# Ishikawa-lab/Area_average_interpolation

Measured on NVIDIA B200. Metric: output Mpixels/s (device-timed), higher is better.
Workload: dtype f32

## Files before the change

area_average_interpolation_b200/__init__.py:

```python
from __future__ import annotations

import ctypes as C
import os
from dataclasses import dataclass
from typing import Optional, Sequence, Tuple

import numpy as np

_HERE = os.path.dirname(os.path.abspath(__file__))
LIB_PATH = os.path.join(_HERE, "libaai_b200.so")

AAI_OK = 0
ERR_RESOLUTION_XY, ERR_RESOLUTION_NONPOS, ERR_NO_ROWS, ERR_NO_COLUMNS = 1, 2, 3, 4
ERR_ANGLE, ERR_ARGUMENT, ERR_CUDA, ERR_NO_DEVICE = 5, 6, 7, 8
F64, F32, U8, U16 = 0, 1, 2, 3
MODE_AREA_AVERAGE, MODE_FAST, MODE_AREA_AVERAGE_EXACT = 1, 2, 3
ARITH_F64, ARITH_F32, ARITH_F32_STAGED, ARITH_F32_BINNED, ARITH_F32_RING = 0, 1, 2, 3, 4

_NP_TO_AAI = {np.dtype(np.float64): F64, np.dtype(np.float32): F32, np.dtype(np.uint8): U8, np.dtype(np.uint16): U16}
_AAI_TO_NP = {v: k for k, v in _NP_TO_AAI.items()}


class AaiError(RuntimeError):
    def __init__(self, status: int, message: str):
        super().__init__(f"aai status {status}: {message}")
        self.status = status
        self.message = message


class Plan(C.Structure):
    _fields_ = [
        ("status", C.c_int32), ("scale", C.c_uint32), ("quadrant", C.c_int32), ("axis_aligned", C.c_int32),
        ("src_w", C.c_int64), ("src_h", C.c_int64), ("mod_w", C.c_int64), ("mod_h", C.c_int64),
        ("dst_w", C.c_int64), ("dst_h", C.c_int64),
        ("theta_deg", C.c_double), ("sin_t", C.c_double), ("cos_t", C.c_double),
        ("iso_x", C.c_double), ("iso_y", C.c_double), ("ratio", C.c_double), ("side", C.c_double),
        ("dst_iso_x", C.c_double), ("dst_iso_y", C.c_double), ("off_ix", C.c_double), ("off_iy", C.c_double),
        ("off_x", C.c_double), ("off_y", C.c_double), ("reach", C.c_double),
    ]

    @property
    def message(self) -> str:
        return status_string(self.status)

    @property
    def dst_isocenter(self) -> Tuple[float, float]:
        return (self.dst_iso_x, self.dst_iso_y)


class Image(C.Structure):
    _fields_ = [
        ("data", C.c_void_p), ("pitch_bytes", C.c_int64), ("width", C.c_int64), ("height", C.c_int64),
        ("y0", C.c_int64), ("rows", C.c_int64), ("dtype", C.c_int32), ("channels", C.c_int32),
    ]


_lib_handle = None


def lib() -> C.CDLL:
    global _lib_handle
    if _lib_handle is None:
        if not os.path.exists(LIB_PATH):
            raise ImportError(
                f"{LIB_PATH} is missing: run `python -c 'import __graft_entry__ as g; g.build()'` "
                "(nvcc, sm_100a).  There is no CPU fallback.")
        L = C.CDLL(LIB_PATH)
        L.aai_plan_create.restype = C.c_int
        L.aai_plan_create.argtypes = [C.c_int64, C.c_int64] + [C.c_double] * 7 + [C.POINTER(Plan)]
        L.aai_status_string.restype = C.c_char_p
        L.aai_status_string.argtypes = [C.c_int]
        L.aai_last_error.restype = C.c_char_p
        L.aai_partition_rows.restype = C.c_int
        L.aai_partition_rows.argtypes = [C.POINTER(Plan), C.c_int, C.POINTER(C.c_int64)]
        L.aai_partition_rows_weighted.restype = C.c_int
        L.aai_partition_rows_weighted.argtypes = [C.POINTER(Plan), C.c_int, C.c_double, C.POINTER(C.c_int64)]
        L.aai_band_empty_weight.restype = C.c_double
        L.aai_band_empty_weight.argtypes = [C.POINTER(Plan), C.c_int, C.c_int]
        L.aai_band_source_window.restype = C.c_int
        L.aai_band_source_window.argtypes = [C.POINTER(Plan), C.c_int64, C.c_int64] + [C.POINTER(C.c_int64)] * 4
        L.aai_covered_pixels.restype = C.c_int64
        L.aai_covered_pixels.argtypes = [C.POINTER(Plan), C.c_int64, C.c_int64]
        L.aai_device_count.restype = C.c_int
        L.aai_image_alloc.restype = C.c_int
        L.aai_image_alloc.argtypes = [C.POINTER(Image), C.c_int] + [C.c_int64] * 4 + [C.c_int32, C.c_int32]
        L.aai_image_free.restype = C.c_int
        L.aai_image_free.argtypes = [C.POINTER(Image), C.c_int]
        L.aai_image_upload.restype = C.c_int
        L.aai_image_upload.argtypes = [C.POINTER(Image), C.POINTER(Image), C.c_int, C.c_void_p]
        L.aai_image_download.restype = C.c_int
        L.aai_image_download.argtypes = [C.POINTER(Image), C.POINTER(Image), C.c_int, C.c_void_p]
        L.aai_image_copy_rows.restype = C.c_int
        L.aai_image_copy_rows.argtypes = [C.POINTER(Image), C.POINTER(Image), C.c_int64, C.c_int64, C.c_int, C.c_void_p]
        L.aai_ipc_export.restype = C.c_int
        L.aai_ipc_export.argtypes = [C.c_void_p, C.c_char_p]
        L.aai_ipc_open.restype = C.c_int
        L.aai_ipc_open.argtypes = [C.c_char_p, C.c_int, C.POINTER(C.c_void_p)]
        L.aai_ipc_close.restype = C.c_int
        L.aai_ipc_close.argtypes = [C.c_void_p, C.c_int]
        L.aai_measure_fp32_tflops.restype = C.c_int
        L.aai_measure_fp32_tflops.argtypes = [C.c_int, C.POINTER(C.c_double)]
        L.aai_expand_device.restype = C.c_int
        L.aai_expand_device.argtypes = [C.POINTER(Plan), C.POINTER(Image), C.POINTER(Image), C.c_int, C.c_void_p]
        L.aai_run_device.restype = C.c_int
        L.aai_run_device.argtypes = [C.POINTER(Plan), C.c_int, C.c_int, C.POINTER(Image), C.POINTER(Image),
                                     C.c_int64, C.c_int64, C.c_int, C.c_void_p]
        L.aai_run_device_batch.restype = C.c_int
        L.aai_run_device_batch.argtypes = [C.POINTER(Plan), C.c_int, C.c_int, C.POINTER(Image), C.POINTER(Image),
                                           C.c_int, C.c_int, C.c_void_p]
        L.aai_run_device_adjoint.restype = C.c_int
        L.aai_run_device_adjoint.argtypes = [C.POINTER(Plan), C.c_int, C.POINTER(Image), C.POINTER(Image), C.c_int,
                                             C.c_int, C.c_void_p]
        L.aai_run_host.restype = C.c_int
        L.aai_run_host.argtypes = [C.POINTER(Plan), C.c_int, C.c_int, C.POINTER(Image), C.POINTER(Image),
                                   C.POINTER(C.c_int), C.c_int]
        L.aai_run_host_band.restype = C.c_int
        L.aai_run_host_band.argtypes = [C.POINTER(Plan), C.c_int, C.c_int, C.POINTER(Image), C.POINTER(Image),
                                        C.c_int64, C.c_int64, C.c_int, C.c_void_p, C.c_int]
        L.aai_run_host_batch.restype = C.c_int
        L.aai_run_host_batch.argtypes = [C.POINTER(Plan), C.c_int, C.c_int, C.POINTER(Image), C.POINTER(Image),
                                         C.c_int, C.c_int, C.c_void_p, C.c_int]
        L.aai_peer_create.restype = C.c_int
        L.aai_peer_create.argtypes = [C.POINTER(Plan), C.c_int32, C.c_int32, C.c_int, C.c_int, C.c_int,
                                      C.POINTER(C.c_void_p)]
        L.aai_peer_export.restype = C.c_int
        L.aai_peer_export.argtypes = [C.c_void_p, C.c_char_p]
        L.aai_peer_connect.restype = C.c_int
        L.aai_peer_connect.argtypes = [C.c_void_p, C.c_char_p]
        L.aai_peer_owned_rows.restype = C.c_int
        L.aai_peer_owned_rows.argtypes = [C.c_void_p, C.POINTER(C.c_int64), C.POINTER(C.c_int64)]
        L.aai_peer_band.restype = C.c_int
        L.aai_peer_band.argtypes = [C.c_void_p, C.POINTER(C.c_int64), C.POINTER(C.c_int64)]
        L.aai_peer_run.restype = C.c_int
        L.aai_peer_run.argtypes = [C.c_void_p, C.c_int, C.c_int, C.POINTER(Image), C.POINTER(Image), C.c_void_p, C.c_int]
        L.aai_peer_device_source.restype = C.c_int
        L.aai_peer_device_source.argtypes = [C.c_void_p, C.POINTER(Image)]
        L.aai_peer_upload_chunks.restype = C.c_int
        L.aai_peer_upload_chunks.argtypes = [C.c_int]
        L.aai_peer_last_timing.restype = C.c_int
        L.aai_peer_last_timing.argtypes = [C.c_void_p, C.POINTER(C.c_float)]
        L.aai_peer_destroy.restype = C.c_int
        L.aai_peer_destroy.argtypes = [C.c_void_p]
        L.aai_launch_count.restype = C.c_int64
        L.aai_last_host_timing.restype = C.c_int
        L.aai_last_host_timing.argtypes = [C.POINTER(C.c_float)] * 3
        _lib_handle = L
    return _lib_handle


def status_string(status: int) -> str:
    return lib().aai_status_string(int(status)).decode()


def last_error() -> str:
    return lib().aai_last_error().decode()


def _check(status: int) -> None:
    if status != AAI_OK:
        msg = status_string(status)
        if status >= ERR_ARGUMENT:
            detail = last_error()
            if detail:
                msg = f"{msg} {detail}"
        raise AaiError(status, msg)


def _pair(v) -> Tuple[float, float]:
    if np.isscalar(v):
        return float(v), float(v)
    return float(v[0]), float(v[1])


def make_plan(src_w: int, src_h: int, src_resolution, dst_resolution, src_isocenter, rotation_angle: float) -> Plan:
    rx, ry = _pair(src_resolution)
    dx, dy = _pair(dst_resolution)
    ix, iy = _pair(src_isocenter)
    p = Plan()
    lib().aai_plan_create(int(src_w), int(src_h), rx, ry, dx, dy, ix, iy, float(rotation_angle), C.byref(p))
    return p


def band_empty_weight(plan: Plan, mode: int = MODE_AREA_AVERAGE, arith: int = ARITH_F32) -> float:
    return float(lib().aai_band_empty_weight(C.byref(plan), int(mode), int(arith)))


def partition_rows(plan: Plan, n_parts: int, empty_weight: Optional[float] = None) -> list:
    b = (C.c_int64 * (n_parts + 1))()
    if empty_weight is None:
        _check(lib().aai_partition_rows(C.byref(plan), int(n_parts), b))
    else:
        _check(lib().aai_partition_rows_weighted(C.byref(plan), int(n_parts), float(empty_weight), b))
    return list(b)


def band_source_window(plan: Plan, row0: int, row1: int) -> Tuple[int, int, int, int]:
    v = [C.c_int64() for _ in range(4)]
    _check(lib().aai_band_source_window(C.byref(plan), int(row0), int(row1), *[C.byref(a) for a in v]))
    return tuple(a.value for a in v)


def covered_pixels(plan: Plan, row0: int = 0, row1: Optional[int] = None) -> int:
    return int(lib().aai_covered_pixels(C.byref(plan), int(row0), int(plan.dst_h if row1 is None else row1)))


def device_count() -> int:
    return int(lib().aai_device_count())


def launch_count() -> int:
    return int(lib().aai_launch_count())


def last_host_timing() -> dict:
    a, b, c = C.c_float(), C.c_float(), C.c_float()
    _check(lib().aai_last_host_timing(C.byref(a), C.byref(b), C.byref(c)))
    return {"h2d_ms": a.value, "kernel_ms": b.value, "d2h_ms": c.value}


def _host_image(arr: np.ndarray) -> Image:
    if arr.dtype not in _NP_TO_AAI:
        raise TypeError(f"unsupported dtype {arr.dtype}; use float64, float32, uint8 or uint16")
    if arr.ndim == 2:
        h, w = arr.shape
        ch = 1
    elif arr.ndim == 3:
        h, w, ch = arr.shape
    else:
        raise ValueError("image must be [h, w] or [h, w, channels]")
    if arr.strides[-1] != arr.itemsize or (arr.ndim == 3 and arr.strides[1] != ch * arr.itemsize):
        raise ValueError("image rows must be dense (only the row pitch may be padded)")
    return Image(arr.ctypes.data, arr.strides[0], w, h, 0, h, _NP_TO_AAI[arr.dtype], ch)


def tensor_image(t, y0: int = 0, height: Optional[int] = None) -> Image:
    import torch

    dt = {torch.float64: F64, torch.float32: F32, torch.uint8: U8, torch.uint16: U16}[t.dtype]
    if t.dim() == 2:
        rows, w = t.shape
        ch = 1
    else:
        rows, w, ch = t.shape
    if t.stride(-1) != 1 or (t.dim() == 3 and t.stride(1) != ch):
        raise ValueError("tensor rows must be dense")
    return Image(t.data_ptr(), t.stride(0) * t.element_size(), w, int(height if height is not None else rows),
                 int(y0), rows, dt, ch)


def image_alloc(device: int, width: int, height: int, dtype: int, channels: int = 1, y0: int = 0,
                rows: Optional[int] = None) -> Image:
    img = Image()
    _check(lib().aai_image_alloc(C.byref(img), int(device), int(width), int(height), int(y0),
                                 int(height if rows is None else rows), int(dtype), int(channels)))
    return img


def image_free(img: Image, device: int) -> None:
    _check(lib().aai_image_free(C.byref(img), int(device)))


def image_upload(device_img: Image, host_img: Image, device: int = 0, stream: int = 0) -> None:
    _check(lib().aai_image_upload(C.byref(device_img), C.byref(host_img), int(device), C.c_void_p(stream)))


def image_download(host_img: Image, device_img: Image, device: int = 0, stream: int = 0) -> None:
    _check(lib().aai_image_download(C.byref(host_img), C.byref(device_img), int(device), C.c_void_p(stream)))


def image_copy_rows(dst_img: Image, src_img: Image, y0: int, y1: int, device: int = 0, stream: int = 0) -> None:
    _check(lib().aai_image_copy_rows(C.byref(dst_img), C.byref(src_img), int(y0), int(y1), int(device),
                                     C.c_void_p(stream)))


def ipc_export(device_ptr: int) -> bytes:
    buf = C.create_string_buffer(64)
    _check(lib().aai_ipc_export(C.c_void_p(device_ptr), buf))
    return buf.raw


def ipc_open(handle: bytes, device: int) -> int:
    p = C.c_void_p()
    _check(lib().aai_ipc_open(handle, int(device), C.byref(p)))
    return p.value


def ipc_close(device_ptr: int, device: int) -> None:
    _check(lib().aai_ipc_close(C.c_void_p(device_ptr), int(device)))


def measure_fp32_tflops(device: int = 0) -> float:
    v = C.c_double(0.0)
    _check(lib().aai_measure_fp32_tflops(int(device), C.byref(v)))
    return v.value


def expand_device(plan: Plan, src_img: Image, dst_mod_img: Image, device: int = 0, stream: int = 0) -> None:
    _check(lib().aai_expand_device(C.byref(plan), C.byref(src_img), C.byref(dst_mod_img), int(device), C.c_void_p(stream)))


def run_device(plan: Plan, src_img: Image, dst_img: Image, row0: int = 0, row1: Optional[int] = None,
               mode: int = MODE_AREA_AVERAGE, arith: int = ARITH_F64, device: int = 0, stream: int = 0) -> None:
    _check(lib().aai_run_device(C.byref(plan), int(mode), int(arith), C.byref(src_img), C.byref(dst_img),
                                int(row0), int(plan.dst_h if row1 is None else row1), int(device),
                                C.c_void_p(stream)))


def run_device_batch(plan: Plan, src_imgs: Sequence[Image], dst_imgs: Sequence[Image], mode: int = MODE_AREA_AVERAGE,
                     arith: int = ARITH_F64, device: int = 0, stream: int = 0) -> None:
    n = len(src_imgs)
    sa, da = (Image * n)(*src_imgs), (Image * n)(*dst_imgs)
    _check(lib().aai_run_device_batch(C.byref(plan), int(mode), int(arith), sa, da, n, int(device), C.c_void_p(stream)))


def run_device_adjoint(plan: Plan, canvas_imgs: Sequence[Image], src_imgs: Sequence[Image],
                       mode: int = MODE_AREA_AVERAGE, device: int = 0, stream: int = 0) -> None:
    n = len(canvas_imgs)
    if len(src_imgs) != n:
        raise ValueError("run_device_adjoint: as many source images as canvas images")
    ca, sa = (Image * max(n, 1))(*canvas_imgs), (Image * max(n, 1))(*src_imgs)
    _check(lib().aai_run_device_adjoint(C.byref(plan), int(mode), ca, sa, n, int(device), C.c_void_p(stream)))


def run_host(plan: Plan, src: np.ndarray, dst: np.ndarray, mode: int = MODE_AREA_AVERAGE, arith: int = ARITH_F64,
             devices: Optional[Sequence[int]] = None) -> None:
    si, di = _host_image(src), _host_image(dst)
    if devices:
        arr = (C.c_int * len(devices))(*devices)
        n = len(devices)
    else:
        arr, n = None, 0
    _check(lib().aai_run_host(C.byref(plan), int(mode), int(arith), C.byref(si), C.byref(di), arr, n))


def run_host_band(plan: Plan, src_img: Image, dst_img: Image, row0: int, row1: int, mode: int = MODE_AREA_AVERAGE,
                  arith: int = ARITH_F64, device: int = 0, stream: int = 0, synchronize: bool = True) -> None:
    _check(lib().aai_run_host_band(C.byref(plan), int(mode), int(arith), C.byref(src_img), C.byref(dst_img),
                                   int(row0), int(row1), int(device), C.c_void_p(stream), int(bool(synchronize))))


def run_host_batch(plan: Plan, src_imgs: Sequence[Image], dst_imgs: Sequence[Image], mode: int = MODE_AREA_AVERAGE,
                   arith: int = ARITH_F64, device: int = 0, stream: int = 0, synchronize: bool = True) -> None:
    n = len(src_imgs)
    sa, da = (Image * n)(*src_imgs), (Image * n)(*dst_imgs)
    _check(lib().aai_run_host_batch(C.byref(plan), int(mode), int(arith), sa, da, n, int(device), C.c_void_p(stream),
                                    int(bool(synchronize))))


PEER_BLOB_BYTES = 2048


def peer_upload_chunks(n: int = 0) -> int:
    return int(lib().aai_peer_upload_chunks(int(n)))


class PeerGroup:

    def __init__(self, plan: Plan, dtype: int, channels: int, rank: int, world: int, device: int, all_gather):
        self.plan, self.rank, self.world, self.device = plan, rank, world, device
        self._h = C.c_void_p()
        _check(lib().aai_peer_create(C.byref(plan), int(dtype), int(channels), int(rank), int(world), int(device),
                                     C.byref(self._h)))
        try:
            buf = C.create_string_buffer(PEER_BLOB_BYTES)
            _check(lib().aai_peer_export(self._h, buf))
            blobs = all_gather(buf.raw)
            if len(blobs) != world or any(len(b) != PEER_BLOB_BYTES for b in blobs):
                raise AaiError(ERR_ARGUMENT, "peer group: the gather must return one blob per rank, in rank order")
            _check(lib().aai_peer_connect(self._h, b"".join(blobs)))
        except Exception:
            self.close()
            raise

    def owned_rows(self) -> Tuple[int, int]:
        a, b = C.c_int64(), C.c_int64()
        _check(lib().aai_peer_owned_rows(self._h, C.byref(a), C.byref(b)))
        return a.value, b.value

    def band(self) -> Tuple[int, int]:
        a, b = C.c_int64(), C.c_int64()
        _check(lib().aai_peer_band(self._h, C.byref(a), C.byref(b)))
        return a.value, b.value

    def device_source(self) -> Image:
        img = Image()
        _check(lib().aai_peer_device_source(self._h, C.byref(img)))
        return img

    def run(self, host_src: Image, host_dst: Image, mode: int = MODE_AREA_AVERAGE, arith: int = ARITH_F64,
            stream: int = 0, synchronize: bool = True) -> None:
        _check(lib().aai_peer_run(self._h, int(mode), int(arith), C.byref(host_src), C.byref(host_dst),
                                  C.c_void_p(stream), int(bool(synchronize))))

    def last_timing(self) -> dict:
        ms = (C.c_float * 4)()
        _check(lib().aai_peer_last_timing(self._h, ms))
        return {"upload_ms": ms[0], "pull_ms": ms[1], "kernel_ms": ms[2], "download_ms": ms[3]}

    def close(self) -> None:
        if self._h:
            lib().aai_peer_destroy(self._h)
            self._h = C.c_void_p()


@dataclass
class Result:
    ok: bool
    message: str
    dst: np.ndarray
    dst_isocenter: Tuple[float, float]
    plan: Plan


class AreaAverageInterpolation:

    def __init__(self, arith: int = ARITH_F64, devices: Optional[Sequence[int]] = None, out_dtype=None):
        self.arith = arith
        self.devices = list(devices) if devices else None
        self.out_dtype = out_dtype

    def _run(self, mode, src, srcResolution, dstResolution, srcIsocenter, rotationAngle, dstIsocenter):
        src = np.asarray(src)
        if src.ndim == 1 and src.size == 0:
            src = src.reshape(0, 0)
        if src.ndim not in (2, 3):
            raise ValueError("src must be [h, w] or [h, w, c]")
        h, w = src.shape[0], src.shape[1]
        plan = make_plan(w, h, srcResolution, dstResolution, srcIsocenter, rotationAngle)
        if plan.status != AAI_OK:
            if plan.status > ERR_NO_COLUMNS:
                raise AaiError(plan.status, plan.message)
            return Result(False, plan.message, np.empty((0, 0)), tuple(dstIsocenter), plan)
        if src.dtype not in _NP_TO_AAI:
            src = src.astype(np.float64)
        src = np.ascontiguousarray(src)
        out_dtype = np.dtype(self.out_dtype) if self.out_dtype is not None else (
            np.dtype(np.float64) if src.dtype in (np.float64, np.uint16) or self.arith == ARITH_F64
            else np.dtype(np.float32))
        shape = (plan.dst_h, plan.dst_w) + ((src.shape[2],) if src.ndim == 3 else ())
        dst = np.empty(shape, dtype=out_dtype)
        if dst.size:
            run_host(plan, src, dst, mode, self.arith, self.devices)
        return Result(True, "", dst, plan.dst_isocenter, plan)

    def areaAverageInterpolation(self, src, srcResolution, dstResolution, srcIsocenter, rotationAngle,
                                 dstIsocenter=(0.0, 0.0)) -> Result:
        return self._run(MODE_AREA_AVERAGE, src, srcResolution, dstResolution, srcIsocenter, rotationAngle,
                         dstIsocenter)

    def fastAreaAverageInterpolation(self, src, srcResolution, dstResolution, srcIsocenter, rotationAngle,
                                     dstIsocenter=(0.0, 0.0)) -> Result:
        return self._run(MODE_FAST, src, srcResolution, dstResolution, srcIsocenter, rotationAngle, dstIsocenter)

    def exactAreaAverageInterpolation(self, src, srcResolution, dstResolution, srcIsocenter, rotationAngle,
                                      dstIsocenter=(0.0, 0.0)) -> Result:
        return self._run(MODE_AREA_AVERAGE_EXACT, src, srcResolution, dstResolution, srcIsocenter, rotationAngle,
                         dstIsocenter)


def __getattr__(name):
    if name in ("resample", "resample_adjoint"):
        from . import torch_ops

        return getattr(torch_ops, name)
    raise AttributeError(f"module {__name__!r} has no attribute {name!r}")


__all__ = [
    "AreaAverageInterpolation", "Result", "Plan", "Image", "AaiError", "make_plan", "partition_rows",
    "band_source_window", "covered_pixels", "device_count", "launch_count", "last_host_timing", "run_device", "run_device_batch", "run_device_adjoint",
    "expand_device", "measure_fp32_tflops", "image_alloc", "image_free", "image_upload", "image_download", "image_copy_rows",
    "ipc_export", "ipc_open", "ipc_close",
    "run_host", "run_host_band", "run_host_batch", "PeerGroup", "tensor_image", "status_string", "last_error", "lib", "LIB_PATH",
]
```

area_average_interpolation_b200/csrc/aai_capi.cu:

```cuda
#include <cuda_runtime.h>

#include <atomic>
#include <cmath>
#include <cstdarg>
#include <cstdio>
#include <cstdlib>
#include <cstring>
#include <mutex>
#include <string>
#include <thread>
#include <vector>

#include "aai_internal.h"

namespace {

thread_local char g_error[512] = "";
std::atomic<int64_t> g_launches{0};
thread_local float g_h2d_ms = -1.f, g_kernel_ms = -1.f, g_d2h_ms = -1.f;

int cuda_fail(cudaError_t e, const char *what) {
    aai_set_error("%s: %s (%s)", what, cudaGetErrorString(e), cudaGetErrorName(e));
    return (e == cudaErrorNoDevice || e == cudaErrorInsufficientDriver) ? AAI_ERR_NO_DEVICE : AAI_ERR_CUDA;
}
#define AAI_CUDA(call)                                   \
    do {                                                 \
        cudaError_t e_ = (call);                         \
        if (e_ != cudaSuccess) return cuda_fail(e_, #call); \
    } while (0)

bool image_ok(const aai_image *im) {
    return im && im->data && aai_elem_size(im->dtype) && im->channels >= 1 && im->channels <= 4 && im->width > 0 &&
           im->height > 0 && im->rows >= 0 && im->y0 >= 0 && im->y0 + im->rows <= im->height &&
           im->pitch_bytes >= (int64_t)(im->width * im->channels * (int64_t)aai_elem_size(im->dtype));
}

struct Workspace {
    void *ptr[2] = {nullptr, nullptr};
    size_t cap[2] = {0, 0};
    cudaStream_t stream = nullptr;
    cudaStream_t up = nullptr, dn = nullptr;
    cudaEvent_t ev[4] = {nullptr, nullptr, nullptr, nullptr};
    std::vector<cudaEvent_t> chunk_ev;
    cudaEvent_t fork = nullptr, join_up = nullptr, join_dn = nullptr;
    cudaEvent_t done = nullptr;
    bool done_valid = false;
    std::mutex busy;
};
constexpr int kMaxDevices = 64;
std::mutex g_ws_mutex;
Workspace g_ws[kMaxDevices];

int workspace_get(int device, size_t bytes0, size_t bytes1, Workspace **out) {
    if (device < 0 || device >= kMaxDevices) {
        aai_set_error("device index %d out of range", device);
        return AAI_ERR_ARGUMENT;
    }
    std::lock_guard<std::mutex> lock(g_ws_mutex);
    Workspace &w = g_ws[device];
    AAI_CUDA(cudaSetDevice(device));
    if (!w.stream) {
        AAI_CUDA(cudaStreamCreateWithFlags(&w.stream, cudaStreamNonBlocking));
        AAI_CUDA(cudaStreamCreateWithFlags(&w.up, cudaStreamNonBlocking));
        AAI_CUDA(cudaStreamCreateWithFlags(&w.dn, cudaStreamNonBlocking));
        for (auto &e : w.ev) AAI_CUDA(cudaEventCreate(&e));
        AAI_CUDA(cudaEventCreateWithFlags(&w.fork, cudaEventDisableTiming));
        AAI_CUDA(cudaEventCreateWithFlags(&w.join_up, cudaEventDisableTiming));
        AAI_CUDA(cudaEventCreateWithFlags(&w.join_dn, cudaEventDisableTiming));
        AAI_CUDA(cudaEventCreateWithFlags(&w.done, cudaEventDisableTiming));
    }
    const size_t need[2] = {bytes0, bytes1};
    for (int k = 0; k < 2; ++k) {
        if (w.cap[k] < need[k]) {
            if (w.ptr[k]) AAI_CUDA(cudaFree(w.ptr[k]));
            w.ptr[k] = nullptr;
            w.cap[k] = 0;
            AAI_CUDA(cudaMalloc(&w.ptr[k], need[k]));
            w.cap[k] = need[k];
        }
    }
    *out = &w;
    return AAI_OK;
}

int64_t round_up(int64_t v, int64_t a) { return (v + a - 1) / a * a; }

}

void aai_count_extra_launches(int n) { g_launches.fetch_add(n); }

int aai_check_dtype_pair(const char *who, int src_dtype, int dst_dtype) {
    if (aai_dtype_pair_ok(src_dtype, dst_dtype)) return AAI_OK;
    aai_set_error("%s: a %s source cannot write a %s canvas (a uint16 canvas takes a uint16 source; a uint16 source "
                  "writes float64, float32 or uint16 canvases)",
                  who, aai_dtype_name(src_dtype), aai_dtype_name(dst_dtype));
    return AAI_ERR_ARGUMENT;
}

void aai_set_error(const char *fmt, ...) {
    va_list ap;
    va_start(ap, fmt);
    vsnprintf(g_error, sizeof g_error, fmt, ap);
    va_end(ap);
}

AaiKernelParams aai_make_kernel_params(const aai_plan &p, const aai_image &src, const aai_image &dst, int64_t row0,
                                       int64_t row1) {
    AaiKernelParams k;
    std::memset(&k, 0, sizeof k);
    k.side = p.side;
    k.off_ix = p.off_ix;
    k.off_iy = p.off_iy;
    k.iso_x = p.iso_x;
    k.iso_y = p.iso_y;
    k.off_x = p.off_x;
    k.off_y = p.off_y;
    const double c = p.cos_t, s = p.sin_t, h = p.side / 2;
    {
        const double u0 = (p.off_ix * p.side - p.iso_x) + p.off_x, v0 = (p.off_iy * p.side - p.iso_y) + p.off_y;
        k.aff_x0 = (u0 * c + v0 * s) + p.iso_x;
        k.aff_y0 = (-u0 * s + v0 * c) + p.iso_y;
        k.aff_xx = p.side * c;
        k.aff_xy = p.side * s;
        k.aff_yx = -p.side * s;
        k.aff_yy = p.side * c;
        k.ext32 = (float)(h * (c + s) + 0.5 + 2e-6);
    }
    k.shape = aai_make_shape(c, s, p.side);
    const AaiShape &g = k.shape;
    k.shapef = aai_make_shape_f(c, s, p.side);
    const double amp = std::fmax(1.0, std::fmax(g.inv_c, g.inv_s));
    const uint64_t max_e = (uint64_t)(p.mod_w > p.mod_h ? p.mod_w : p.mod_h);
    k.f32_ok = (s > 0.0 && c > 0.0 && amp <= 20.0 && max_e * p.scale < 0x100000000ULL) ? 1 : 0;
    k.quirk = 1;
    k.reach = p.reach;
    k.hb = h * (c + s);
    k.mod_w = (int32_t)p.mod_w;
    k.mod_h = (int32_t)p.mod_h;
    k.dst_w = (int32_t)p.dst_w;
    k.dst_h = (int32_t)p.dst_h;
    k.scale = (int32_t)p.scale;
    k.quadrant = p.quadrant;
    const int32_t mw1 = (int32_t)p.mod_w - 1, mh1 = (int32_t)p.mod_h - 1;
    switch (p.quadrant) {
        case 0: k.e_axi = 1; k.e_axj = 0; k.e_ax0 = 0; k.e_ayi = 0; k.e_ayj = 1; k.e_ay0 = 0; break;
        case 1: k.e_axi = 0; k.e_axj = 1; k.e_ax0 = 0; k.e_ayi = -1; k.e_ayj = 0; k.e_ay0 = mw1; break;
        case 2: k.e_axi = -1; k.e_axj = 0; k.e_ax0 = mw1; k.e_ayi = 0; k.e_ayj = -1; k.e_ay0 = mh1; break;
        default: k.e_axi = 0; k.e_axj = -1; k.e_ax0 = mh1; k.e_ayi = 1; k.e_ayj = 0; k.e_ay0 = 0; break;
    }
    k.div_magic = p.scale > 1 ? (uint32_t)(0x100000000ULL / p.scale) + 1u : 0u;
    k.src = src.data;
    k.src_pitch = src.pitch_bytes;
    k.src_w = (int32_t)src.width;
    k.src_h = (int32_t)src.height;
    k.src_y0 = (int32_t)src.y0;
    k.src_rows = (int32_t)src.rows;
    k.channels = src.channels;
    k.dst = dst.data;
    k.dst_pitch = dst.pitch_bytes;
    k.dst_y0 = (int32_t)dst.y0;
    k.row0 = (int32_t)row0;
    k.row1 = (int32_t)row1;
    return k;
}

static int launch_rows(const aai_plan &plan, int mode, int arith, AaiKernelParams kp, int src_dtype, int dst_dtype,
                       void *stream) {
    const int32_t row0 = kp.row0, row1 = kp.row1;
    kp.staged = arith == AAI_ARITH_F32_STAGED ? 1 : arith == AAI_ARITH_F32_BINNED ? 2 : arith == AAI_ARITH_F32_RING ? 3 : 0;
    if (kp.staged) arith = AAI_ARITH_F32;
    for (int64_t a = row0; a < row1; a += AAI_MAX_ROWS_PER_LAUNCH) {
        kp.row0 = (int32_t)a;
        kp.row1 = (int32_t)(a + AAI_MAX_ROWS_PER_LAUNCH < row1 ? a + AAI_MAX_ROWS_PER_LAUNCH : row1);
        {
            const int64_t n = kp.row1 - kp.row0, e = n / 8 > 64 ? 64 : (n / 8 > 0 ? n / 8 : 1);
            kp.reverse_rows = aai_covered_pixels(&plan, kp.row0, kp.row0 + e) > aai_covered_pixels(&plan, kp.row1 - e, kp.row1) ? 1 : 0;
        }
        int e;
        if (mode == AAI_MODE_FAST)
            e = aai_launch_fast(kp, arith, src_dtype, dst_dtype, stream);
        else if (plan.axis_aligned)
            e = aai_launch_separable(kp, arith, src_dtype, dst_dtype, stream);
        else
            e = aai_launch_overlap(kp, arith, src_dtype, dst_dtype, stream);
        if (e != (int)cudaSuccess) return e;
        g_launches.fetch_add(1);
    }
    return (int)cudaSuccess;
}

extern "C" {

const char *aai_last_error(void) { return g_error; }

int64_t aai_launch_count(void) { return g_launches.load(); }

int aai_device_count(void) {
    int n = 0;
    if (cudaGetDeviceCount(&n) != cudaSuccess) {
        cudaGetLastError();
        return 0;
    }
    return n;
}

int aai_image_alloc(aai_image *img, int device, int64_t width, int64_t height, int64_t y0, int64_t rows,
                    int32_t dtype, int32_t channels) {
    if (!img || !aai_elem_size(dtype) || channels < 1 || channels > 4 || width <= 0 || height <= 0 || rows < 0 ||
        y0 < 0 || y0 + rows > height) {
        aai_set_error("aai_image_alloc: bad argument");
        return AAI_ERR_ARGUMENT;
    }
    AAI_CUDA(cudaSetDevice(device));
    std::memset(img, 0, sizeof *img);
    img->width = width;
    img->height = height;
    img->y0 = y0;
    img->rows = rows;
    img->dtype = dtype;
    img->channels = channels;
    img->pitch_bytes = round_up(width * channels * (int64_t)aai_elem_size(dtype), 512);
    const size_t bytes = (size_t)img->pitch_bytes * (size_t)(rows > 0 ? rows : 1);
    AAI_CUDA(cudaMalloc(&img->data, bytes));
    return AAI_OK;
}

int aai_image_free(aai_image *img, int device) {
    if (!img) return AAI_ERR_ARGUMENT;
    if (img->data) {
        AAI_CUDA(cudaSetDevice(device));
        AAI_CUDA(cudaFree(img->data));
    }
    img->data = nullptr;
    return AAI_OK;
}

static int copy_rows(const aai_image *dst, const aai_image *src, cudaMemcpyKind kind, int device, void *stream) {
    if (!image_ok(dst) || !image_ok(src) || dst->width != src->width || dst->height != src->height ||
        dst->dtype != src->dtype || dst->channels != src->channels) {
        aai_set_error("aai_image copy: incompatible images");
        return AAI_ERR_ARGUMENT;
    }
    const aai_image *band = (kind == cudaMemcpyHostToDevice) ? dst : src;
    const aai_image *full = (kind == cudaMemcpyHostToDevice) ? src : dst;
    if (band->y0 < full->y0 || band->y0 + band->rows > full->y0 + full->rows) {
        aai_set_error("aai_image copy: band rows [%lld,%lld) not inside [%lld,%lld)", (long long)band->y0,
                      (long long)(band->y0 + band->rows), (long long)full->y0, (long long)(full->y0 + full->rows));
        return AAI_ERR_ARGUMENT;
    }
    if (band->rows == 0) return AAI_OK;
    AAI_CUDA(cudaSetDevice(device));
    const size_t row_bytes = (size_t)(band->width * band->channels) * aai_elem_size(band->dtype);
    const char *s = (const char *)src->data + (kind == cudaMemcpyHostToDevice ? (band->y0 - src->y0) * src->pitch_bytes : 0);
    char *d = (char *)dst->data + (kind == cudaMemcpyDeviceToHost ? (band->y0 - dst->y0) * dst->pitch_bytes : 0);
    if ((size_t)dst->pitch_bytes == row_bytes && (size_t)src->pitch_bytes == row_bytes)
        AAI_CUDA(cudaMemcpyAsync(d, s, row_bytes * (size_t)band->rows, kind, (cudaStream_t)stream));
    else
        AAI_CUDA(cudaMemcpy2DAsync(d, (size_t)dst->pitch_bytes, s, (size_t)src->pitch_bytes, row_bytes,
                                   (size_t)band->rows, kind, (cudaStream_t)stream));
    return AAI_OK;
}

int aai_image_upload(const aai_image *device_img, const aai_image *host_img, int device, void *stream) {
    return copy_rows(device_img, host_img, cudaMemcpyHostToDevice, device, stream);
}
int aai_image_download(const aai_image *host_img, const aai_image *device_img, int device, void *stream) {
    return copy_rows(host_img, device_img, cudaMemcpyDeviceToHost, device, stream);
}

int aai_image_copy_rows(const aai_image *dst, const aai_image *src, int64_t y0, int64_t y1, int device, void *stream) {
    if (!image_ok(dst) || !image_ok(src) || dst->width != src->width || dst->height != src->height ||
        dst->dtype != src->dtype || dst->channels != src->channels || y0 < 0 || y1 < y0 || y0 < dst->y0 ||
        y1 > dst->y0 + dst->rows || y0 < src->y0 || y1 > src->y0 + src->rows) {
        aai_set_error("aai_image_copy_rows: incompatible images or rows [%lld,%lld) not present", (long long)y0,
                      (long long)y1);
        return AAI_ERR_ARGUMENT;
    }
    if (y1 == y0) return AAI_OK;
    AAI_CUDA(cudaSetDevice(device));
    const size_t row_bytes = (size_t)(src->width * src->channels) * aai_elem_size(src->dtype);
    char *d = (char *)dst->data + (y0 - dst->y0) * dst->pitch_bytes;
    const char *s = (const char *)src->data + (y0 - src->y0) * src->pitch_bytes;
    if ((size_t)dst->pitch_bytes == row_bytes && (size_t)src->pitch_bytes == row_bytes)
        AAI_CUDA(cudaMemcpyAsync(d, s, row_bytes * (size_t)(y1 - y0), cudaMemcpyDefault, (cudaStream_t)stream));
    else
        AAI_CUDA(cudaMemcpy2DAsync(d, (size_t)dst->pitch_bytes, s, (size_t)src->pitch_bytes, row_bytes,
                                   (size_t)(y1 - y0), cudaMemcpyDefault, (cudaStream_t)stream));
    return AAI_OK;
}

int aai_ipc_export(const void *device_ptr, unsigned char handle[AAI_IPC_HANDLE_BYTES]) {
    static_assert(sizeof(cudaIpcMemHandle_t) == AAI_IPC_HANDLE_BYTES, "IPC handle size");
    if (!device_ptr || !handle) return AAI_ERR_ARGUMENT;
    cudaIpcMemHandle_t h;
    AAI_CUDA(cudaIpcGetMemHandle(&h, const_cast<void *>(device_ptr)));
    std::memcpy(handle, &h, sizeof h);
    return AAI_OK;
}

int aai_ipc_open(const unsigned char handle[AAI_IPC_HANDLE_BYTES], int device, void **device_ptr) {
    if (!handle || !device_ptr) return AAI_ERR_ARGUMENT;
    AAI_CUDA(cudaSetDevice(device));
    cudaIpcMemHandle_t h;
    std::memcpy(&h, handle, sizeof h);
    AAI_CUDA(cudaIpcOpenMemHandle(device_ptr, h, cudaIpcMemLazyEnablePeerAccess));
    return AAI_OK;
}

int aai_ipc_close(void *device_ptr, int device) {
    if (!device_ptr) return AAI_OK;
    AAI_CUDA(cudaSetDevice(device));
    AAI_CUDA(cudaIpcCloseMemHandle(device_ptr));
    return AAI_OK;
}

int aai_run_device(const aai_plan *plan, int mode, int arith, const aai_image *src, const aai_image *dst,
                   int64_t row0, int64_t row1, int device, void *stream) {
    if (!plan) {
        aai_set_error("aai_run_device: null plan");
        return AAI_ERR_ARGUMENT;
    }
    if (plan->status != AAI_OK) return plan->status;
    if (!image_ok(src) || !image_ok(dst) || src->width != plan->src_w || src->height != plan->src_h ||
        dst->width != plan->dst_w || dst->height != plan->dst_h || src->channels != dst->channels) {
        aai_set_error("aai_run_device: images do not match the plan (src %lldx%lld, canvas %lldx%lld)",
                      (long long)plan->src_w, (long long)plan->src_h, (long long)plan->dst_w, (long long)plan->dst_h);
        return AAI_ERR_ARGUMENT;
    }
    if (const int r = aai_check_dtype_pair("aai_run_device", src->dtype, dst->dtype)) return r;
    if (mode != AAI_MODE_AREA_AVERAGE && mode != AAI_MODE_FAST && mode != AAI_MODE_AREA_AVERAGE_EXACT) {
        aai_set_error("aai_run_device: interpolation mode must be 1, 2 or 3");
        return AAI_ERR_ARGUMENT;
    }
    if (arith != AAI_ARITH_F64 && arith != AAI_ARITH_F32 && arith != AAI_ARITH_F32_STAGED && arith != AAI_ARITH_F32_BINNED &&
        arith != AAI_ARITH_F32_RING) {
        aai_set_error("aai_run_device: unknown arithmetic %d", arith);
        return AAI_ERR_ARGUMENT;
    }
    if (row0 < 0 || row1 > plan->dst_h || row0 > row1 || row0 < dst->y0 || row1 > dst->y0 + dst->rows) {
        aai_set_error("aai_run_device: rows [%lld,%lld) outside the destination band", (long long)row0, (long long)row1);
        return AAI_ERR_ARGUMENT;
    }
    if (row0 == row1) return AAI_OK;
    int64_t sx0, sx1, sy0, sy1;
    aai_band_source_window(plan, row0, row1, &sx0, &sx1, &sy0, &sy1);
    if (sy1 > sy0 && (sy0 < src->y0 || sy1 > src->y0 + src->rows)) {
        aai_set_error("aai_run_device: source rows [%lld,%lld) needed, [%lld,%lld) present", (long long)sy0,
                      (long long)sy1, (long long)src->y0, (long long)(src->y0 + src->rows));
        return AAI_ERR_ARGUMENT;
    }
    AAI_CUDA(cudaSetDevice(device));
    AaiKernelParams kp = aai_make_kernel_params(*plan, *src, *dst, row0, row1);
    kp.quirk = mode == AAI_MODE_AREA_AVERAGE_EXACT ? 0 : 1;
    const int e = launch_rows(*plan, mode, arith, kp, src->dtype, dst->dtype, stream);
    if (e != (int)cudaSuccess) return cuda_fail((cudaError_t)e, "kernel launch");
    return AAI_OK;
}

static int check_host_images(const char *who, const aai_plan *plan, const aai_image *src, const aai_image *dst,
                             bool whole) {
    if (!plan) {
        aai_set_error("%s: null plan", who);
        return AAI_ERR_ARGUMENT;
    }
    if (plan->status != AAI_OK) return plan->status;
    if (!image_ok(src) || !image_ok(dst) || src->width != plan->src_w || src->height != plan->src_h ||
        dst->width != plan->dst_w || dst->height != plan->dst_h || src->channels != dst->channels) {
        aai_set_error("%s: host images do not match the plan", who);
        return AAI_ERR_ARGUMENT;
    }
    if (const int r = aai_check_dtype_pair(who, src->dtype, dst->dtype)) return r;
    if (whole && (src->y0 != 0 || src->rows != src->height || dst->y0 != 0 || dst->rows != dst->height)) {
        aai_set_error("%s: whole host images expected", who);
        return AAI_ERR_ARGUMENT;
    }
    return AAI_OK;
}

int aai_expand_device(const aai_plan *plan, const aai_image *src, const aai_image *dst_mod, int device, void *stream) {
    if (!plan) {
        aai_set_error("aai_expand_device: null plan");
        return AAI_ERR_ARGUMENT;
    }
    if (plan->status != AAI_OK) return plan->status;
    if (!image_ok(src) || !image_ok(dst_mod) || src->width != plan->src_w || src->height != plan->src_h ||
        src->y0 != 0 || src->rows != src->height || dst_mod->width != plan->mod_w || dst_mod->height != plan->mod_h ||
        dst_mod->y0 != 0 || dst_mod->rows != dst_mod->height || src->dtype != dst_mod->dtype ||
        src->channels != dst_mod->channels) {
        aai_set_error("aai_expand_device: need a whole source image and a whole %lld x %lld image of the same type",
                      (long long)plan->mod_w, (long long)plan->mod_h);
        return AAI_ERR_ARGUMENT;
    }
    AAI_CUDA(cudaSetDevice(device));
    aai_image canvas = *dst_mod;
    canvas.width = plan->dst_w;
    canvas.height = plan->dst_h;
    AaiKernelParams kp = aai_make_kernel_params(*plan, *src, canvas, 0, 0);
    kp.dst = dst_mod->data;
    kp.dst_pitch = dst_mod->pitch_bytes;
    const int e = aai_launch_expand(kp, (int)aai_elem_size(src->dtype), stream);
    if (e != (int)cudaSuccess) return cuda_fail((cudaError_t)e, "expand kernel launch");
    g_launches.fetch_add(1);
    return AAI_OK;
}

int aai_measure_fp32_tflops(int device, double *tflops) {
    if (!tflops) {
        aai_set_error("aai_measure_fp32_tflops: null result");
        return AAI_ERR_ARGUMENT;
    }
    AAI_CUDA(cudaSetDevice(device));
    int sms = 0;
    AAI_CUDA(cudaDeviceGetAttribute(&sms, cudaDevAttrMultiProcessorCount, device));
    float *scratch = nullptr;
    cudaEvent_t e0 = nullptr, e1 = nullptr;
    double flop = 0.0, best = 0.0;
    int rc = AAI_OK;
    cudaError_t ce = cudaMalloc(&scratch, 256);
    if (ce == cudaSuccess) ce = cudaEventCreate(&e0);
    if (ce == cudaSuccess) ce = cudaEventCreate(&e1);
    if (ce != cudaSuccess) rc = cuda_fail(ce, "FP32 probe set-up");
    for (int rep = 0; rep < 4 && rc == AAI_OK; ++rep) {
        cudaEventRecord(e0, 0);
        const int e = aai_probe_fp32(sms * 8, 1 << 16, scratch, &flop, nullptr);
        cudaEventRecord(e1, 0);
        if (e != (int)cudaSuccess || cudaEventSynchronize(e1) != cudaSuccess) {
            rc = cuda_fail((cudaError_t)(e != (int)cudaSuccess ? e : (int)cudaGetLastError()), "FP32 probe");
            break;
        }
        float ms = 0.f;
        cudaEventElapsedTime(&ms, e0, e1);
        if (rep > 0 && ms > 0.f && flop / (ms * 1e-3) / 1e12 > best) best = flop / (ms * 1e-3) / 1e12;
    }
    if (e0) cudaEventDestroy(e0);
    if (e1) cudaEventDestroy(e1);
    if (scratch) cudaFree(scratch);
    *tflops = best;
    return rc;
}

static bool whole_image_stack(const aai_plan *plan, const aai_image *srcs, const aai_image *dsts, int n_images,
                              int64_t *sstride_out, int64_t *dstride_out) {
    const aai_image &s0 = srcs[0], &d0 = dsts[0];
    bool stack = n_images > 1 && image_ok(&s0) && image_ok(&d0) && s0.y0 == 0 && s0.rows == s0.height && d0.y0 == 0 &&
                 d0.rows == d0.height && s0.width == plan->src_w && s0.height == plan->src_h &&
                 d0.width == plan->dst_w && d0.height == plan->dst_h && s0.channels == d0.channels;
    const int64_t sstride = stack ? (const char *)srcs[1].data - (const char *)s0.data : 0;
    const int64_t dstride = stack ? (const char *)dsts[1].data - (const char *)d0.data : 0;
    for (int k = 1; stack && k < n_images; ++k) {
        const aai_image &a = srcs[k], &b = dsts[k];
        stack = a.data == (const char *)s0.data + k * sstride && b.data == (char *)d0.data + k * dstride &&
                a.pitch_bytes == s0.pitch_bytes && b.pitch_bytes == d0.pitch_bytes && a.dtype == s0.dtype &&
                b.dtype == d0.dtype && a.width == s0.width && a.height == s0.height && a.y0 == 0 &&
                a.rows == a.height && b.width == d0.width && b.height == d0.height && b.y0 == 0 &&
                b.rows == b.height && a.channels == s0.channels && b.channels == d0.channels;
    }
    *sstride_out = sstride;
    *dstride_out = dstride;
    return stack && sstride > 0 && dstride > 0 && sstride % s0.pitch_bytes == 0 && dstride % d0.pitch_bytes == 0 &&
           sstride / s0.pitch_bytes < (1 << 30) && dstride / d0.pitch_bytes < (1 << 30);
}

int aai_run_device_batch(const aai_plan *plan, int mode, int arith, const aai_image *srcs, const aai_image *dsts,
                         int n_images, int device, void *stream) {
    if (!plan || !srcs || !dsts || n_images <= 0) {
        aai_set_error("aai_run_device_batch: bad argument");
        return AAI_ERR_ARGUMENT;
    }
    if (plan->status != AAI_OK) return plan->status;
    for (int k = 0; k < n_images; ++k)
        if (const int r = aai_check_dtype_pair("aai_run_device_batch", srcs[k].dtype, dsts[k].dtype)) return r;
    const aai_image &s0 = srcs[0], &d0 = dsts[0];
    const bool known = (mode == AAI_MODE_AREA_AVERAGE || mode == AAI_MODE_FAST || mode == AAI_MODE_AREA_AVERAGE_EXACT) &&
                       (arith == AAI_ARITH_F64 || arith == AAI_ARITH_F32 || arith == AAI_ARITH_F32_STAGED ||
                        arith == AAI_ARITH_F32_BINNED || arith == AAI_ARITH_F32_RING);
    int64_t sstride = 0, dstride = 0;
    if (known && whole_image_stack(plan, srcs, dsts, n_images, &sstride, &dstride)) {
        AAI_CUDA(cudaSetDevice(device));
        const int64_t srows = sstride / s0.pitch_bytes, drows = dstride / d0.pitch_bytes;
        int64_t per_launch = 65535;
        const int64_t most_rows = srows > drows ? srows : drows;
        if (per_launch * most_rows > 0x7fffffffLL) per_launch = 0x7fffffffLL / most_rows;
        if (per_launch < 1) per_launch = 1;
        for (int first = 0; first < n_images; first += (int)per_launch) {
            const int n = n_images - first < per_launch ? n_images - first : (int)per_launch;
            AaiKernelParams kp = aai_make_kernel_params(*plan, srcs[first], dsts[first], 0, plan->dst_h);
            kp.quirk = mode == AAI_MODE_AREA_AVERAGE_EXACT ? 0 : 1;
            kp.batch = n;
            kp.src_batch_stride = sstride;
            kp.dst_batch_stride = dstride;
            kp.src_batch_rows = (int32_t)srows;
            kp.dst_batch_rows = (int32_t)drows;
            const int e = launch_rows(*plan, mode, arith, kp, s0.dtype, d0.dtype, stream);
            if (e != (int)cudaSuccess) return cuda_fail((cudaError_t)e, "batched kernel launch");
        }
        return AAI_OK;
    }
    for (int k = 0; k < n_images; ++k) {
        const int r = aai_run_device(plan, mode, arith, &srcs[k], &dsts[k], 0, plan->dst_h, device, stream);
        if (r != AAI_OK) return r;
    }
    return AAI_OK;
}

static int check_adjoint_args(const aai_plan *plan, int mode, const aai_image *canvas_grads, const aai_image *src_grads,
                              int n_images) {
    const char *who = "aai_run_device_adjoint";
    if (!plan || !canvas_grads || !src_grads || n_images <= 0) {
        aai_set_error("%s: null pointer or no images", who);
        return AAI_ERR_ARGUMENT;
    }
    if (plan->status != AAI_OK) return plan->status;
    if (mode != AAI_MODE_AREA_AVERAGE && mode != AAI_MODE_FAST && mode != AAI_MODE_AREA_AVERAGE_EXACT) {
        aai_set_error("%s: interpolation mode must be 1, 2 or 3", who);
        return AAI_ERR_ARGUMENT;
    }
    for (int k = 0; k < n_images; ++k) {
        const aai_image &g = canvas_grads[k], &s = src_grads[k];
        if (!g.data || !s.data) {
            aai_set_error("%s: image %d has no data", who, k);
            return AAI_ERR_ARGUMENT;
        }
        if ((g.dtype != AAI_F32 && g.dtype != AAI_F64) || (s.dtype != AAI_F32 && s.dtype != AAI_F64) ||
            g.dtype != s.dtype) {
            aai_set_error("%s: gradients are float32 or float64, the same on both sides (image %d: canvas %s, source %s)",
                          who, k, aai_dtype_name(g.dtype), aai_dtype_name(s.dtype));
            return AAI_ERR_ARGUMENT;
        }
        if (g.channels != s.channels) {
            aai_set_error("%s: image %d: the canvas has %d channels, the source %d", who, k, (int)g.channels,
                          (int)s.channels);
            return AAI_ERR_ARGUMENT;
        }
        if (g.y0 != 0 || g.rows != g.height || s.y0 != 0 || s.rows != s.height) {
            aai_set_error("%s: image %d: whole images expected (y0 = 0, rows = height)", who, k);
            return AAI_ERR_ARGUMENT;
        }
        if (g.width != plan->dst_w || g.height != plan->dst_h || s.width != plan->src_w || s.height != plan->src_h ||
            !image_ok(&g) || !image_ok(&s)) {
            aai_set_error("%s: image %d does not match the plan (source %lldx%lld, canvas %lldx%lld, 1-4 channels, "
                          "pitch >= row bytes)",
                          who, k, (long long)plan->src_w, (long long)plan->src_h, (long long)plan->dst_w,
                          (long long)plan->dst_h);
            return AAI_ERR_ARGUMENT;
        }
    }
    return AAI_OK;
}

int aai_run_device_adjoint(const aai_plan *plan, int mode, const aai_image *canvas_grads, const aai_image *src_grads,
                           int n_images, int device, void *stream) {
    if (const int r = check_adjoint_args(plan, mode, canvas_grads, src_grads, n_images)) return r;
    AAI_CUDA(cudaSetDevice(device));
    cudaStream_t st = (cudaStream_t)stream;
    const aai_image &s0 = src_grads[0], &g0 = canvas_grads[0];
    AaiAdjointParams ap;
    std::memset(&ap, 0, sizeof ap);
    ap.kp = aai_make_kernel_params(*plan, s0, g0, 0, plan->dst_h);
    ap.kp.quirk = mode == AAI_MODE_AREA_AVERAGE_EXACT ? 0 : 1;
    const size_t rcp_bytes = (size_t)plan->dst_w * (size_t)plan->dst_h * sizeof(double);
    AAI_CUDA(cudaMallocAsync((void **)&ap.rcp, rcp_bytes, st));
    int e = (int)cudaSuccess;
    const char *what = "adjoint normaliser launch";
    for (int64_t a = 0; a < plan->dst_h && e == (int)cudaSuccess; a += AAI_MAX_ROWS_PER_LAUNCH) {
        ap.row0 = (int32_t)a;
        ap.row1 = (int32_t)(a + AAI_MAX_ROWS_PER_LAUNCH < plan->dst_h ? a + AAI_MAX_ROWS_PER_LAUNCH : plan->dst_h);
        e = aai_launch_adjoint_norm(ap, mode, plan->axis_aligned, st);
        if (e == (int)cudaSuccess) g_launches.fetch_add(1);
    }
    ap.inv_side = 1.0 / plan->side;
    auto gather = [&](int first, int n, int64_t canvas_stride, int64_t out_stride) {
        ap.kp.channels = src_grads[first].channels;
        ap.canvas = canvas_grads[first].data;
        ap.canvas_pitch = canvas_grads[first].pitch_bytes;
        ap.canvas_stride = canvas_stride;
        ap.out = src_grads[first].data;
        ap.out_pitch = src_grads[first].pitch_bytes;
        ap.out_stride = out_stride;
        for (int64_t a = 0; a < plan->src_h; a += AAI_MAX_ROWS_PER_LAUNCH) {
            ap.row0 = (int32_t)a;
            ap.row1 = (int32_t)(a + AAI_MAX_ROWS_PER_LAUNCH < plan->src_h ? a + AAI_MAX_ROWS_PER_LAUNCH : plan->src_h);
            const int r = aai_launch_adjoint_gather(ap, mode, plan->axis_aligned, src_grads[first].dtype, n, st);
            if (r != (int)cudaSuccess) return r;
            g_launches.fetch_add(1);
        }
        return (int)cudaSuccess;
    };
    if (e == (int)cudaSuccess) {
        what = "adjoint gather launch";
        int64_t sstride = 0, cstride = 0;
        if (whole_image_stack(plan, src_grads, canvas_grads, n_images, &sstride, &cstride)) {
            for (int first = 0; first < n_images && e == (int)cudaSuccess; first += 65535)
                e = gather(first, n_images - first < 65535 ? n_images - first : 65535, cstride, sstride);
        } else {
            for (int k = 0; k < n_images && e == (int)cudaSuccess; ++k) e = gather(k, 1, 0, 0);
        }
    }
    const cudaError_t ef = cudaFreeAsync(ap.rcp, st);
    if (e != (int)cudaSuccess) return cuda_fail((cudaError_t)e, what);
    AAI_CUDA(ef);
    return AAI_OK;
}

int aai_run_host_band(const aai_plan *plan, int mode, int arith, const aai_image *src, const aai_image *dst,
                      int64_t row0, int64_t row1, int device, void *stream, int synchronize) {
    int r = check_host_images("aai_run_host_band", plan, src, dst, false);
    if (r != AAI_OK) return r;
    if (row0 < 0 || row1 > plan->dst_h || row0 > row1) {
        aai_set_error("aai_run_host_band: bad rows [%lld,%lld)", (long long)row0, (long long)row1);
        return AAI_ERR_ARGUMENT;
    }
    if (row1 == row0) return AAI_OK;
    if (aai_device_count() <= device || device < 0) {
        aai_set_error("aai_run_host_band: device %d not present; this library has no CPU fallback", device);
        return aai_device_count() <= 0 ? AAI_ERR_NO_DEVICE : AAI_ERR_ARGUMENT;
    }
    int64_t sx0, sx1, sy0, sy1;
    aai_band_source_window(plan, row0, row1, &sx0, &sx1, &sy0, &sy1);
    aai_image dsrc = *src, ddst = *dst;
    dsrc.y0 = sy0;
    dsrc.rows = sy1 - sy0;
    dsrc.pitch_bytes = round_up(src->width * src->channels * (int64_t)aai_elem_size(src->dtype), 512);
    ddst.y0 = row0;
    ddst.rows = row1 - row0;
    ddst.pitch_bytes = round_up(dst->width * dst->channels * (int64_t)aai_elem_size(dst->dtype), 512);
    std::lock_guard<std::mutex> busy(g_ws[device < kMaxDevices ? device : 0].busy);
    Workspace *w = nullptr;
    r = workspace_get(device, (size_t)dsrc.pitch_bytes * (size_t)(dsrc.rows > 0 ? dsrc.rows : 1),
                      (size_t)ddst.pitch_bytes * (size_t)ddst.rows, &w);
    if (r != AAI_OK) return r;
    dsrc.data = w->ptr[0];
    ddst.data = w->ptr[1];
    cudaStream_t st = stream ? (cudaStream_t)stream : w->stream;
    if (w->done_valid) AAI_CUDA(cudaStreamWaitEvent(st, w->done, 0));
    const size_t total_bytes = (size_t)dsrc.pitch_bytes * (size_t)dsrc.rows + (size_t)ddst.pitch_bytes * (size_t)ddst.rows;
    const int64_t band_rows = row1 - row0;
    int chunks = 1;
    if (total_bytes >= ((size_t)48 << 20) && band_rows >= 64) chunks = (int)(band_rows < 32 * 16 ? band_rows / 16 : 32);
#ifdef AAI_DEV_KNOBS
    if (const char *e = getenv("AAI_HOST_CHUNKS")) chunks = atoi(e) > 0 ? atoi(e) : chunks;
#endif
    if (chunks > band_rows) chunks = (int)band_rows;
    if (chunks <= 1) {
        AAI_CUDA(cudaEventRecord(w->ev[0], st));
        if (dsrc.rows > 0) {
            r = aai_image_upload(&dsrc, src, device, st);
            if (r != AAI_OK) return r;
        }
        AAI_CUDA(cudaEventRecord(w->ev[1], st));
        r = aai_run_device(plan, mode, arith, &dsrc, &ddst, row0, row1, device, st);
        if (r != AAI_OK) return r;
        AAI_CUDA(cudaEventRecord(w->ev[2], st));
        r = aai_image_download(dst, &ddst, device, st);
        if (r != AAI_OK) return r;
        AAI_CUDA(cudaEventRecord(w->ev[3], st));
        AAI_CUDA(cudaEventRecord(w->done, st));
        w->done_valid = true;
        if (synchronize || !stream) {
            AAI_CUDA(cudaStreamSynchronize(st));
            AAI_CUDA(cudaEventElapsedTime(&g_h2d_ms, w->ev[0], w->ev[1]));
            AAI_CUDA(cudaEventElapsedTime(&g_kernel_ms, w->ev[1], w->ev[2]));
            AAI_CUDA(cudaEventElapsedTime(&g_d2h_ms, w->ev[2], w->ev[3]));
        }
        return AAI_OK;
    }
    while ((int)w->chunk_ev.size() < 2 * chunks) {
        cudaEvent_t e;
        AAI_CUDA(cudaEventCreateWithFlags(&e, cudaEventDisableTiming));
        w->chunk_ev.push_back(e);
    }
    AAI_CUDA(cudaEventRecord(w->ev[0], st));
    cudaStream_t s_k = st;
    AAI_CUDA(cudaStreamWaitEvent(w->up, w->ev[0], 0));
    AAI_CUDA(cudaStreamWaitEvent(w->dn, w->ev[0], 0));
    int64_t have_lo = 0, have_hi = 0;
    bool have_any = false;
    auto upload_rows = [&](int64_t a, int64_t b) -> int {
        if (b <= a) return AAI_OK;
        aai_image part = dsrc;
        part.data = (char *)dsrc.data + (a - dsrc.y0) * dsrc.pitch_bytes;
        part.y0 = a;
        part.rows = b - a;
        return aai_image_upload(&part, src, device, w->up);
    };
    for (int c = 0; c < chunks; ++c) {
        const int64_t r0 = row0 + band_rows * c / chunks, r1 = row0 + band_rows * (c + 1) / chunks;
        int64_t cx0, cx1, a, b;
        aai_band_source_window(plan, r0, r1, &cx0, &cx1, &a, &b);
        if (b > a) {
            if (!have_any) {
                r = upload_rows(a, b);
                have_lo = a;
                have_hi = b;
                have_any = true;
            } else {
                r = AAI_OK;
                if (a < have_lo) {
                    r = upload_rows(a, have_lo);
                    have_lo = a;
                }
                if (r == AAI_OK && b > have_hi) {
                    r = upload_rows(have_hi, b);
                    have_hi = b;
                }
            }
            if (r != AAI_OK) return r;
        }
        AAI_CUDA(cudaEventRecord(w->chunk_ev[2 * c], w->up));
        AAI_CUDA(cudaStreamWaitEvent(s_k, w->chunk_ev[2 * c], 0));
        r = aai_run_device(plan, mode, arith, &dsrc, &ddst, r0, r1, device, s_k);
        if (r != AAI_OK) return r;
        AAI_CUDA(cudaEventRecord(w->chunk_ev[2 * c + 1], s_k));
        AAI_CUDA(cudaStreamWaitEvent(w->dn, w->chunk_ev[2 * c + 1], 0));
        aai_image part = ddst;
        part.data = (char *)ddst.data + (r0 - ddst.y0) * ddst.pitch_bytes;
        part.y0 = r0;
        part.rows = r1 - r0;
        r = aai_image_download(dst, &part, device, w->dn);
        if (r != AAI_OK) return r;
    }
    AAI_CUDA(cudaEventRecord(w->join_up, w->up));
    AAI_CUDA(cudaEventRecord(w->join_dn, w->dn));
    AAI_CUDA(cudaStreamWaitEvent(st, w->join_up, 0));
    AAI_CUDA(cudaStreamWaitEvent(st, w->join_dn, 0));
    AAI_CUDA(cudaEventRecord(w->ev[3], st));
    AAI_CUDA(cudaEventRecord(w->done, st));
    w->done_valid = true;
    if (synchronize || !stream) {
        AAI_CUDA(cudaStreamSynchronize(st));
        float total = 0.f;
        AAI_CUDA(cudaEventElapsedTime(&total, w->ev[0], w->ev[3]));
        g_h2d_ms = total;
        g_kernel_ms = 0.f;
        g_d2h_ms = 0.f;
    }
    return AAI_OK;
}

int aai_run_host_batch(const aai_plan *plan, int mode, int arith, const aai_image *srcs, const aai_image *dsts,
                       int n_images, int device, void *stream, int synchronize) {
    if (!plan || !srcs || !dsts || n_images <= 0) {
        aai_set_error("aai_run_host_batch: bad argument");
        return AAI_ERR_ARGUMENT;
    }
    for (int k = 0; k < n_images; ++k) {
        const int r = check_host_images("aai_run_host_batch", plan, &srcs[k], &dsts[k], true);
        if (r != AAI_OK) return r;
        if (srcs[k].dtype != srcs[0].dtype || dsts[k].dtype != dsts[0].dtype || srcs[k].channels != srcs[0].channels) {
            aai_set_error("aai_run_host_batch: the images of a batch must share element types and channel count");
            return AAI_ERR_ARGUMENT;
        }
    }
    if (aai_device_count() <= device || device < 0) {
        aai_set_error("aai_run_host_batch: device %d not present; this library has no CPU fallback", device);
        return aai_device_count() <= 0 ? AAI_ERR_NO_DEVICE : AAI_ERR_ARGUMENT;
    }
    constexpr int kRing = 3;
    aai_image ds = srcs[0], dd = dsts[0];
    ds.pitch_bytes = round_up(ds.width * ds.channels * (int64_t)aai_elem_size(ds.dtype), 512);
    dd.pitch_bytes = round_up(dd.width * dd.channels * (int64_t)aai_elem_size(dd.dtype), 512);
    const size_t s_bytes = (size_t)ds.pitch_bytes * (size_t)ds.height, d_bytes = (size_t)dd.pitch_bytes * (size_t)dd.height;
    int per = (int)(((size_t)192 << 20) / (s_bytes + d_bytes));
    per = per < 1 ? 1 : (per > 16 ? 16 : per);
    if (per > n_images) per = n_images;
    const int groups = (n_images + per - 1) / per;
    std::lock_guard<std::mutex> busy(g_ws[device < kMaxDevices ? device : 0].busy);
    Workspace *w = nullptr;
    int r = workspace_get(device, s_bytes * (size_t)per * kRing, d_bytes * (size_t)per * kRing, &w);
    if (r != AAI_OK) return r;
    cudaStream_t st = stream ? (cudaStream_t)stream : w->stream;
    if (w->done_valid) AAI_CUDA(cudaStreamWaitEvent(st, w->done, 0));
    while ((int)w->chunk_ev.size() < 3 * kRing) {
        cudaEvent_t e;
        AAI_CUDA(cudaEventCreateWithFlags(&e, cudaEventDisableTiming));
        w->chunk_ev.push_back(e);
    }
    AAI_CUDA(cudaEventRecord(w->ev[0], st));
    AAI_CUDA(cudaStreamWaitEvent(w->up, w->ev[0], 0));
    AAI_CUDA(cudaStreamWaitEvent(w->dn, w->ev[0], 0));
    std::vector<aai_image> gs((size_t)per), gd((size_t)per);
    for (int g = 0; g < groups; ++g) {
        const int slot = g % kRing, first = g * per, n = n_images - first < per ? n_images - first : per;
        cudaEvent_t up_done = w->chunk_ev[3 * slot], k_done = w->chunk_ev[3 * slot + 1], dn_done = w->chunk_ev[3 * slot + 2];
        if (g >= kRing) {
            AAI_CUDA(cudaStreamWaitEvent(w->up, k_done, 0));
            AAI_CUDA(cudaStreamWaitEvent(st, dn_done, 0));
        }
        for (int k = 0; k < n; ++k) {
            gs[(size_t)k] = ds;
            gs[(size_t)k].data = (char *)w->ptr[0] + ((size_t)slot * per + k) * s_bytes;
            gd[(size_t)k] = dd;
            gd[(size_t)k].data = (char *)w->ptr[1] + ((size_t)slot * per + k) * d_bytes;
            r = aai_image_upload(&gs[(size_t)k], &srcs[first + k], device, w->up);
            if (r != AAI_OK) return r;
        }
        AAI_CUDA(cudaEventRecord(up_done, w->up));
        AAI_CUDA(cudaStreamWaitEvent(st, up_done, 0));
        r = aai_run_device_batch(plan, mode, arith, gs.data(), gd.data(), n, device, st);
        if (r != AAI_OK) return r;
        AAI_CUDA(cudaEventRecord(k_done, st));
        AAI_CUDA(cudaStreamWaitEvent(w->dn, k_done, 0));
        for (int k = 0; k < n; ++k) {
            r = aai_image_download(&dsts[first + k], &gd[(size_t)k], device, w->dn);
            if (r != AAI_OK) return r;
        }
        AAI_CUDA(cudaEventRecord(dn_done, w->dn));
    }
    AAI_CUDA(cudaEventRecord(w->join_up, w->up));
    AAI_CUDA(cudaEventRecord(w->join_dn, w->dn));
    AAI_CUDA(cudaStreamWaitEvent(st, w->join_up, 0));
    AAI_CUDA(cudaStreamWaitEvent(st, w->join_dn, 0));
    AAI_CUDA(cudaEventRecord(w->ev[3], st));
    AAI_CUDA(cudaEventRecord(w->done, st));
    w->done_valid = true;
    if (synchronize || !stream) {
        AAI_CUDA(cudaStreamSynchronize(st));
        float total = 0.f;
        AAI_CUDA(cudaEventElapsedTime(&total, w->ev[0], w->ev[3]));
        g_h2d_ms = total;
        g_kernel_ms = 0.f;
        g_d2h_ms = 0.f;
    }
    return AAI_OK;
}

int aai_run_host(const aai_plan *plan, int mode, int arith, const aai_image *src, const aai_image *dst,
                 const int *devices, int n_devices) {
    int rc = check_host_images("aai_run_host", plan, src, dst, true);
    if (rc != AAI_OK) return rc;
    const int dev0 = 0;
    if (!devices || n_devices <= 0) {
        devices = &dev0;
        n_devices = 1;
    }
    const int have = aai_device_count();
    if (have <= 0) {
        aai_set_error("aai_run_host: no CUDA device; this library has no CPU fallback");
        return AAI_ERR_NO_DEVICE;
    }
    for (int k = 0; k < n_devices; ++k)
        if (devices[k] < 0 || devices[k] >= have) {
            aai_set_error("aai_run_host: device %d not present (%d devices)", devices[k], have);
            return AAI_ERR_ARGUMENT;
        }
    std::vector<int64_t> bounds((size_t)n_devices + 1);
    rc = aai_partition_rows_weighted(plan, n_devices, aai_band_empty_weight(plan, mode, arith), bounds.data());
    if (rc != AAI_OK) return rc;
    if (n_devices == 1) return aai_run_host_band(plan, mode, arith, src, dst, 0, plan->dst_h, devices[0], nullptr, 1);

    std::vector<int> status((size_t)n_devices, AAI_OK);
    std::vector<std::string> messages((size_t)n_devices);
    std::vector<float> t_h2d((size_t)n_devices, 0.f), t_k((size_t)n_devices, 0.f), t_d2h((size_t)n_devices, 0.f);
    std::vector<std::thread> pool;
    for (int k = 0; k < n_devices; ++k)
        pool.emplace_back([&, k]() {
            status[(size_t)k] = aai_run_host_band(plan, mode, arith, src, dst, bounds[(size_t)k],
                                                  bounds[(size_t)k + 1], devices[k], nullptr, 1);
            if (status[(size_t)k] != AAI_OK) messages[(size_t)k] = g_error;
            t_h2d[(size_t)k] = g_h2d_ms;
            t_k[(size_t)k] = g_kernel_ms;
            t_d2h[(size_t)k] = g_d2h_ms;
        });
    for (auto &t : pool) t.join();
    for (int k = 0; k < n_devices; ++k)
        if (status[(size_t)k] != AAI_OK) {
            aai_set_error("device %d: %s", devices[k], messages[(size_t)k].c_str());
            return status[(size_t)k];
        }
    g_h2d_ms = g_kernel_ms = g_d2h_ms = 0.f;
    for (int k = 0; k < n_devices; ++k) {
        g_h2d_ms = std::fmax(g_h2d_ms, t_h2d[(size_t)k]);
        g_kernel_ms = std::fmax(g_kernel_ms, t_k[(size_t)k]);
        g_d2h_ms = std::fmax(g_d2h_ms, t_d2h[(size_t)k]);
    }
    return AAI_OK;
}

int aai_last_host_timing(float *h2d_ms, float *kernel_ms, float *d2h_ms) {
    if (g_kernel_ms < 0.f) return AAI_ERR_ARGUMENT;
    if (h2d_ms) *h2d_ms = g_h2d_ms;
    if (kernel_ms) *kernel_ms = g_kernel_ms;
    if (d2h_ms) *d2h_ms = g_d2h_ms;
    return AAI_OK;
}

}
```

area_average_interpolation_b200/csrc/aai_device.cuh:

```cuda
#ifndef AAI_DEVICE_CUH_
#define AAI_DEVICE_CUH_

#include <cuda.h>
#include <cuda_runtime.h>

#include <cfloat>
#include <cstdint>

#include "aai_cell.cuh"
#include "aai_internal.h"

namespace aai_dev {

constexpr int TILE_W = AAI_TILE_W;
constexpr int TILE_H = AAI_TILE_H;

template <typename T>
struct Elem;
template <>
struct Elem<double> {
    static constexpr int dtype = AAI_F64;
    static constexpr CUtensorMapDataType tmap = CU_TENSOR_MAP_DATA_TYPE_FLOAT64;
};
template <>
struct Elem<float> {
    static constexpr int dtype = AAI_F32;
    static constexpr CUtensorMapDataType tmap = CU_TENSOR_MAP_DATA_TYPE_FLOAT32;
};
template <>
struct Elem<uint16_t> {
    static constexpr int dtype = AAI_U16;
    static constexpr CUtensorMapDataType tmap = CU_TENSOR_MAP_DATA_TYPE_UINT16;
};
template <>
struct Elem<uint8_t> {
    static constexpr int dtype = AAI_U8;
    static constexpr CUtensorMapDataType tmap = CU_TENSOR_MAP_DATA_TYPE_UINT8;
};
template <typename TI, typename TO>
constexpr bool pair_ok() {
    return aai_dtype_pair_ok(Elem<TI>::dtype, Elem<TO>::dtype);
}

template <typename T>
struct SrcLoad;
template <>
struct SrcLoad<double> {
    static __device__ __forceinline__ double get(const void *row, int idx) { return __ldg((const double *)row + idx); }
};
template <>
struct SrcLoad<float> {
    static __device__ __forceinline__ double get(const void *row, int idx) {
        return (double)__ldg((const float *)row + idx);
    }
};
template <>
struct SrcLoad<uint8_t> {
    static __device__ __forceinline__ double get(const void *row, int idx) {
        return (double)__ldg((const uint8_t *)row + idx);
    }
};
template <>
struct SrcLoad<uint16_t> {
    static __device__ __forceinline__ double get(const void *row, int idx) {
        return (double)__ldg((const uint16_t *)row + idx);
    }
};

#ifndef AAI_U16_CVT_MAGIC
#define AAI_U16_CVT_MAGIC 1
#endif
__device__ __forceinline__ float u16_to_float(uint32_t v) {
#if AAI_U16_CVT_MAGIC
    return __int_as_float(0x4B000000u | v) - 8388608.0f;
#else
    return (float)v;
#endif
}
template <typename TA, typename T>
__device__ __forceinline__ TA to_arith(T v) {
    return (TA)v;
}
template <>
__device__ __forceinline__ float to_arith<float, uint16_t>(uint16_t v) {
    return u16_to_float(v);
}

template <typename T>
struct LoadF;
template <>
struct LoadF<double> {
    static __device__ __forceinline__ float get(const char *p) { return (float)__ldg((const double *)p); }
};
template <>
struct LoadF<float> {
    static __device__ __forceinline__ float get(const char *p) { return __ldg((const float *)p); }
};
template <>
struct LoadF<uint8_t> {
    static __device__ __forceinline__ float get(const char *p) { return (float)__ldg((const uint8_t *)p); }
};
template <>
struct LoadF<uint16_t> {
    static __device__ __forceinline__ float get(const char *p) { return u16_to_float(__ldg((const uint16_t *)p)); }
};

template <typename T>
__device__ __forceinline__ void store_dst(void *row, int idx, double v);
template <>
__device__ __forceinline__ void store_dst<double>(void *row, int idx, double v) {
    ((double *)row)[idx] = v;
}
template <>
__device__ __forceinline__ void store_dst<float>(void *row, int idx, double v) {
    ((float *)row)[idx] = (float)v;
}
template <>
__device__ __forceinline__ void store_dst<uint8_t>(void *row, int idx, double v) {
    double r = floor(v + 0.5);
    r = fmin(fmax(r, 0.0), 255.0);
    ((uint8_t *)row)[idx] = (uint8_t)(int)r;
}
template <>
__device__ __forceinline__ void store_dst<uint16_t>(void *row, int idx, double v) {
    double r = floor(v + 0.5);
    r = fmin(fmax(r, 0.0), 65535.0);
    ((uint16_t *)row)[idx] = (uint16_t)(int)r;
}

template <typename T>
__device__ __forceinline__ void store_f(void *row, int idx, float v);
template <>
__device__ __forceinline__ void store_f<double>(void *row, int idx, float v) {
    ((double *)row)[idx] = (double)v;
}
template <>
__device__ __forceinline__ void store_f<float>(void *row, int idx, float v) {
    ((float *)row)[idx] = v;
}
template <>
__device__ __forceinline__ void store_f<uint8_t>(void *row, int idx, float v) {
    ((uint8_t *)row)[idx] = (uint8_t)__float2int_rd(fminf(fmaxf(v + 0.5f, 0.0f), 255.0f));
}
template <>
__device__ __forceinline__ void store_f<uint16_t>(void *row, int idx, float v) {
    ((uint16_t *)row)[idx] = (uint16_t)__float2int_rd(fminf(fmaxf(v + 0.5f, 0.0f), 65535.0f));
}

__device__ __forceinline__ int src_row0(const AaiKernelParams &kp) {
    return kp.src_y0 - (int)blockIdx.z * kp.src_batch_rows;
}
__device__ __forceinline__ int dst_row0(const AaiKernelParams &kp) {
    return kp.dst_y0 - (int)blockIdx.z * kp.dst_batch_rows;
}

__device__ __forceinline__ void mod_to_src(const AaiKernelParams &kp, int mx, int my, int &sx, int &sy) {
    int ex, ey;
    switch (kp.quadrant) {
        case 0: ex = mx; ey = my; break;
        case 1: ex = my; ey = kp.mod_w - 1 - mx; break;
        case 2: ex = kp.mod_w - 1 - mx; ey = kp.mod_h - 1 - my; break;
        default: ex = kp.mod_h - 1 - my; ey = mx; break;
    }
    if (kp.scale == 1) {
        sx = ex;
        sy = ey;
    } else {
        sx = ex / kp.scale;
        sy = ey / kp.scale;
    }
}

__device__ __forceinline__ void pixel_centre(const AaiKernelParams &kp, int x, int y, double &cx, double &cy) {
    const double u = __dadd_rn(__dsub_rn(__dmul_rn(__dadd_rn((double)x, kp.off_ix), kp.side), kp.iso_x), kp.off_x);
    const double v = __dadd_rn(__dsub_rn(__dmul_rn(__dadd_rn((double)y, kp.off_iy), kp.side), kp.iso_y), kp.off_y);
    cx = __dadd_rn(__dadd_rn(__dmul_rn(u, kp.shape.cs), __dmul_rn(v, kp.shape.sn)), kp.iso_x);
    cy = __dadd_rn(__dadd_rn(__dmul_rn(-u, kp.shape.sn), __dmul_rn(v, kp.shape.cs)), kp.iso_y);
}

__device__ __forceinline__ void search_window(const AaiKernelParams &kp, double cx, double cy, int &x0, int &x1,
                                              int &y0, int &y1) {
    x0 = max(0, __double2int_rd(__dsub_rn(__dsub_rn(cx, kp.reach), 1.0)));
    x1 = min(__double2int_ru(__dadd_rn(__dadd_rn(cx, kp.reach), 1.0)), kp.mod_w - 1);
    y0 = max(0, __double2int_rd(__dsub_rn(__dsub_rn(cy, kp.reach), 1.0)));
    y1 = min(__double2int_ru(__dadd_rn(__dadd_rn(cy, kp.reach), 1.0)), kp.mod_h - 1);
}

template <typename TI, int NC>
__device__ __forceinline__ void pixel_f64(const AaiKernelParams &kp, double cx, double cy, int ix0, int ix1, int jy0,
                                          int jy1, double &sumA, double (&acc)[NC]) {
    sumA = 0.0;
#pragma unroll
    for (int ch = 0; ch < NC; ++ch) acc[ch] = 0.0;
    if (ix0 > ix1 || jy0 > jy1) return;
    const AaiShape &g = kp.shape;
    double xlT, xrT;
    aai_chord_h(g, ((double)jy0 - 0.5) - cy, xlT, xrT);
    for (int j = jy0; j <= jy1; ++j) {
        const double ry = (double)j - cy;
        double xlB, xrB;
        aai_chord_h(g, ry + 0.5, xlB, xrB);
        double yt, yb;
        aai_chord_v(g, ((double)ix0 - 0.5) - cx, yt, yb);
        double lenL = aai_overlap1(yt, yb, ry);
        for (int i = ix0; i <= ix1; ++i) {
            const double rx = (double)i - cx;
            aai_chord_v(g, rx + 0.5, yt, yb);
            const double lenR = aai_overlap1(yt, yb, ry);
            const double lenT = aai_overlap1(xlT, xrT, rx);
            const double lenB = aai_overlap1(xlB, xrB, rx);
            const double area = aai_cell_area(g, rx, ry, lenT, lenB, lenL, lenR, kp.quirk != 0);
            lenL = lenR;
            if (area != 0.0) {
                int sx, sy;
                mod_to_src(kp, i, j, sx, sy);
                const char *row = (const char *)kp.src + (int64_t)(sy - src_row0(kp)) * kp.src_pitch;
                sumA += area;
#pragma unroll
                for (int ch = 0; ch < NC; ++ch) acc[ch] += SrcLoad<TI>::get(row, sx * NC + ch) * area;
            }
        }
        xlT = xlB;
        xrT = xrB;
    }
}

template <typename TI, int NC>
__device__ __forceinline__ void pixel_fast_f64(const AaiKernelParams &kp, int x, int y, int &count, double (&acc)[NC]) {
    double cx, cy;
    pixel_centre(kp, x, y, cx, cy);
    int wx0, wx1, wy0, wy1;
    search_window(kp, cx, cy, wx0, wx1, wy0, wy1);
    const double ext = kp.hb + 1e-6;
    const int ix0 = max(wx0, __double2int_ru(cx - ext)), ix1 = min(wx1, __double2int_rd(cx + ext));
    const int jy0 = max(wy0, __double2int_ru(cy - ext)), jy1 = min(wy1, __double2int_rd(cy + ext));
    count = 0;
#pragma unroll
    for (int ch = 0; ch < NC; ++ch) acc[ch] = 0.0;
    for (int j = jy0; j <= jy1; ++j) {
        const double ry = (double)j - cy;
        for (int i = ix0; i <= ix1; ++i) {
            const double rx = (double)i - cx;
            const double u0 = rx * kp.shape.cs - ry * kp.shape.sn;
            const double v0 = rx * kp.shape.sn + ry * kp.shape.cs;
            if (fabs(u0) <= kp.shape.half && fabs(v0) <= kp.shape.half) {
                int sx, sy;
                mod_to_src(kp, i, j, sx, sy);
                const char *row = (const char *)kp.src + (int64_t)(sy - src_row0(kp)) * kp.src_pitch;
                count += 1;
#pragma unroll
                for (int ch = 0; ch < NC; ++ch) acc[ch] += SrcLoad<TI>::get(row, sx * NC + ch);
            }
        }
    }
}

__device__ __forceinline__ bool cell_range(const AaiKernelParams &kp, double cx, double cy, int &ix0, int &ix1,
                                           int &jy0, int &jy1) {
    const double ext = kp.hb + 0.5 + 1e-9;
    const int bx0 = __double2int_ru(cx - ext), bx1 = __double2int_rd(cx + ext);
    const int by0 = __double2int_ru(cy - ext), by1 = __double2int_rd(cy + ext);
    ix0 = max(0, bx0);
    ix1 = min(kp.mod_w - 1, bx1);
    jy0 = max(0, by0);
    jy1 = min(kp.mod_h - 1, by1);
    return bx0 < 0 || by0 < 0 || bx1 > kp.mod_w - 1 || by1 > kp.mod_h - 1;
}


template <typename TI, int NC>
__device__ __forceinline__ void warp_pixels_f64(const AaiKernelParams &kp, bool need, int x, int y, double &sumA,
                                                double (&acc)[NC]) {
    constexpr unsigned FULL = 0xffffffffu;
    const int lane = (threadIdx.y * TILE_W + threadIdx.x) & 31;
    unsigned todo = __ballot_sync(FULL, need);
    while (todo) {
        const int src_lane = __ffs(todo) - 1;
        todo &= todo - 1;
        const int px = __shfl_sync(FULL, x, src_lane), py = __shfl_sync(FULL, y, src_lane);
        double cx, cy;
        pixel_centre(kp, px, py, cx, cy);
        int i0, i1, j0, j1;
        cell_range(kp, cx, cy, i0, i1, j0, j1);
        const int nc = i1 - i0 + 1, ncell = nc > 0 && j1 >= j0 ? nc * (j1 - j0 + 1) : 0;
        double s = 0.0, a[NC];
#pragma unroll
        for (int ch = 0; ch < NC; ++ch) a[ch] = 0.0;
        for (int c = lane; c < ncell; c += 32) {
            const int j = j0 + c / nc, i = i0 + c % nc;
            const double area = aai_pair_area(kp.shape, cx, cy, i, j, kp.quirk != 0);
            if (area != 0.0) {
                int sx, sy;
                mod_to_src(kp, i, j, sx, sy);
                const char *row = (const char *)kp.src + (int64_t)(sy - src_row0(kp)) * kp.src_pitch;
                s += area;
#pragma unroll
                for (int ch = 0; ch < NC; ++ch) a[ch] += SrcLoad<TI>::get(row, sx * NC + ch) * area;
            }
        }
#pragma unroll
        for (int off = 16; off > 0; off >>= 1) {
            s += __shfl_xor_sync(FULL, s, off);
#pragma unroll
            for (int ch = 0; ch < NC; ++ch) a[ch] += __shfl_xor_sync(FULL, a[ch], off);
        }
        if (lane == src_lane) {
            sumA = s;
#pragma unroll
            for (int ch = 0; ch < NC; ++ch) acc[ch] = a[ch];
        }
    }
}

}

#endif
```

area_average_interpolation_b200/csrc/aai_internal.h:

```cpp
#ifndef AAI_INTERNAL_H_
#define AAI_INTERNAL_H_

#include <cstdint>
#include <vector>

#include "../../include/aai.h"
#include "aai_cell.cuh"

#ifndef AAI_TILE_W
#define AAI_TILE_W 16
#endif
#ifndef AAI_TILE_H
#define AAI_TILE_H 8
#endif
#define AAI_MAX_ROWS_PER_LAUNCH (65535LL * AAI_TILE_H)

struct AaiKernelParams {
    double side, off_ix, off_iy, iso_x, iso_y, off_x, off_y;
    double aff_x0, aff_xx, aff_xy, aff_y0, aff_yx, aff_yy;
    float ext32;
    AaiShape shape;
    AaiShapeF shapef;
    int32_t f32_ok;
    int32_t quirk;
    int32_t staged;
    int32_t reverse_rows;
    double reach;
    double hb;
    int32_t mod_w, mod_h, dst_w, dst_h;
    int32_t scale, quadrant;
    int32_t e_axi, e_axj, e_ax0, e_ayi, e_ayj, e_ay0;
    uint32_t div_magic;
    const void *src;
    int64_t src_pitch;
    int32_t src_w, src_h, src_y0, src_rows;
    int32_t channels;
    void *dst;
    int64_t dst_pitch;
    int32_t dst_y0, row0, row1;
    int32_t batch;
    int64_t src_batch_stride, dst_batch_stride;
    int32_t src_batch_rows, dst_batch_rows;
};

inline size_t aai_elem_size(int dtype) {
    switch (dtype) {
        case AAI_F64: return 8;
        case AAI_F32: return 4;
        case AAI_U16: return 2;
        case AAI_U8: return 1;
        default: return 0;
    }
}
inline const char *aai_dtype_name(int dtype) {
    switch (dtype) {
        case AAI_F64: return "float64";
        case AAI_F32: return "float32";
        case AAI_U16: return "uint16";
        case AAI_U8: return "uint8";
        default: return "unknown";
    }
}
inline constexpr bool aai_dtype_pair_ok(int src_dtype, int dst_dtype) {
    if (dst_dtype == AAI_U16) return src_dtype == AAI_U16;
    if (src_dtype == AAI_U16) return dst_dtype != AAI_U8;
    return true;
}
int aai_check_dtype_pair(const char *who, int src_dtype, int dst_dtype);

AaiKernelParams aai_make_kernel_params(const aai_plan &plan, const aai_image &src, const aai_image &dst,
                                       int64_t row0, int64_t row1);

int aai_launch_overlap(const AaiKernelParams &kp, int arith, int src_dtype, int dst_dtype, void *stream);
int aai_launch_separable(const AaiKernelParams &kp, int arith, int src_dtype, int dst_dtype, void *stream);
int aai_launch_fast(const AaiKernelParams &kp, int arith, int src_dtype, int dst_dtype, void *stream);
int aai_launch_expand(const AaiKernelParams &kp, int elem_bytes, void *stream);
int aai_probe_fp32(int blocks, int iters, float *scratch, double *flop, void *stream);
int aai_launch_separable_tma(const AaiKernelParams &kp, int arith, int src_dtype, int dst_dtype, void *stream);
int aai_launch_separable_direct_f32(const AaiKernelParams &kp, int src_dtype, int dst_dtype, void *stream);
int aai_launch_overlap_f32_n4(const AaiKernelParams &kp, int src_dtype, int dst_dtype, void *stream);
int aai_launch_overlap_f32_n5(const AaiKernelParams &kp, int src_dtype, int dst_dtype, void *stream);
int aai_launch_overlap_f32_n6(const AaiKernelParams &kp, int src_dtype, int dst_dtype, void *stream);
int aai_launch_overlap_f32_n8(const AaiKernelParams &kp, int src_dtype, int dst_dtype, void *stream);
int aai_launch_fast_f32_n4(const AaiKernelParams &kp, int src_dtype, int dst_dtype, void *stream);
int aai_launch_fast_f32_n5(const AaiKernelParams &kp, int src_dtype, int dst_dtype, void *stream);
int aai_launch_fast_f32_n6(const AaiKernelParams &kp, int src_dtype, int dst_dtype, void *stream);
int aai_launch_fast_f32_n8(const AaiKernelParams &kp, int src_dtype, int dst_dtype, void *stream);
int aai_launch_fast_bin(const AaiKernelParams &kp, int src_dtype, int dst_dtype, void *stream);
int aai_launch_overlap_f64_n4(const AaiKernelParams &kp, int src_dtype, int dst_dtype, void *stream);
int aai_launch_overlap_f64_n5(const AaiKernelParams &kp, int src_dtype, int dst_dtype, void *stream);
int aai_launch_overlap_f64_n6(const AaiKernelParams &kp, int src_dtype, int dst_dtype, void *stream);
int aai_launch_overlap_f64_n8(const AaiKernelParams &kp, int src_dtype, int dst_dtype, void *stream);

struct AaiAdjointParams {
    AaiKernelParams kp;
    double *rcp;
    double inv_side;
    const void *canvas;
    int64_t canvas_pitch, canvas_stride;
    void *out;
    int64_t out_pitch, out_stride;
    int32_t row0, row1;
};
int aai_launch_adjoint_norm(const AaiAdjointParams &ap, int mode, int axis_aligned, void *stream);
int aai_launch_adjoint_gather(const AaiAdjointParams &ap, int mode, int axis_aligned, int dtype, int n_images,
                              void *stream);

void aai_set_error(const char *fmt, ...);
void aai_count_extra_launches(int n);

#endif
```

area_average_interpolation_b200/csrc/aai_kernels.cu:

```cuda
#include <cuda_runtime.h>

#include <cfloat>
#include <cstdint>
#include <cstdlib>

#include "aai_device.cuh"

using namespace aai_dev;

namespace {

template <typename TI, typename TO, int NC>
__global__ void __launch_bounds__(TILE_W *TILE_H)
    overlap_kernel_f64(const __grid_constant__ AaiKernelParams kp) {
    const int x = blockIdx.x * TILE_W + threadIdx.x;
    const int y = kp.row0 + blockIdx.y * TILE_H + threadIdx.y;
    if (x >= kp.dst_w || y >= kp.row1) return;
    double cx, cy;
    pixel_centre(kp, x, y, cx, cy);
    int ix0, ix1, jy0, jy1;
    cell_range(kp, cx, cy, ix0, ix1, jy0, jy1);
    double sumA, acc[NC];
    pixel_f64<TI, NC>(kp, cx, cy, ix0, ix1, jy0, jy1, sumA, acc);
    char *drow = (char *)kp.dst + (int64_t)(y - dst_row0(kp)) * kp.dst_pitch;
    const bool ok = DBL_EPSILON < fabs(sumA);
#pragma unroll
    for (int ch = 0; ch < NC; ++ch) store_dst<TO>(drow, x * NC + ch, ok ? acc[ch] / sumA : 0.0);
}

template <typename TI, typename TO, int NC>
__global__ void __launch_bounds__(TILE_W *TILE_H)
    separable_kernel_f64(const __grid_constant__ AaiKernelParams kp) {
    const int x = blockIdx.x * TILE_W + threadIdx.x;
    const int y = kp.row0 + blockIdx.y * TILE_H + threadIdx.y;
    if (x >= kp.dst_w || y >= kp.row1) return;
    double cx, cy;
    pixel_centre(kp, x, y, cx, cy);
    int wx0, wx1, wy0, wy1;
    search_window(kp, cx, cy, wx0, wx1, wy0, wy1);
    const double ext = kp.shape.half + 0.5 + 1e-9;
    const int ix0 = max(wx0, __double2int_ru(cx - ext)), ix1 = min(wx1, __double2int_rd(cx + ext));
    const int jy0 = max(wy0, __double2int_ru(cy - ext)), jy1 = min(wy1, __double2int_rd(cy + ext));
    const double xl = cx - kp.shape.half, xr = cx + kp.shape.half, yt = cy - kp.shape.half, yb = cy + kp.shape.half;
    double sumA = 0.0;
    double acc[NC];
#pragma unroll
    for (int ch = 0; ch < NC; ++ch) acc[ch] = 0.0;
    for (int j = jy0; j <= jy1; ++j) {
        const double wy = fmax(fmin(yb, (double)j + 0.5) - fmax(yt, (double)j - 0.5), 0.0);
        for (int i = ix0; i <= ix1; ++i) {
            const double wx = fmax(fmin(xr, (double)i + 0.5) - fmax(xl, (double)i - 0.5), 0.0);
            const double area = wx * wy;
            if (area != 0.0) {
                int sx, sy;
                mod_to_src(kp, i, j, sx, sy);
                const char *row = (const char *)kp.src + (int64_t)(sy - src_row0(kp)) * kp.src_pitch;
                sumA += area;
#pragma unroll
                for (int ch = 0; ch < NC; ++ch) acc[ch] += SrcLoad<TI>::get(row, sx * NC + ch) * area;
            }
        }
    }
    char *drow = (char *)kp.dst + (int64_t)(y - dst_row0(kp)) * kp.dst_pitch;
    const bool ok = DBL_EPSILON < fabs(sumA);
#pragma unroll
    for (int ch = 0; ch < NC; ++ch) store_dst<TO>(drow, x * NC + ch, ok ? acc[ch] / sumA : 0.0);
}

template <typename TI, typename TO, int NC>
__global__ void __launch_bounds__(TILE_W *TILE_H) fast_kernel(const __grid_constant__ AaiKernelParams kp) {
    const int x = blockIdx.x * TILE_W + threadIdx.x;
    const int y = kp.row0 + blockIdx.y * TILE_H + threadIdx.y;
    if (x >= kp.dst_w || y >= kp.row1) return;
    int count;
    double acc[NC];
    pixel_fast_f64<TI, NC>(kp, x, y, count, acc);
    char *drow = (char *)kp.dst + (int64_t)(y - dst_row0(kp)) * kp.dst_pitch;
#pragma unroll
    for (int ch = 0; ch < NC; ++ch) store_dst<TO>(drow, x * NC + ch, count > 0 ? acc[ch] / (double)count : 0.0);
}

template <typename TI, typename TO, int NC>
__global__ void __launch_bounds__(TILE_W *TILE_H) fast_kernel_f32(const __grid_constant__ AaiKernelParams kp) {
    const int x = blockIdx.x * TILE_W + threadIdx.x;
    const int y = kp.row0 + blockIdx.y * TILE_H + threadIdx.y;
    if (x >= kp.dst_w || y >= kp.row1) return;
    const double cx = fma((double)x, kp.aff_xx, fma((double)y, kp.aff_xy, kp.aff_x0));
    const double cy = fma((double)x, kp.aff_yx, fma((double)y, kp.aff_yy, kp.aff_y0));
    const int irx = __double2int_rn(cx), iry = __double2int_rn(cy);
    const float fx = (float)(cx - (double)irx), fy = (float)(cy - (double)iry);
    const float ext = kp.shapef.hb + 4e-6f;
    const int ix0 = max(0, irx + __float2int_ru(fx - ext)), ix1 = min(kp.mod_w - 1, irx + __float2int_rd(fx + ext));
    const int jy0 = max(0, iry + __float2int_ru(fy - ext)), jy1 = min(kp.mod_h - 1, iry + __float2int_rd(fy + ext));
    const AaiShapeF &g = kp.shapef;
    const float tau = 4e-6f;
    float count = 0.0f, acc[NC], worst = 1.0f;
#pragma unroll
    for (int ch = 0; ch < NC; ++ch) acc[ch] = 0.0f;
    const bool ident = kp.scale == 1 && kp.quadrant == 0;
    constexpr int ESZ = (int)sizeof(TI) * NC;
    const float rx0 = (float)(ix0 - irx) - fx;
    for (int j = jy0; j <= jy1; ++j) {
        const float ry = (float)(j - iry) - fy;
        const float ur = -ry * g.sn, vr = ry * g.cs;
        const char *rowp = (const char *)kp.src + (int64_t)(j - src_row0(kp)) * kp.src_pitch + (int64_t)ix0 * ESZ;
        float rx = rx0;
        for (int i = ix0; i <= ix1; ++i, rx += 1.0f, rowp += ESZ) {
            const float mu = g.half - fabsf(fmaf(rx, g.cs, ur));
            const float mv = g.half - fabsf(fmaf(rx, g.sn, vr));
            if (mv > -tau) worst = fminf(worst, fabsf(mu));
            if (mu > -tau) worst = fminf(worst, fabsf(mv));
            if (mu >= 0.0f && mv >= 0.0f) {
                const char *p = rowp;
                if (!ident) {
                    int sx, sy;
                    mod_to_src(kp, i, j, sx, sy);
                    p = (const char *)kp.src + (int64_t)(sy - src_row0(kp)) * kp.src_pitch + (int64_t)sx * ESZ;
                }
                count += 1.0f;
#pragma unroll
                for (int ch = 0; ch < NC; ++ch) acc[ch] += LoadF<TI>::get(p + ch * (int)sizeof(TI));
            }
        }
    }
    char *drow = (char *)kp.dst + (int64_t)(y - dst_row0(kp)) * kp.dst_pitch;
    if (worst < tau) {
        int c64;
        double a64[NC];
        pixel_fast_f64<TI, NC>(kp, x, y, c64, a64);
#pragma unroll
        for (int ch = 0; ch < NC; ++ch) store_dst<TO>(drow, x * NC + ch, c64 > 0 ? a64[ch] / (double)c64 : 0.0);
    } else {
        const float inv = count > 0.0f ? 1.0f / count : 0.0f;
#pragma unroll
        for (int ch = 0; ch < NC; ++ch) store_dst<TO>(drow, x * NC + ch, (double)(acc[ch] * inv));
    }
}

template <typename T>
__global__ void __launch_bounds__(256) expand_kernel(const __grid_constant__ AaiKernelParams kp) {
    const int mx = blockIdx.x * 64 + (threadIdx.x & 63);
    const int my = kp.row0 + blockIdx.y * 4 + (threadIdx.x >> 6);
    if (mx >= kp.mod_w || my >= kp.mod_h) return;
    int sx, sy;
    mod_to_src(kp, mx, my, sx, sy);
    const T *srow = (const T *)((const char *)kp.src + (int64_t)(sy - kp.src_y0) * kp.src_pitch);
    T *drow = (T *)((char *)kp.dst + (int64_t)my * kp.dst_pitch);
    for (int ch = 0; ch < kp.channels; ++ch) drow[mx * kp.channels + ch] = srow[sx * kp.channels + ch];
}

__global__ void __launch_bounds__(256) fp32_peak_kernel(float *out, int iters, float a, float b) {
    float v[16];
#pragma unroll
    for (int k = 0; k < 16; ++k) v[k] = (float)(threadIdx.x + k);
    for (int it = 0; it < iters; ++it) {
#pragma unroll
        for (int k = 0; k < 16; ++k) v[k] = fmaf(v[k], a, b);
    }
    float sum = 0.0f;
#pragma unroll
    for (int k = 0; k < 16; ++k) sum += v[k];
    if (sum == 123.456f) out[0] = sum;
}

enum KernelKind { K_OVERLAP, K_SEPARABLE, K_FAST, K_FAST_F32 };

template <typename TI, typename TO, int NC>
cudaError_t launch_typed(KernelKind kind, const AaiKernelParams &kp, cudaStream_t stream) {
    const int rows = kp.row1 - kp.row0;
    if (rows <= 0 || kp.dst_w <= 0) return cudaSuccess;
    dim3 block(TILE_W, TILE_H);
    dim3 grid((kp.dst_w + TILE_W - 1) / TILE_W, (rows + TILE_H - 1) / TILE_H, kp.batch > 1 ? kp.batch : 1);
    switch (kind) {
        case K_OVERLAP: overlap_kernel_f64<TI, TO, NC><<<grid, block, 0, stream>>>(kp); break;
        case K_SEPARABLE: separable_kernel_f64<TI, TO, NC><<<grid, block, 0, stream>>>(kp); break;
        case K_FAST: fast_kernel<TI, TO, NC><<<grid, block, 0, stream>>>(kp); break;
        case K_FAST_F32: fast_kernel_f32<TI, TO, NC><<<grid, block, 0, stream>>>(kp); break;
    }
    return cudaGetLastError();
}

template <typename TI, typename TO>
cudaError_t launch_channels(KernelKind kind, const AaiKernelParams &kp, cudaStream_t stream) {
    switch (kp.channels) {
        case 1: return launch_typed<TI, TO, 1>(kind, kp, stream);
        case 2: return launch_typed<TI, TO, 2>(kind, kp, stream);
        case 3: return launch_typed<TI, TO, 3>(kind, kp, stream);
        case 4: return launch_typed<TI, TO, 4>(kind, kp, stream);
        default: return cudaErrorInvalidValue;
    }
}

template <typename TI>
cudaError_t launch_dst(KernelKind kind, const AaiKernelParams &kp, int dst_dtype, cudaStream_t stream) {
    switch (dst_dtype) {
        case AAI_F64: return launch_channels<TI, double>(kind, kp, stream);
        case AAI_F32: return launch_channels<TI, float>(kind, kp, stream);
        case AAI_U8: if constexpr (pair_ok<TI, uint8_t>()) return launch_channels<TI, uint8_t>(kind, kp, stream); break;
        case AAI_U16: if constexpr (pair_ok<TI, uint16_t>()) return launch_channels<TI, uint16_t>(kind, kp, stream); break;
    }
    return cudaErrorInvalidValue;
}

cudaError_t launch_any(KernelKind kind, const AaiKernelParams &kp, int src_dtype, int dst_dtype, cudaStream_t stream) {
    switch (src_dtype) {
        case AAI_F64: return launch_dst<double>(kind, kp, dst_dtype, stream);
        case AAI_F32: return launch_dst<float>(kind, kp, dst_dtype, stream);
        case AAI_U8: return launch_dst<uint8_t>(kind, kp, dst_dtype, stream);
        case AAI_U16: return launch_dst<uint16_t>(kind, kp, dst_dtype, stream);
        default: return cudaErrorInvalidValue;
    }
}

}

int aai_launch_overlap(const AaiKernelParams &kp, int arith, int src_dtype, int dst_dtype, void *stream) {
    if (arith == AAI_ARITH_F32 && kp.f32_ok && (kp.channels == 1 || kp.channels == 3)) {
        const int n = (int)floor(2.0 * (double)kp.ext32 + 1e-6) + 1;
        if (n <= 4) return aai_launch_overlap_f32_n4(kp, src_dtype, dst_dtype, stream);
        if (n <= 5) return aai_launch_overlap_f32_n5(kp, src_dtype, dst_dtype, stream);
        if (n <= 6) return aai_launch_overlap_f32_n6(kp, src_dtype, dst_dtype, stream);
        if (n <= 8) return aai_launch_overlap_f32_n8(kp, src_dtype, dst_dtype, stream);
    }
    const uint64_t max_e = (uint64_t)(kp.mod_w > kp.mod_h ? kp.mod_w : kp.mod_h);
    bool unrolled = kp.shape.sn > 0.0 && kp.shape.cs > 0.0 && max_e * (uint64_t)kp.scale < 0x100000000ULL;
#ifdef AAI_DEV_KNOBS
    if (getenv("AAI_F64_ROLLED")) unrolled = false;
#endif
    if (unrolled) {
        const int n = (int)floor(2.0 * kp.hb + 1.0 + 2e-9) + 1;
        int e = (int)cudaErrorNotSupported;
        if (n <= 4) e = aai_launch_overlap_f64_n4(kp, src_dtype, dst_dtype, stream);
        else if (n <= 5) e = aai_launch_overlap_f64_n5(kp, src_dtype, dst_dtype, stream);
        else if (n <= 6) e = aai_launch_overlap_f64_n6(kp, src_dtype, dst_dtype, stream);
        else if (n <= 8) e = aai_launch_overlap_f64_n8(kp, src_dtype, dst_dtype, stream);
        if (e != (int)cudaErrorNotSupported) return e;
    }
    return (int)launch_any(K_OVERLAP, kp, src_dtype, dst_dtype, (cudaStream_t)stream);
}
int aai_probe_fp32(int blocks, int iters, float *scratch, double *flop, void *stream) {
    fp32_peak_kernel<<<blocks, 256, 0, (cudaStream_t)stream>>>(scratch, iters, 0.999f, 0.001f);
    *flop = (double)blocks * 256.0 * 16.0 * 2.0 * (double)iters;
    return (int)cudaGetLastError();
}
int aai_launch_separable(const AaiKernelParams &kp, int arith, int src_dtype, int dst_dtype, void *stream) {
    int e = aai_launch_separable_tma(kp, arith, src_dtype, dst_dtype, stream);
    if (e != (int)cudaErrorNotSupported) return e;
    if (arith == AAI_ARITH_F32) {
        e = aai_launch_separable_direct_f32(kp, src_dtype, dst_dtype, stream);
        if (e != (int)cudaErrorNotSupported) return e;
    }
    return (int)launch_any(K_SEPARABLE, kp, src_dtype, dst_dtype, (cudaStream_t)stream);
}
int aai_launch_expand(const AaiKernelParams &kp, int elem_bytes, void *stream) {
    if (kp.mod_w <= 0 || kp.mod_h <= 0) return (int)cudaSuccess;
    cudaStream_t st = (cudaStream_t)stream;
    AaiKernelParams k = kp;
    constexpr int kSlab = 65535 * 4;
    for (int r0 = 0; r0 < kp.mod_h; r0 += kSlab) {
        const int rows = kp.mod_h - r0 < kSlab ? kp.mod_h - r0 : kSlab;
        const dim3 grid((kp.mod_w + 63) / 64, (rows + 3) / 4);
        k.row0 = r0;
        switch (elem_bytes) {
            case 1: expand_kernel<uint8_t><<<grid, 256, 0, st>>>(k); break;
            case 2: expand_kernel<uint16_t><<<grid, 256, 0, st>>>(k); break;
            case 4: expand_kernel<float><<<grid, 256, 0, st>>>(k); break;
            case 8: expand_kernel<double><<<grid, 256, 0, st>>>(k); break;
            default: return (int)cudaErrorInvalidValue;
        }
        const cudaError_t e = cudaGetLastError();
        if (e != cudaSuccess) return (int)e;
    }
    return (int)cudaSuccess;
}

int aai_launch_fast(const AaiKernelParams &kp, int arith, int src_dtype, int dst_dtype, void *stream) {
    const uint64_t max_e = (uint64_t)(kp.mod_w > kp.mod_h ? kp.mod_w : kp.mod_h);
    const bool f32 = arith == AAI_ARITH_F32 && src_dtype != AAI_F64 && dst_dtype != AAI_F64 && max_e < (1u << 30);
    if (f32 && kp.staged == 2) {
        const int e = aai_launch_fast_bin(kp, src_dtype, dst_dtype, stream);
        if (e != (int)cudaErrorNotSupported) return e;
    }
    if (f32 && (kp.channels == 1 || kp.channels == 3) && max_e * (uint64_t)kp.scale < 0x100000000ULL) {
        const int nf = (int)floor(2.0 * ((double)kp.shapef.hb + 4e-6) + 1e-6) + 1;
        if (nf <= 3) return aai_launch_fast_f32_n4(kp, src_dtype, dst_dtype, stream);
        if (nf <= 4) return aai_launch_fast_f32_n5(kp, src_dtype, dst_dtype, stream);
        if (nf <= 5) return aai_launch_fast_f32_n6(kp, src_dtype, dst_dtype, stream);
        if (nf <= 7) return aai_launch_fast_f32_n8(kp, src_dtype, dst_dtype, stream);
    }
    return (int)launch_any(f32 ? K_FAST_F32 : K_FAST, kp, src_dtype, dst_dtype, (cudaStream_t)stream);
}
```

area_average_interpolation_b200/csrc/aai_kernels_f32.cu:

```cuda
#include <cuda.h>

#include <algorithm>
#include <cmath>

#include "aai_device.cuh"

#ifndef AAI_MAXN
#error "compile with -DAAI_MAXN=4|5|6|8"
#endif

using namespace aai_dev;

namespace {

constexpr int MAXN = AAI_MAXN;
#ifndef AAI_ROW_UNROLL
#define AAI_ROW_UNROLL 1
#endif
constexpr int kRowUnroll = AAI_ROW_UNROLL;
#ifndef AAI_MINC
#define AAI_MINC (AAI_MAXN == 8 ? 6 : AAI_MAXN == 4 ? 2 : AAI_MAXN - 1)
#endif
constexpr int MINC = AAI_MINC;


struct StageParams {
    int bw, bh;
};

__device__ __forceinline__ uint32_t st_smem_u32(const void *p) { return (uint32_t)__cvta_generic_to_shared(p); }

template <int EB, int NC>
__device__ __forceinline__ void stage_window(const CUtensorMap *tmap, const AaiKernelParams &kp, const StageParams &sp,
                                             unsigned char *smem, uint64_t *bar, int *origin, float ext, int &sox,
                                             int &soy) {
    const int tid = threadIdx.y * TILE_W + threadIdx.x;
    if (tid == 0) {
        const int x0 = blockIdx.x * TILE_W, y0 = kp.row0 + blockIdx.y * TILE_H;
        double lox = 1e300, loy = 1e300;
#pragma unroll
        for (int c = 0; c < 4; ++c) {
            const double xx = (double)(x0 + (c & 1) * (TILE_W - 1)), yy = (double)(y0 + (c >> 1) * (TILE_H - 1));
            lox = fmin(lox, fma(xx, kp.aff_xx, fma(yy, kp.aff_xy, kp.aff_x0)));
            loy = fmin(loy, fma(xx, kp.aff_yx, fma(yy, kp.aff_yy, kp.aff_y0)));
        }
        constexpr int EAL = 16 / EB;
        int ex = (__double2int_rd(lox - (double)ext) - 1) * NC;
        ex = (ex >= 0 ? ex / EAL : -((-ex + EAL - 1) / EAL)) * EAL;
        const int ey = __double2int_rd(loy - (double)ext) - 1;
        origin[0] = ex;
        origin[1] = ey;
        asm volatile("mbarrier.init.shared::cta.b64 [%0], %1;" ::"r"(st_smem_u32(bar)), "r"(1));
        asm volatile("fence.mbarrier_init.release.cluster;" ::: "memory");
        const uint32_t bytes = (uint32_t)(sp.bw * sp.bh * EB);
        asm volatile("mbarrier.arrive.expect_tx.shared::cta.b64 _, [%0], %1;" ::"r"(st_smem_u32(bar)), "r"(bytes) : "memory");
        asm volatile(
            "cp.async.bulk.tensor.2d.shared::cluster.global.mbarrier::complete_tx::bytes [%0], [%1, {%3, %4}], [%2];" ::
                "r"(st_smem_u32(smem)),
            "l"(tmap), "r"(st_smem_u32(bar)), "r"(ex), "r"(ey - src_row0(kp))
            : "memory");
    }
    __syncthreads();
    sox = origin[0];
    soy = origin[1];
    asm volatile(
        "{\n"
        ".reg .pred p;\n"
        "ST_WAIT:\n"
        "mbarrier.try_wait.parity.shared::cta.b64 p, [%0], %1;\n"
        "@p bra.uni ST_DONE;\n"
        "bra.uni ST_WAIT;\n"
        "ST_DONE:\n"
        "}\n" ::"r"(st_smem_u32(bar)),
        "r"(0)
        : "memory");
}

template <typename TI, bool STAGED>
struct LoadS {
    static __device__ __forceinline__ float get(const char *p) {
        if constexpr (STAGED)
            return to_arith<float>(*reinterpret_cast<const TI *>(p));
        else
            return LoadF<TI>::get(p);
    }
};

typedef CUresult (*StEncodeTiledFn)(CUtensorMap *, CUtensorMapDataType, cuuint32_t, void *, const cuuint64_t *,
                                    const cuuint64_t *, const cuuint32_t *, const cuuint32_t *, CUtensorMapInterleave,
                                    CUtensorMapSwizzle, CUtensorMapL2promotion, CUtensorMapFloatOOBfill);
StEncodeTiledFn st_encode_fn() {
    static const StEncodeTiledFn fn = [] {
        void *p = nullptr;
        cudaDriverEntryPointQueryResult q;
        if (cudaGetDriverEntryPoint("cuTensorMapEncodeTiled", &p, cudaEnableDefault, &q) == cudaSuccess &&
            q == cudaDriverEntryPointSuccess)
            return (StEncodeTiledFn)p;
        cudaGetLastError();
        return (StEncodeTiledFn) nullptr;
    }();
    return fn;
}

struct StageHost {
    CUtensorMap map;
    StageParams sp;
    size_t smem;
};
template <typename TI, int NC>
bool stage_prepare(const AaiKernelParams &kp, double ext, StageHost &h) {
    StEncodeTiledFn enc = st_encode_fn();
    if (!enc || kp.scale != 1 || kp.quadrant != 0 || sizeof(TI) == 8) return false;
    if ((kp.src_pitch % 16) != 0 || (reinterpret_cast<uintptr_t>(kp.src) % 16) != 0) return false;
    constexpr int EB = (int)sizeof(TI), EAL = 16 / EB;
    const double sx = (TILE_W - 1) * std::fabs(kp.aff_xx) + (TILE_H - 1) * std::fabs(kp.aff_xy);
    const double sy = (TILE_W - 1) * std::fabs(kp.aff_yx) + (TILE_H - 1) * std::fabs(kp.aff_yy);
    const int wpx = (int)std::ceil(sx + 2.0 * ext) + 4;
    h.sp.bw = (wpx * NC + (EAL - 1) + EAL - 1) / EAL * EAL;
    h.sp.bh = (int)std::ceil(sy + 2.0 * ext) + 4;
    h.smem = (size_t)h.sp.bw * h.sp.bh * EB;
    if (h.sp.bw > 256 || h.sp.bh > 256 || h.smem > 30 * 1024) return false;
    const int64_t rows = kp.batch > 1 ? (int64_t)kp.src_batch_rows * kp.batch : (int64_t)kp.src_rows;
    const cuuint64_t gdim[2] = {(cuuint64_t)kp.src_w * NC, (cuuint64_t)rows};
    const cuuint64_t gstride[1] = {(cuuint64_t)kp.src_pitch};
    const cuuint32_t box[2] = {(cuuint32_t)h.sp.bw, (cuuint32_t)h.sp.bh};
    const cuuint32_t estr[2] = {1, 1};
    return enc(&h.map, Elem<TI>::tmap, 2, const_cast<void *>(kp.src), gdim, gstride, box, estr, CU_TENSOR_MAP_INTERLEAVE_NONE,
               CU_TENSOR_MAP_SWIZZLE_NONE, CU_TENSOR_MAP_L2_PROMOTION_L2_128B,
               CU_TENSOR_MAP_FLOAT_OOB_FILL_NONE) == CUDA_SUCCESS;
}


#ifndef AAI_F32_MIN_BLOCKS
#define AAI_F32_MIN_BLOCKS ((AAI_MAXN <= 4 ? 896 : AAI_MAXN == 5 ? 768 : 512) / (AAI_TILE_W * AAI_TILE_H))
#endif
enum { ADDR_GENERAL = 0, ADDR_IDENT = 1, ADDR_GROUPED = 2 };
template <typename TI, typename TO, int NC, int ADDR, bool STAGED, bool PDL = false, bool REV = false>
__device__ __forceinline__ void overlap_body(const AaiKernelParams &kp, const char *stage, int spitch, int sox, int soy) {
    constexpr bool IDENT = ADDR == ADDR_IDENT, GROUPED = ADDR == ADDR_GROUPED;
    static_assert(!STAGED || IDENT, "staging is implemented for identity addressing");
    if constexpr (PDL) asm volatile("griddepcontrol.launch_dependents;");
    const int x = blockIdx.x * TILE_W + threadIdx.x;
    const int by = REV ? (int)gridDim.y - 1 - (int)blockIdx.y : (int)blockIdx.y;
    const int y = kp.row0 + by * TILE_H + threadIdx.y;
    const bool valid = x < kp.dst_w && y < kp.row1;
    const double cx = fma((double)x, kp.aff_xx, fma((double)y, kp.aff_xy, kp.aff_x0));
    const double cy = fma((double)x, kp.aff_yx, fma((double)y, kp.aff_yy, kp.aff_y0));
    const int irx = __double2int_rn(cx), iry = __double2int_rn(cy);
    const float fx = (float)(cx - (double)irx), fy = (float)(cy - (double)iry);
    const int bx0 = irx + __float2int_ru(fx - kp.ext32), bx1 = irx + __float2int_rd(fx + kp.ext32);
    const int by0 = iry + __float2int_ru(fy - kp.ext32), by1 = iry + __float2int_rd(fy + kp.ext32);
    const int ix0 = max(0, bx0), ix1 = min(kp.mod_w - 1, bx1), jy0 = max(0, by0), jy1 = min(kp.mod_h - 1, by1);
    const bool border = bx0 < 0 || by0 < 0 || bx1 > kp.mod_w - 1 || by1 > kp.mod_h - 1;
    const int ncols = ix1 - ix0 + 1, nrows = jy1 - jy0 + 1;
    char *drow = (char *)kp.dst + (int64_t)(y - dst_row0(kp)) * kp.dst_pitch;
    const bool work = valid && ncols > 0 && nrows > 0;
    if constexpr (PDL) asm volatile("griddepcontrol.wait;" ::: "memory");
    if (valid && !work) {
#pragma unroll
        for (int ch = 0; ch < NC; ++ch) store_f<TO>(drow, x * NC + ch, 0.0f);
    }
    float sumA = 0.0f, acc[NC];
#pragma unroll
    for (int ch = 0; ch < NC; ++ch) acc[ch] = 0.0f;
    float worst = 1.0f;
    bool redo = work && (border || ncols > MAXN || nrows > MAXN || ncols < MINC);
    if (work && !redo) {
        const AaiShapeF &g = kp.shapef;
        const int dj0 = jy0 - iry;
        const float rx0 = (float)(ix0 - irx) - fx;
        float yt[MAXN + 1], yb[MAXN + 1];
        if (!GROUPED) {
#pragma unroll
            for (int k = 0; k + 1 <= MAXN; k += 2) {
                AaiF2 t2, b2;
                aai_chord_v_f32x2(g, aai_f2(rx0 + ((float)k - 0.5f), rx0 + ((float)k + 0.5f)), t2, b2);
                yt[k] = t2.x;
                yt[k + 1] = t2.y;
                yb[k] = b2.x;
                yb[k + 1] = b2.y;
            }
            if ((MAXN + 1) & 1) aai_chord_v_f32(g, rx0 + ((float)MAXN - 0.5f), yt[MAXN], yb[MAXN]);
        }
        float xlT = 0.0f, xrT = 0.0f;
        const float t0 = ((float)dj0 - fy) - 0.5f;
        if (!GROUPED) aai_chord_h_f32(g, t0, xlT, xrT);
        const float e0 = rx0 - 0.5f;
        constexpr int ESZ = (int)sizeof(TI) * NC;
        const int64_t pitch = STAGED ? (int64_t)spitch : kp.src_pitch;
        const char *rowp0 = STAGED ? stage + (jy0 - soy) * spitch + (ix0 * NC - sox) * (int)sizeof(TI)
                                   : (const char *)kp.src + (int64_t)(jy0 - src_row0(kp)) * kp.src_pitch + (int64_t)ix0 * ESZ;
        const char *rowp = rowp0;
        const bool swapped = kp.e_axi == 0;
        auto div_s = [&](int e) -> int64_t {
            return (int64_t)(kp.scale != 1 ? __umulhi((unsigned)e, kp.div_magic) : (unsigned)e);
        };
        auto col_off = [&](int i) -> int64_t {
            return swapped ? (div_s(kp.e_ayi * i + kp.e_ay0) - src_row0(kp)) * kp.src_pitch
                           : div_s(kp.e_axi * i + kp.e_ax0) * ESZ;
        };
        auto row_off = [&](int j) -> int64_t {
            return swapped ? div_s(kp.e_axj * j + kp.e_ax0) * ESZ
                           : (div_s(kp.e_ayj * j + kp.e_ay0) - src_row0(kp)) * kp.src_pitch;
        };
        int64_t coff[MAXN];
        if (!IDENT && !GROUPED) {
#pragma unroll
            for (int k = 0; k < MAXN; ++k) coff[k] = col_off(ix0 + min(k, ncols - 1));
        }
        int nA = MAXN, nT = MAXN;
        float W00 = 0.0f, W01 = 0.0f, W10 = 0.0f, W11 = 0.0f;
        if (GROUPED) {
            auto first_group = [&](int e, int step) -> int {
                const int rem = e - (int)div_s(e) * kp.scale;
                return step > 0 ? kp.scale - rem : rem + 1;
            };
            const int ac = swapped ? kp.e_ayi : kp.e_axi, ec0 = swapped ? kp.e_ay0 : kp.e_ax0;
            const int ar = swapped ? kp.e_axj : kp.e_ayj, er0 = swapped ? kp.e_ax0 : kp.e_ay0;
            nA = first_group(ac * ix0 + ec0, ac);
            nT = first_group(ar * jy0 + er0, ar);
            aai_quadrant_areas_f32(g, e0 + (float)nA, t0 + (float)nT, nA < ncols, nT < nrows, W00, W01, W10, W11);
        }
        float lenTop[MAXN];
        if (!GROUPED) {
#pragma unroll
            for (int k = 0; k < MAXN; ++k) lenTop[k] = aai_overlap1_f32(xlT, xrT, e0 + (float)k);
        }
        constexpr bool PREFETCH = NC == 1 && !GROUPED;
        float buf[MAXN][NC];
        auto fetch = [&](int r, float (&v)[MAXN][NC]) {
            if (IDENT)
                rowp = rowp0 + (int64_t)r * pitch;
            else
                rowp = (const char *)kp.src + row_off(jy0 + r);
#pragma unroll
            for (int k = 0; k < MAXN; ++k) {
#pragma unroll
                for (int ch = 0; ch < NC; ++ch) v[k][ch] = 0.0f;
                if (k < MINC || k < ncols) {
                    const char *p = IDENT ? rowp + k * ESZ : rowp + coff[k];
#pragma unroll
                    for (int ch = 0; ch < NC; ++ch) v[k][ch] = LoadS<TI, STAGED>::get(p + ch * (int)sizeof(TI));
                }
            }
        };
        if (PREFETCH) fetch(0, buf);
        auto row = [&](int r, float (&cur)[MAXN][NC], float (&nxt)[MAXN][NC]) {
            if (PREFETCH) {
                if (r + 1 < nrows) fetch(r + 1, nxt);
            } else {
                rowp = IDENT ? rowp0 + (int64_t)r * pitch : (const char *)kp.src + row_off(jy0 + r);
            }
            const float ry = (float)(dj0 + r) - fy;
            float xlB, xrB;
            aai_chord_h_f32(g, ry + 0.5f, xlB, xrB);
            const float ey = ry - 0.5f;
            float lenL = aai_overlap1_f32(yt[0], yb[0], ey);
            const float ur = -ry * g.sn, vr = ry * g.cs;
            auto take = [&](int k, float area) {
                if (PREFETCH) {
#pragma unroll
                    for (int ch = 0; ch < NC; ++ch) acc[ch] = fmaf(cur[k][ch], area, acc[ch]);
                } else if (k < MINC || k < ncols) {
                    const char *p = IDENT ? rowp + k * ESZ : rowp + coff[k];
#pragma unroll
                    for (int ch = 0; ch < NC; ++ch)
                        acc[ch] = fmaf(LoadS<TI, STAGED>::get(p + ch * (int)sizeof(TI)), area, acc[ch]);
                }
            };
#pragma unroll
            for (int k = 0; k + 1 < MAXN; k += 2) {
                const float rxa = rx0 + (float)k, rxb = rx0 + (float)(k + 1);
                const float exa = rxa - 0.5f, exb = rxb - 0.5f;
                const AaiF2 lMR = aai_sub2(aai_f2(aai_sat(yb[k + 1] - ey), aai_sat(yb[k + 2] - ey)),
                                           aai_f2(aai_sat(yt[k + 1] - ey), aai_sat(yt[k + 2] - ey)));
                const float lenM = lMR.x, lenR = lMR.y;
                const AaiF2 lT = aai_f2(lenTop[k], lenTop[k + 1]);
                const AaiF2 lB = aai_sub2(aai_f2(aai_sat(xrB - exa), aai_sat(xrB - exb)),
                                          aai_f2(aai_sat(xlB - exa), aai_sat(xlB - exb)));
                lenTop[k] = lB.x;
                lenTop[k + 1] = lB.y;
                const AaiF2 rx2 = aai_f2(rxa, rxb);
                const AaiF2 u0 = aai_fma2(rx2, aai_f2(g.cs), aai_f2(ur)), v0 = aai_fma2(rx2, aai_f2(g.sn), aai_f2(vr));
                const AaiF2 area = aai_cell_exact_f32x2(g, u0, v0, lT, lB, aai_f2(lenL, lenM), aai_f2(lenM, lenR));
                lenL = lenR;
                take(k, area.x);
                take(k + 1, area.y);
            }
            if (MAXN & 1) {
                constexpr int k = MAXN - 1;
                const float rx = rx0 + (float)k;
                const float ex = rx - 0.5f;
                const float lenR = aai_overlap1_f32(yt[k + 1], yb[k + 1], ey);
                const float lenT = lenTop[k];
                const float lenB = aai_overlap1_f32(xlB, xrB, ex);
                lenTop[k] = lenB;
                const float u0 = fmaf(rx, g.cs, ur), v0 = fmaf(rx, g.sn, vr);
                const float area = aai_cell_exact_f32(g, u0, v0, lenT, lenB, lenL, lenR);
                take(k, area);
            }
        };
        if (!GROUPED) {
#pragma unroll kRowUnroll
            for (int r = 0; r < nrows; ++r) {
                float nxt[MAXN][NC];
                row(r, buf, nxt);
                if (PREFETCH) {
#pragma unroll
                    for (int k = 0; k < MAXN; ++k)
#pragma unroll
                        for (int ch = 0; ch < NC; ++ch) buf[k][ch] = nxt[k][ch];
                }
            }
        }
        sumA = g.area_total;
        if (kp.quirk) {
            const float g0m = g.steep ? e0 : t0, g0M = g.steep ? t0 : e0;
            const int64_t minor_stride = IDENT ? (g.steep ? (int64_t)ESZ : pitch) : 0;
            auto fix2 = [&](int mi, int Mi, float d_before, float d_after) {
                const int mlim = (g.steep ? ncols : nrows) - 2, Mlim = (g.steep ? nrows : ncols) - 1;
                mi = max(0, min(mi, mlim));
                Mi = max(0, min(Mi, Mlim));
                const int k = g.steep ? mi : Mi, r = g.steep ? Mi : mi;
                if (GROUPED) {
                    const int k1 = k + (g.steep ? 1 : 0), r1 = r + (g.steep ? 0 : 1);
                    const float both = d_before + d_after;
                    if (g.steep) {
                        const float dA = (k < nA ? d_before : 0.0f) + (k1 < nA ? d_after : 0.0f), dB = both - dA;
                        const bool top = r < nT;
                        W00 += top ? dA : 0.0f;
                        W01 += top ? dB : 0.0f;
                        W10 += top ? 0.0f : dA;
                        W11 += top ? 0.0f : dB;
                    } else {
                        const float dT = (r < nT ? d_before : 0.0f) + (r1 < nT ? d_after : 0.0f), dBt = both - dT;
                        const bool left = k < nA;
                        W00 += left ? dT : 0.0f;
                        W10 += left ? dBt : 0.0f;
                        W01 += left ? 0.0f : dT;
                        W11 += left ? 0.0f : dBt;
                    }
                    sumA += both;
                    return;
                }
                const char *p0, *p1;
                if (IDENT) {
                    p0 = rowp0 + (int64_t)r * pitch + (int64_t)k * ESZ;
                    p1 = p0 + minor_stride;
                } else {
                    p0 = (const char *)kp.src + row_off(jy0 + r) + col_off(ix0 + k);
                    p1 = (const char *)kp.src + row_off(jy0 + r + (g.steep ? 0 : 1)) + col_off(ix0 + k + (g.steep ? 1 : 0));
                }
                sumA += d_before + d_after;
#pragma unroll
                for (int ch = 0; ch < NC; ++ch) {
                    acc[ch] = fmaf(LoadS<TI, STAGED>::get(p0 + ch * (int)sizeof(TI)), d_before, acc[ch]);
                    acc[ch] = fmaf(LoadS<TI, STAGED>::get(p1 + ch * (int)sizeof(TI)), d_after, acc[ch]);
                }
            };
            for (int q = 0; q < g.ncross; ++q) {
                int mi[2], Mi[2];
                float db[2], da[2];
                aai_edge_quirk_pair_f32(g, g0m, g0M, q, mi, Mi, db, da, worst);
                fix2(mi[0], Mi[0], db[0], da[0]);
                fix2(mi[1], Mi[1], db[1], da[1]);
            }

        }
        if (GROUPED) {
            const int64_t roff0 = row_off(jy0), roffL = row_off(jy1), coff0 = col_off(ix0), coffL = col_off(ix1);
            const char *base = (const char *)kp.src;
            const char *p00 = base + roff0 + coff0, *p01 = base + roff0 + coffL;
            const char *p10 = base + roffL + coff0, *p11 = base + roffL + coffL;
#pragma unroll
            for (int ch = 0; ch < NC; ++ch) {
                const int o = ch * (int)sizeof(TI);
                acc[ch] = fmaf(LoadS<TI, STAGED>::get(p00 + o), W00,
                               fmaf(LoadS<TI, STAGED>::get(p01 + o), W01,
                                    fmaf(LoadS<TI, STAGED>::get(p10 + o), W10, LoadS<TI, STAGED>::get(p11 + o) * W11)));
            }
        }
        redo = worst < g.tau || sumA < 0.25f;
    }
    double s64 = 0.0, a64[NC];
    if (__any_sync(0xffffffffu, redo)) warp_pixels_f64<TI, NC>(kp, redo, x, y, s64, a64);
    if (redo) {
        const bool ok = DBL_EPSILON < fabs(s64);
#pragma unroll
        for (int ch = 0; ch < NC; ++ch) store_dst<TO>(drow, x * NC + ch, ok ? a64[ch] / s64 : 0.0);
    } else if (work) {
        const float inv = 1.0f / sumA;
#pragma unroll
        for (int ch = 0; ch < NC; ++ch) store_f<TO>(drow, x * NC + ch, acc[ch] * inv);
    }
}

template <typename TI, typename TO, int NC, int ADDR, bool PDL = false, bool REV = false>
__global__ void __launch_bounds__(TILE_W *TILE_H, AAI_F32_MIN_BLOCKS)
    overlap_kernel_f32(const __grid_constant__ AaiKernelParams kp) {
    overlap_body<TI, TO, NC, ADDR, false, PDL, REV>(kp, nullptr, 0, 0, 0);
}
#ifndef AAI_PDL
#define AAI_PDL 1
#endif
constexpr long long kPdlMaxCtas = 150000;
template <typename TI, typename TO, int NC>
cudaError_t launch_short_pdl(const AaiKernelParams &kp, dim3 grid, dim3 block, cudaStream_t stream) {
    cudaLaunchConfig_t cfg = {};
    cfg.gridDim = grid;
    cfg.blockDim = block;
    cfg.dynamicSmemBytes = 0;
    cfg.stream = stream;
    cudaLaunchAttribute attr[1];
    attr[0].id = cudaLaunchAttributeProgrammaticStreamSerialization;
    attr[0].val.programmaticStreamSerializationAllowed = 1;
    cfg.attrs = attr;
    cfg.numAttrs = 1;
    if (kp.reverse_rows) return cudaLaunchKernelEx(&cfg, overlap_kernel_f32<TI, TO, NC, ADDR_IDENT, true, true>, kp);
    return cudaLaunchKernelEx(&cfg, overlap_kernel_f32<TI, TO, NC, ADDR_IDENT, true, false>, kp);
}

template <typename TI, typename TO, int NC>
__global__ void __launch_bounds__(TILE_W *TILE_H, AAI_F32_MIN_BLOCKS)
    overlap_kernel_f32_tma(const __grid_constant__ CUtensorMap tmap, const __grid_constant__ AaiKernelParams kp,
                           const StageParams sp) {
    extern __shared__ __align__(128) unsigned char stage_raw[];
    __shared__ uint64_t bar;
    __shared__ int origin[2];
    int sox, soy;
    stage_window<(int)sizeof(TI), NC>(&tmap, kp, sp, stage_raw, &bar, origin, kp.ext32, sox, soy);
    overlap_body<TI, TO, NC, ADDR_IDENT, true>(kp, (const char *)stage_raw, sp.bw * (int)sizeof(TI), sox, soy);
}

template <typename TI, typename TO, int NC>
cudaError_t launch3(const AaiKernelParams &kp, cudaStream_t stream) {
    const int rows = kp.row1 - kp.row0;
    if (rows <= 0 || kp.dst_w <= 0) return cudaSuccess;
    dim3 block(TILE_W, TILE_H);
    dim3 grid((kp.dst_w + TILE_W - 1) / TILE_W, (rows + TILE_H - 1) / TILE_H, kp.batch > 1 ? kp.batch : 1);
    if (kp.scale == 1 && kp.quadrant == 0) {
        StageHost h;
        if (kp.staged == 1 && stage_prepare<TI, NC>(kp, (double)kp.ext32, h)) {
            overlap_kernel_f32_tma<TI, TO, NC><<<grid, block, h.smem, stream>>>(h.map, kp, h.sp);
            return cudaGetLastError();
        }
        if (AAI_PDL && (long long)grid.x * grid.y * grid.z <= kPdlMaxCtas) return launch_short_pdl<TI, TO, NC>(kp, grid, block, stream);
        overlap_kernel_f32<TI, TO, NC, ADDR_IDENT><<<grid, block, 0, stream>>>(kp);
    } else if (MAXN == 4 && kp.scale >= MAXN - 1)
        overlap_kernel_f32<TI, TO, NC, (MAXN == 4 ? ADDR_GROUPED : ADDR_GENERAL)><<<grid, block, 0, stream>>>(kp);
    else
        overlap_kernel_f32<TI, TO, NC, ADDR_GENERAL><<<grid, block, 0, stream>>>(kp);
    return cudaGetLastError();
}
template <typename TI, typename TO>
cudaError_t launch2(const AaiKernelParams &kp, cudaStream_t stream) {
    return kp.channels == 1 ? launch3<TI, TO, 1>(kp, stream) : launch3<TI, TO, 3>(kp, stream);
}
template <typename TI>
cudaError_t launch1(const AaiKernelParams &kp, int dst_dtype, cudaStream_t stream) {
    switch (dst_dtype) {
        case AAI_F64: return launch2<TI, double>(kp, stream);
        case AAI_F32: return launch2<TI, float>(kp, stream);
        case AAI_U8: if constexpr (pair_ok<TI, uint8_t>()) return launch2<TI, uint8_t>(kp, stream); break;
        case AAI_U16: if constexpr (pair_ok<TI, uint16_t>()) return launch2<TI, uint16_t>(kp, stream); break;
    }
    return cudaErrorInvalidValue;
}


constexpr int NF = MAXN - 1;
#ifndef AAI_FAST_VEC_LOADS
#define AAI_FAST_VEC_LOADS 1
#endif
#ifndef AAI_FAST_PRED_LOADS
#define AAI_FAST_PRED_LOADS 1
#endif
#ifndef AAI_FAST_SKIP_LOADS
#define AAI_FAST_SKIP_LOADS 1
#endif
template <typename TI, typename TO, int NC, bool IDENT, bool STAGED, bool VEC = false>
__device__ __forceinline__ void fast_body(const AaiKernelParams &kp, const char *stage, int spitch, int sox, int soy,
                                          int tile_x, int tile_y) {
    static_assert(!STAGED || IDENT, "staging is implemented for identity addressing");
    static_assert(!VEC || (IDENT && !STAGED && NC == 1 && sizeof(TI) == 4), "vector loads: float, 1 channel, identity");
    constexpr int NV = (NF + 3 + 3) / 4;
    const int x = tile_x * TILE_W + threadIdx.x;
    const int y = kp.row0 + tile_y * TILE_H + threadIdx.y;
    if (x >= kp.dst_w || y >= kp.row1) return;
    const double cx = fma((double)x, kp.aff_xx, fma((double)y, kp.aff_xy, kp.aff_x0));
    const double cy = fma((double)x, kp.aff_yx, fma((double)y, kp.aff_yy, kp.aff_y0));
    const int irx = __double2int_rn(cx), iry = __double2int_rn(cy);
    const float fx = (float)(cx - (double)irx), fy = (float)(cy - (double)iry);
    const AaiShapeF &g = kp.shapef;
    constexpr float tau = 4e-6f;
    const float ext = g.hb + tau;
    const int bx0 = irx + __float2int_ru(fx - ext), bx1 = irx + __float2int_rd(fx + ext);
    const int by0 = iry + __float2int_ru(fy - ext), by1 = iry + __float2int_rd(fy + ext);
    char *drow = (char *)kp.dst + (int64_t)(y - dst_row0(kp)) * kp.dst_pitch;
    if (bx1 < 0 || by1 < 0 || bx0 > kp.mod_w - 1 || by0 > kp.mod_h - 1) {
#pragma unroll
        for (int ch = 0; ch < NC; ++ch) store_f<TO>(drow, x * NC + ch, 0.0f);
        return;
    }
    const bool inside_img = bx0 >= 0 && by0 >= 0 && bx0 + NF - 1 <= kp.mod_w - 1 && by0 + NF - 1 <= kp.mod_h - 1 &&
                            bx1 - bx0 < NF && by1 - by0 < NF && (!VEC || (bx0 & ~3) + 4 * NV <= kp.mod_w);
    float count = 0.0f, acc[NC], worst = 1.0f;
#pragma unroll
    for (int ch = 0; ch < NC; ++ch) acc[ch] = 0.0f;
    if (inside_img) {
        constexpr int ESZ = (int)sizeof(TI) * NC;
        const bool swapped = kp.e_axi == 0;
        auto div_s = [&](int e) -> int64_t {
            return (int64_t)(kp.scale != 1 ? __umulhi((unsigned)e, kp.div_magic) : (unsigned)e);
        };
        int64_t coff[NF], roff[NF];
        if (STAGED) {
#pragma unroll
            for (int k = 0; k < NF; ++k) {
                coff[k] = ((bx0 + k) * NC - sox) * (int)sizeof(TI);
                roff[k] = (by0 + k - soy) * spitch;
            }
        } else if (IDENT) {
#pragma unroll
            for (int k = 0; k < NF; ++k) {
                coff[k] = (int64_t)(bx0 + k) * ESZ;
                roff[k] = (int64_t)(by0 + k - src_row0(kp)) * kp.src_pitch;
            }
        } else {
#pragma unroll
            for (int k = 0; k < NF; ++k) {
                const int i = bx0 + k, j = by0 + k;
                coff[k] = swapped ? (div_s(kp.e_ayi * i + kp.e_ay0) - src_row0(kp)) * kp.src_pitch
                                  : div_s(kp.e_axi * i + kp.e_ax0) * ESZ;
                roff[k] = swapped ? div_s(kp.e_axj * j + kp.e_ax0) * ESZ
                                  : (div_s(kp.e_ayj * j + kp.e_ay0) - src_row0(kp)) * kp.src_pitch;
            }
        }
        const float rx0 = (float)(bx0 - irx) - fx, ry0 = (float)(by0 - iry) - fy;
        if constexpr (VEC) {
            const int o = bx0 & 3;
            const char *rowp = (const char *)kp.src + (int64_t)(by0 - src_row0(kp)) * kp.src_pitch + (int64_t)(bx0 - o) * 4;
            float v[NF][NF];
            const int last_col = o + (bx1 - bx0), last_row = by1 - by0;
#pragma unroll
            for (int r = 0; r < NF; ++r) {
                float w[4 * NV];
#pragma unroll
                for (int q = 0; q < NV; ++q) {
                    const bool need = AAI_FAST_SKIP_LOADS ? (r <= last_row && 4 * q <= last_col) : true;
                    const float4 t = need ? __ldg(reinterpret_cast<const float4 *>(rowp) + q) : make_float4(0.f, 0.f, 0.f, 0.f);
                    w[4 * q] = t.x;
                    w[4 * q + 1] = t.y;
                    w[4 * q + 2] = t.z;
                    w[4 * q + 3] = t.w;
                }
                rowp += kp.src_pitch;
                float t1[NF + 2];
#pragma unroll
                for (int i = 0; i < NF + 2; ++i) t1[i] = (o & 1) ? w[i + 1] : w[i];
#pragma unroll
                for (int k = 0; k < NF; ++k) v[r][k] = (o & 2) ? t1[k + 2] : t1[k];
            }
#pragma unroll
            for (int r = 0; r < NF; ++r) {
                const float ry = ry0 + (float)r;
                const float2 uvr = make_float2(-ry * g.sn, ry * g.cs), cssn = make_float2(g.cs, g.sn);
#pragma unroll
                for (int k = 0; k < NF; ++k) {
                    const float rx = rx0 + (float)k;
                    const float2 uv = __ffma2_rn(make_float2(rx, rx), cssn, uvr);
                    const float m = g.half - fmaxf(fabsf(uv.x), fabsf(uv.y));
                    worst = fminf(worst, fabsf(m));
                    if (m >= 0.0f) {
                        count += 1.0f;
                        acc[0] += v[r][k];
                    }
                }
            }
        } else
        if constexpr (AAI_FAST_PRED_LOADS && NC > 1) {
        float mm[NF][NF];
#pragma unroll
        for (int r = 0; r < NF; ++r) {
            const float ry = ry0 + (float)r;
            const float ur = -ry * g.sn, vr = ry * g.cs;
#pragma unroll
            for (int k = 0; k < NF; ++k) {
                const float rx = rx0 + (float)k;
                const float mu = g.half - fabsf(fmaf(rx, g.cs, ur));
                const float mv = g.half - fabsf(fmaf(rx, g.sn, vr));
                const float m = fminf(mu, mv);
                worst = fminf(worst, fabsf(m));
                mm[r][k] = m;
            }
        }
#pragma unroll
        for (int r = 0; r < NF; ++r) {
            const char *rowp = (STAGED ? stage : (const char *)kp.src) + roff[r];
#pragma unroll
            for (int k = 0; k < NF; ++k) {
                if (mm[r][k] >= 0.0f) {
                    count += 1.0f;
#pragma unroll
                    for (int ch = 0; ch < NC; ++ch)
                        acc[ch] += LoadS<TI, STAGED>::get(rowp + coff[k] + ch * (int)sizeof(TI));
                }
            }
        }
        } else {
#pragma unroll
        for (int r = 0; r < NF; ++r) {
            float v[NF][NC];
            const char *rowp = (STAGED ? stage : (const char *)kp.src) + roff[r];
#pragma unroll
            for (int k = 0; k < NF; ++k)
#pragma unroll
                for (int ch = 0; ch < NC; ++ch) v[k][ch] = LoadS<TI, STAGED>::get(rowp + coff[k] + ch * (int)sizeof(TI));
            const float ry = ry0 + (float)r;
            const float ur = -ry * g.sn, vr = ry * g.cs;
#pragma unroll
            for (int k = 0; k < NF; ++k) {
                const float rx = rx0 + (float)k;
                const float mu = g.half - fabsf(fmaf(rx, g.cs, ur));
                const float mv = g.half - fabsf(fmaf(rx, g.sn, vr));
                const float m = fminf(mu, mv);
                worst = fminf(worst, fabsf(m));
                if (m >= 0.0f) {
                    count += 1.0f;
#pragma unroll
                    for (int ch = 0; ch < NC; ++ch) acc[ch] += v[k][ch];
                }
            }
        }
        }
    }
    if (!inside_img || worst < tau) {
        int c64;
        double a64[NC];
        pixel_fast_f64<TI, NC>(kp, x, y, c64, a64);
#pragma unroll
        for (int ch = 0; ch < NC; ++ch) store_dst<TO>(drow, x * NC + ch, c64 > 0 ? a64[ch] / (double)c64 : 0.0);
    } else {
        const float inv = count > 0.0f ? 1.0f / count : 0.0f;
#pragma unroll
        for (int ch = 0; ch < NC; ++ch) store_f<TO>(drow, x * NC + ch, acc[ch] * inv);
    }
}

template <typename TI, typename TO, int NC, bool IDENT>
__global__ void __launch_bounds__(TILE_W *TILE_H, 1024 / (TILE_W * TILE_H))
    fast_kernel_f32u(const __grid_constant__ AaiKernelParams kp) {
    fast_body<TI, TO, NC, IDENT, false>(kp, nullptr, 0, 0, 0, blockIdx.x, blockIdx.y);
}
template <typename TO>
__global__ void __launch_bounds__(TILE_W *TILE_H, 1024 / (TILE_W * TILE_H))
    fast_kernel_f32u_vec(const __grid_constant__ AaiKernelParams kp) {
    fast_body<float, TO, 1, true, false, true>(kp, nullptr, 0, 0, 0, blockIdx.x, blockIdx.y);
}

template <typename TI, typename TO, int NC>
__global__ void __launch_bounds__(TILE_W *TILE_H, 1024 / (TILE_W * TILE_H))
    fast_kernel_f32u_tma(const __grid_constant__ CUtensorMap tmap, const __grid_constant__ AaiKernelParams kp,
                         const StageParams sp) {
    extern __shared__ __align__(128) unsigned char stage_raw[];
    __shared__ uint64_t bar;
    __shared__ int origin[2];
    int sox, soy;
    stage_window<(int)sizeof(TI), NC>(&tmap, kp, sp, stage_raw, &bar, origin, kp.shapef.hb + 4e-6f, sox, soy);
    fast_body<TI, TO, NC, true, true>(kp, (const char *)stage_raw, sp.bw * (int)sizeof(TI), sox, soy, blockIdx.x, blockIdx.y);
}

constexpr int RING_STAGES = 2;
template <typename TI, typename TO, int NC>
__global__ void __launch_bounds__(TILE_W *TILE_H, 1024 / (TILE_W * TILE_H))
    fast_kernel_f32u_ring(const __grid_constant__ CUtensorMap tmap, const __grid_constant__ AaiKernelParams kp,
                          const StageParams sp, const int tiles_x, const int ntiles) {
    extern __shared__ __align__(128) unsigned char stage_raw[];
    __shared__ uint64_t full[RING_STAGES];
    __shared__ int origin[RING_STAGES][2];
    constexpr int EB = (int)sizeof(TI), EAL = 16 / EB;
    const int tid = threadIdx.y * TILE_W + threadIdx.x;
    const uint32_t stage_bytes = (uint32_t)(sp.bw * sp.bh * EB);
    const uint32_t stage_stride = (stage_bytes + 127u) & ~127u;
    const float ext = kp.shapef.hb + 4e-6f;
    auto issue = [&](int t, int s) {
        const int ty = t / tiles_x, tx = t - ty * tiles_x;
        const int x0 = tx * TILE_W, y0 = kp.row0 + ty * TILE_H;
        double lox = 1e300, loy = 1e300;
#pragma unroll
        for (int c = 0; c < 4; ++c) {
            const double xx = (double)(x0 + (c & 1) * (TILE_W - 1)), yy = (double)(y0 + (c >> 1) * (TILE_H - 1));
            lox = fmin(lox, fma(xx, kp.aff_xx, fma(yy, kp.aff_xy, kp.aff_x0)));
            loy = fmin(loy, fma(xx, kp.aff_yx, fma(yy, kp.aff_yy, kp.aff_y0)));
        }
        int ex = (__double2int_rd(lox - (double)ext) - 1) * NC;
        ex = (ex >= 0 ? ex / EAL : -((-ex + EAL - 1) / EAL)) * EAL;
        const int ey = __double2int_rd(loy - (double)ext) - 1;
        origin[s][0] = ex;
        origin[s][1] = ey;
        asm volatile("mbarrier.arrive.expect_tx.shared::cta.b64 _, [%0], %1;" ::"r"(st_smem_u32(&full[s])), "r"(stage_bytes)
                     : "memory");
        asm volatile(
            "cp.async.bulk.tensor.2d.shared::cluster.global.mbarrier::complete_tx::bytes [%0], [%1, {%3, %4}], [%2];" ::
                "r"(st_smem_u32(stage_raw + (size_t)s * stage_stride)),
            "l"(&tmap), "r"(st_smem_u32(&full[s])), "r"(ex), "r"(ey - src_row0(kp))
            : "memory");
    };
    if (tid == 0) {
#pragma unroll
        for (int s = 0; s < RING_STAGES; ++s)
            asm volatile("mbarrier.init.shared::cta.b64 [%0], %1;" ::"r"(st_smem_u32(&full[s])), "r"(1));
        asm volatile("fence.mbarrier_init.release.cluster;" ::: "memory");
        if ((int)blockIdx.x < ntiles) issue((int)blockIdx.x, 0);
    }
    int k = 0;
    for (int t = (int)blockIdx.x; t < ntiles; t += (int)gridDim.x, ++k) {
        const int s = k & 1;
        __syncthreads();
        if (tid == 0 && t + (int)gridDim.x < ntiles) issue(t + (int)gridDim.x, s ^ 1);
        asm volatile(
            "{\n"
            ".reg .pred p;\n"
            "RG_WAIT:\n"
            "mbarrier.try_wait.parity.shared::cta.b64 p, [%0], %1;\n"
            "@p bra.uni RG_DONE;\n"
            "bra.uni RG_WAIT;\n"
            "RG_DONE:\n"
            "}\n" ::"r"(st_smem_u32(&full[s])),
            "r"((k >> 1) & 1)
            : "memory");
        const int ty = t / tiles_x, tx = t - ty * tiles_x;
        fast_body<TI, TO, NC, true, true>(kp, (const char *)stage_raw + (size_t)s * stage_stride, sp.bw * EB, origin[s][0],
                                          origin[s][1], tx, ty);
    }
}

template <typename TI, typename TO, int NC>
cudaError_t launch_fast3(const AaiKernelParams &kp, cudaStream_t stream) {
    const int rows = kp.row1 - kp.row0;
    if (rows <= 0 || kp.dst_w <= 0) return cudaSuccess;
    dim3 block(TILE_W, TILE_H);
    dim3 grid((kp.dst_w + TILE_W - 1) / TILE_W, (rows + TILE_H - 1) / TILE_H, kp.batch > 1 ? kp.batch : 1);
    if (kp.scale == 1 && kp.quadrant == 0) {
        StageHost h;
        if ((kp.staged == 1 || kp.staged == 3) && stage_prepare<TI, NC>(kp, (double)kp.shapef.hb + 1e-5, h)) {
            if (kp.staged == 3) {
                int dev = 0, sms = 0;
                cudaGetDevice(&dev);
                cudaDeviceGetAttribute(&sms, cudaDevAttrMultiProcessorCount, dev);
                const int tiles_x = (int)grid.x, ntiles = (int)(grid.x * grid.y);
                const size_t smem = RING_STAGES * ((h.smem + 127) & ~(size_t)127);
                const int per_sm = 1024 / (TILE_W * TILE_H);
                const dim3 pgrid((unsigned)std::min(ntiles, sms * per_sm), 1, grid.z);
                static thread_local int attr_dev = -1;
                if (attr_dev != dev) {
                    const cudaError_t e = cudaFuncSetAttribute(fast_kernel_f32u_ring<TI, TO, NC>,
                                                               cudaFuncAttributeMaxDynamicSharedMemorySize, 64 * 1024);
                    if (e != cudaSuccess) return e;
                    attr_dev = dev;
                }
                fast_kernel_f32u_ring<TI, TO, NC><<<pgrid, block, smem, stream>>>(h.map, kp, h.sp, tiles_x, ntiles);
                return cudaGetLastError();
            }
            fast_kernel_f32u_tma<TI, TO, NC><<<grid, block, h.smem, stream>>>(h.map, kp, h.sp);
            return cudaGetLastError();
        }
        if constexpr (sizeof(TI) == 4 && NC == 1) {
            if ((kp.src_pitch % 16) == 0 && (reinterpret_cast<uintptr_t>(kp.src) % 16) == 0 && AAI_FAST_VEC_LOADS) {
                fast_kernel_f32u_vec<TO><<<grid, block, 0, stream>>>(kp);
                return cudaGetLastError();
            }
        }
        fast_kernel_f32u<TI, TO, NC, true><<<grid, block, 0, stream>>>(kp);
    } else {
        fast_kernel_f32u<TI, TO, NC, false><<<grid, block, 0, stream>>>(kp);
    }
    return cudaGetLastError();
}
template <typename TI>
cudaError_t launch_fast1(const AaiKernelParams &kp, int dst_dtype, cudaStream_t stream) {
    const bool one = kp.channels == 1;
    switch (dst_dtype) {
        case AAI_F32: return one ? launch_fast3<TI, float, 1>(kp, stream) : launch_fast3<TI, float, 3>(kp, stream);
        case AAI_U8:
            if constexpr (pair_ok<TI, uint8_t>())
                return one ? launch_fast3<TI, uint8_t, 1>(kp, stream) : launch_fast3<TI, uint8_t, 3>(kp, stream);
            break;
        case AAI_U16:
            if constexpr (pair_ok<TI, uint16_t>())
                return one ? launch_fast3<TI, uint16_t, 1>(kp, stream) : launch_fast3<TI, uint16_t, 3>(kp, stream);
            break;
    }
    return cudaErrorInvalidValue;
}

}

#define AAI_CAT2(a, b) a##b
#define AAI_CAT(a, b) AAI_CAT2(a, b)

int AAI_CAT(aai_launch_overlap_f32_n, AAI_MAXN)(const AaiKernelParams &kp, int src_dtype, int dst_dtype, void *stream) {
    cudaStream_t st = (cudaStream_t)stream;
    switch (src_dtype) {
        case AAI_F64: return (int)launch1<double>(kp, dst_dtype, st);
        case AAI_F32: return (int)launch1<float>(kp, dst_dtype, st);
        case AAI_U8: return (int)launch1<uint8_t>(kp, dst_dtype, st);
        case AAI_U16: return (int)launch1<uint16_t>(kp, dst_dtype, st);
        default: return (int)cudaErrorInvalidValue;
    }
}

int AAI_CAT(aai_launch_fast_f32_n, AAI_MAXN)(const AaiKernelParams &kp, int src_dtype, int dst_dtype, void *stream) {
    cudaStream_t st = (cudaStream_t)stream;
    switch (src_dtype) {
        case AAI_F32: return (int)launch_fast1<float>(kp, dst_dtype, st);
        case AAI_U8: return (int)launch_fast1<uint8_t>(kp, dst_dtype, st);
        case AAI_U16: return (int)launch_fast1<uint16_t>(kp, dst_dtype, st);
        default: return (int)cudaErrorInvalidValue;
    }
}
```

area_average_interpolation_b200/csrc/aai_plan.cpp:

```cpp
#include <cfloat>
#include <cmath>
#include <cstring>

#include "aai_internal.h"

namespace {

inline void centre_of(const aai_plan &p, double x, double y, double &cx, double &cy) {
    const double u = (x + p.off_ix) * p.side - p.iso_x + p.off_x;
    const double v = (y + p.off_iy) * p.side - p.iso_y + p.off_y;
    cx = u * p.cos_t + v * p.sin_t + p.iso_x;
    cy = -u * p.sin_t + v * p.cos_t + p.iso_y;
}

inline void covered_span(const aai_plan &p, int64_t y, int64_t &xa, int64_t &xb) {
    const double m = p.reach + 2.0;
    double c0x, c0y;
    centre_of(p, 0.0, (double)y, c0x, c0y);
    const double dxx = p.side * p.cos_t, dxy = -p.side * p.sin_t;
    double lo = 0.0, hi = (double)p.dst_w;
    auto clip = [&](double c0, double d, double cmin, double cmax) {
        if (std::fabs(d) < 1e-300) {
            if (c0 < cmin || c0 > cmax) hi = lo;
            return;
        }
        double t0 = (cmin - c0) / d, t1 = (cmax - c0) / d;
        if (t0 > t1) {
            double t = t0;
            t0 = t1;
            t1 = t;
        }
        if (t0 > lo) lo = t0;
        if (t1 + 1.0 < hi) hi = t1 + 1.0;
    };
    clip(c0x, dxx, -m, (double)(p.mod_w - 1) + m);
    clip(c0y, dxy, -m, (double)(p.mod_h - 1) + m);
    if (!(hi > lo)) {
        xa = xb = 0;
        return;
    }
    xa = (int64_t)std::floor(lo);
    xb = (int64_t)std::ceil(hi);
    if (xa < 0) xa = 0;
    if (xb > p.dst_w) xb = p.dst_w;
    if (xb < xa) xb = xa;
}

}

extern "C" {

const char *aai_status_string(int status) {
    switch (status) {
        case AAI_OK: return "";
        case AAI_ERR_RESOLUTION_XY: return "Assumed X & Y resolution are same.";
        case AAI_ERR_RESOLUTION_NONPOS: return "0 or negative resolution is not acceptable.";
        case AAI_ERR_NO_ROWS: return "There is no data in src array.";
        case AAI_ERR_NO_COLUMNS: return "There is no data in the second dimension of src array.";
        case AAI_ERR_ANGLE: return "Rotation angle is not a finite number.";
        case AAI_ERR_ARGUMENT: return "Invalid argument.";
        case AAI_ERR_CUDA: return "CUDA failure.";
        case AAI_ERR_NO_DEVICE: return "No usable CUDA device (this library has no CPU fallback).";
        default: return "Unknown status.";
    }
}

int aai_plan_create(int64_t src_w, int64_t src_h, double src_res_x, double src_res_y, double dst_res_x,
                    double dst_res_y, double src_iso_x, double src_iso_y, double angle_deg, aai_plan *plan) {
    if (!plan) return AAI_ERR_ARGUMENT;
    std::memset(plan, 0, sizeof *plan);
    aai_plan &p = *plan;
    if (DBL_EPSILON < std::fabs(src_res_x - src_res_y) || DBL_EPSILON < std::fabs(dst_res_x - dst_res_y))
        return p.status = AAI_ERR_RESOLUTION_XY;
    if (src_res_x <= DBL_EPSILON || dst_res_x <= DBL_EPSILON) return p.status = AAI_ERR_RESOLUTION_NONPOS;
    if (src_h <= 0) return p.status = AAI_ERR_NO_ROWS;
    if (src_w <= 0) return p.status = AAI_ERR_NO_COLUMNS;
    if (!std::isfinite(angle_deg)) return p.status = AAI_ERR_ANGLE;
    if (!std::isfinite(src_res_x) || !std::isfinite(dst_res_x) || !std::isfinite(src_iso_x) ||
        !std::isfinite(src_iso_y))
        return p.status = AAI_ERR_ARGUMENT;

    const double scale_real = dst_res_x / src_res_x * std::sqrt(2) + 1 + DBL_EPSILON;
    if (!(scale_real < 65536.0)) return p.status = AAI_ERR_ARGUMENT;
    p.scale = static_cast<unsigned int>(scale_real);
    double angle = angle_deg;
    if (std::fabs(angle) > 1e9) angle = std::fmod(angle, 360.0);
    while (angle < 0) angle += 360;
    while (360 <= angle) angle -= 360;
    if (angle < 90) {
        p.quadrant = 0;
    } else if (angle < 180) {
        p.quadrant = 1;
        angle -= 90;
    } else if (angle < 270) {
        p.quadrant = 2;
        angle -= 180;
    } else {
        p.quadrant = 3;
        angle -= 270;
    }
    p.theta_deg = angle;
    p.sin_t = std::sin(angle / 180.0 * M_PI);
    p.cos_t = std::cos(angle / 180.0 * M_PI);

    p.src_w = src_w;
    p.src_h = src_h;
    const int64_t ew = src_w * (int64_t)p.scale, eh = src_h * (int64_t)p.scale;
    if (ew > 0x7fffffffLL || eh > 0x7fffffffLL) return p.status = AAI_ERR_ARGUMENT;
    const bool swapped = (p.quadrant == 1 || p.quadrant == 3);
    const unsigned mw = (unsigned)(swapped ? eh : ew), mh = (unsigned)(swapped ? ew : eh);
    p.mod_w = mw;
    p.mod_h = mh;

    p.iso_x = src_iso_x * p.scale + (p.scale - 1) / 2.0;
    p.iso_y = src_iso_y * p.scale + (p.scale - 1) / 2.0;
    const double src_res = src_res_x * p.scale;
    p.ratio = dst_res_x / src_res;
    p.side = src_res / dst_res_x;
    const double wreal = std::round((mw * std::fabs(p.cos_t) + mh * std::fabs(p.sin_t)) * p.ratio);
    const double hreal = std::round((mw * std::fabs(p.sin_t) + mh * std::fabs(p.cos_t)) * p.ratio);
    if (!(wreal < 2147483647.0) || !(hreal < 2147483647.0)) return p.status = AAI_ERR_ARGUMENT;
    p.dst_w = (unsigned int)wreal;
    p.dst_h = (unsigned int)hreal;
    const double dix = (p.iso_x * p.cos_t + (mh - p.iso_y) * p.sin_t) * p.ratio;
    const double diy = (p.iso_x * p.sin_t + p.iso_y * p.cos_t) * p.ratio;
    if (!(std::fabs(dix) < 2147483647.0) || !(std::fabs(diy) < 2147483647.0)) return p.status = AAI_ERR_ARGUMENT;
    p.off_ix = dix - int(dix);
    p.off_iy = diy - int(diy);
    p.dst_iso_x = (int)dix;
    p.dst_iso_y = (int)diy;
    const double sx = p.iso_x, sy = p.iso_y, c = p.cos_t, s = p.sin_t;
    double ox = 0, oy = 0;
    ox = std::fmin(ox, -sx * c + sy * s + sx);
    oy = std::fmin(oy, -sx * s - sy * c + sy);
    ox = std::fmin(ox, (mw - 1 - sx) * c + sy * s + sx);
    oy = std::fmin(oy, (mw - 1 - sx) * s - sy * c + sy);
    ox = std::fmin(ox, -sx * c - (mh - 1 - sy) * s + sx);
    oy = std::fmin(oy, -sx * s + (mh - 1 - sy) * c + sy);
    ox = std::fmin(ox, (mw - 1 - sx) * c - (mh - 1 - sy) * s + sx);
    oy = std::fmin(oy, (mw - 1 - sx) * s + (mh - 1 - sy) * c + sy);
    p.off_x = ox;
    p.off_y = oy;
    p.reach = p.side * std::sqrt(2) / 2;
    p.axis_aligned = (p.sin_t == 0.0 && p.cos_t == 1.0) ? 1 : 0;
    return p.status = AAI_OK;
}

int64_t aai_covered_pixels(const aai_plan *plan, int64_t row0, int64_t row1) {
    if (!plan || plan->status != AAI_OK) return 0;
    if (row0 < 0) row0 = 0;
    if (row1 > plan->dst_h) row1 = plan->dst_h;
    int64_t total = 0;
    for (int64_t y = row0; y < row1; ++y) {
        int64_t xa, xb;
        covered_span(*plan, y, xa, xb);
        total += xb - xa;
    }
    return total;
}

double aai_band_empty_weight(const aai_plan *plan, int mode, int arith) {
    if (mode == AAI_MODE_FAST) return 0.27;
    if (arith == AAI_ARITH_F64) return 0.06;
    return (plan && plan->scale >= 3) ? 0.20 : 0.17;
}

int aai_partition_rows(const aai_plan *plan, int n_parts, int64_t *bounds) {
    return aai_partition_rows_weighted(plan, n_parts, aai_band_empty_weight(plan, AAI_MODE_AREA_AVERAGE, AAI_ARITH_F32), bounds);
}

int aai_partition_rows_weighted(const aai_plan *plan, int n_parts, double empty_weight, int64_t *bounds) {
    if (!plan || plan->status != AAI_OK || n_parts <= 0 || !bounds || !(empty_weight >= 0.0) || !(empty_weight <= 1.0))
        return AAI_ERR_ARGUMENT;
    const int64_t h = plan->dst_h;
    std::vector<double> prefix((size_t)h + 1, 0.0);
    for (int64_t y = 0; y < h; ++y) {
        int64_t xa, xb;
        covered_span(*plan, y, xa, xb);
        prefix[(size_t)y + 1] = prefix[(size_t)y] + (double)(xb - xa) + empty_weight * (double)(plan->dst_w - (xb - xa)) + 1.0;
    }
    const double total = prefix[(size_t)h];
    bounds[0] = 0;
    int64_t y = 0;
    for (int k = 1; k < n_parts; ++k) {
        const double target = total * (double)k / (double)n_parts;
        while (y < h && prefix[(size_t)y + 1] <= target) ++y;
        int64_t cut = y;
        if (y < h && (target - prefix[(size_t)y]) > (prefix[(size_t)y + 1] - target)) cut = y + 1;
        if (cut < bounds[k - 1]) cut = bounds[k - 1];
        bounds[k] = cut;
    }
    bounds[n_parts] = h;
    return AAI_OK;
}

int aai_band_source_window(const aai_plan *plan, int64_t row0, int64_t row1, int64_t *src_x0, int64_t *src_x1,
                           int64_t *src_y0, int64_t *src_y1) {
    if (!plan || plan->status != AAI_OK) return AAI_ERR_ARGUMENT;
    const aai_plan &p = *plan;
    if (row0 < 0) row0 = 0;
    if (row1 > p.dst_h) row1 = p.dst_h;
    int64_t mx0 = 0, mx1 = 0, my0 = 0, my1 = 0;
    if (row1 > row0 && p.dst_w > 0) {
        double lox = 1e300, hix = -1e300, loy = 1e300, hiy = -1e300;
        const double xs[2] = {0.0, (double)(p.dst_w - 1)}, ys[2] = {(double)row0, (double)(row1 - 1)};
        for (double x : xs)
            for (double y : ys) {
                double cx, cy;
                centre_of(p, x, y, cx, cy);
                lox = std::fmin(lox, cx);
                hix = std::fmax(hix, cx);
                loy = std::fmin(loy, cy);
                hiy = std::fmax(hiy, cy);
            }
        const double m = p.reach + 2.0;
        mx0 = (int64_t)std::floor(std::fmax(lox - m, 0.0));
        my0 = (int64_t)std::floor(std::fmax(loy - m, 0.0));
        mx1 = (int64_t)std::fmin(std::ceil(hix + m) + 1.0, (double)p.mod_w);
        my1 = (int64_t)std::fmin(std::ceil(hiy + m) + 1.0, (double)p.mod_h);
        if (mx1 < mx0) mx1 = mx0;
        if (my1 < my0) my1 = my0;
    }
    int64_t ex0, ex1, ey0, ey1;
    switch (p.quadrant) {
        case 0: ex0 = mx0; ex1 = mx1; ey0 = my0; ey1 = my1; break;
        case 1: ex0 = my0; ex1 = my1; ey0 = p.mod_w - mx1; ey1 = p.mod_w - mx0; break;
        case 2: ex0 = p.mod_w - mx1; ex1 = p.mod_w - mx0; ey0 = p.mod_h - my1; ey1 = p.mod_h - my0; break;
        default: ex0 = p.mod_h - my1; ex1 = p.mod_h - my0; ey0 = mx0; ey1 = mx1; break;
    }
    const int64_t S = (int64_t)p.scale;
    auto lo = [&](int64_t e) { return e / S; };
    auto hi = [&](int64_t e) { return (e + S - 1) / S; };
    int64_t x0 = lo(ex0), x1 = hi(ex1), y0 = lo(ey0), y1 = hi(ey1);
    if (x1 > p.src_w) x1 = p.src_w;
    if (y1 > p.src_h) y1 = p.src_h;
    if (x1 <= x0 || y1 <= y0) x0 = x1 = y0 = y1 = 0;
    if (src_x0) *src_x0 = x0;
    if (src_x1) *src_x1 = x1;
    if (src_y0) *src_y0 = y0;
    if (src_y1) *src_y1 = y1;
    return AAI_OK;
}

}
```

include/aai.h:

```cpp
#ifndef AAI_H_
#define AAI_H_

#include <stddef.h>
#include <stdint.h>

#ifdef __cplusplus
extern "C" {
#endif

#define AAI_VERSION 100

enum {
    AAI_OK = 0,
    AAI_ERR_RESOLUTION_XY = 1,
    AAI_ERR_RESOLUTION_NONPOS = 2,
    AAI_ERR_NO_ROWS = 3,
    AAI_ERR_NO_COLUMNS = 4,
    AAI_ERR_ANGLE = 5,
    AAI_ERR_ARGUMENT = 6,
    AAI_ERR_CUDA = 7,
    AAI_ERR_NO_DEVICE = 8
};

enum { AAI_F64 = 0, AAI_F32 = 1, AAI_U8 = 2, AAI_U16 = 3 };

enum {
    AAI_MODE_AREA_AVERAGE = 1,
    AAI_MODE_FAST = 2,
    AAI_MODE_AREA_AVERAGE_EXACT = 3
};

enum {
    AAI_ARITH_F64 = 0,
    AAI_ARITH_F32 = 1,
    AAI_ARITH_F32_STAGED = 2,
    AAI_ARITH_F32_BINNED = 3,
    AAI_ARITH_F32_RING = 4
};

typedef struct aai_plan {
    int32_t status;
    uint32_t scale;
    int32_t quadrant;
    int32_t axis_aligned;
    int64_t src_w, src_h;
    int64_t mod_w, mod_h;
    int64_t dst_w, dst_h;
    double theta_deg;
    double sin_t, cos_t;
    double iso_x, iso_y;
    double ratio;
    double side;
    double dst_iso_x, dst_iso_y;
    double off_ix, off_iy;
    double off_x, off_y;
    double reach;
} aai_plan;

typedef struct aai_image {
    void *data;
    int64_t pitch_bytes;
    int64_t width, height;
    int64_t y0, rows;
    int32_t dtype;
    int32_t channels;
} aai_image;


int aai_plan_create(int64_t src_w, int64_t src_h, double src_res_x, double src_res_y, double dst_res_x,
                    double dst_res_y, double src_iso_x, double src_iso_y, double angle_deg, aai_plan *plan);

const char *aai_status_string(int status);

const char *aai_last_error(void);


int aai_partition_rows(const aai_plan *plan, int n_parts, int64_t *bounds);
int aai_partition_rows_weighted(const aai_plan *plan, int n_parts, double empty_weight, int64_t *bounds);
double aai_band_empty_weight(const aai_plan *plan, int mode, int arith);

int aai_band_source_window(const aai_plan *plan, int64_t row0, int64_t row1, int64_t *src_x0, int64_t *src_x1,
                           int64_t *src_y0, int64_t *src_y1);

int64_t aai_covered_pixels(const aai_plan *plan, int64_t row0, int64_t row1);


int aai_device_count(void);

int aai_image_alloc(aai_image *img, int device, int64_t width, int64_t height, int64_t y0, int64_t rows,
                    int32_t dtype, int32_t channels);
int aai_image_free(aai_image *img, int device);
int aai_image_upload(const aai_image *device_img, const aai_image *host_img, int device, void *stream);
int aai_image_download(const aai_image *host_img, const aai_image *device_img, int device, void *stream);

int aai_image_copy_rows(const aai_image *dst_device_img, const aai_image *src_device_img, int64_t y0, int64_t y1,
                        int device, void *stream);

#define AAI_IPC_HANDLE_BYTES 64
int aai_ipc_export(const void *device_ptr, unsigned char handle[AAI_IPC_HANDLE_BYTES]);
int aai_ipc_open(const unsigned char handle[AAI_IPC_HANDLE_BYTES], int device, void **device_ptr);
int aai_ipc_close(void *device_ptr, int device);

int aai_expand_device(const aai_plan *plan, const aai_image *src, const aai_image *dst_mod, int device, void *stream);

int aai_measure_fp32_tflops(int device, double *tflops);


int aai_run_device(const aai_plan *plan, int mode, int arith, const aai_image *src, const aai_image *dst,
                   int64_t row0, int64_t row1, int device, void *stream);

int aai_run_device_batch(const aai_plan *plan, int mode, int arith, const aai_image *srcs, const aai_image *dsts,
                         int n_images, int device, void *stream);

int aai_run_device_adjoint(const aai_plan *plan, int mode, const aai_image *canvas_grads, const aai_image *src_grads,
                           int n_images, int device, void *stream);

int aai_run_host(const aai_plan *plan, int mode, int arith, const aai_image *src, const aai_image *dst,
                 const int *devices, int n_devices);

int aai_run_host_band(const aai_plan *plan, int mode, int arith, const aai_image *src, const aai_image *dst,
                      int64_t row0, int64_t row1, int device, void *stream, int synchronize);

int aai_run_host_batch(const aai_plan *plan, int mode, int arith, const aai_image *srcs, const aai_image *dsts,
                       int n_images, int device, void *stream, int synchronize);

typedef struct aai_peer aai_peer;
#define AAI_PEER_BLOB_BYTES 2048
int aai_peer_upload_chunks(int n);
int aai_peer_create(const aai_plan *plan, int32_t dtype, int32_t channels, int rank, int world_size, int device,
                    aai_peer **out);
int aai_peer_export(aai_peer *peer, unsigned char blob[AAI_PEER_BLOB_BYTES]);
int aai_peer_connect(aai_peer *peer, const unsigned char *blobs_of_all_ranks);
int aai_peer_owned_rows(const aai_peer *peer, int64_t *y0, int64_t *y1);
int aai_peer_band(const aai_peer *peer, int64_t *row0, int64_t *row1);
int aai_peer_run(aai_peer *peer, int mode, int arith, const aai_image *host_src, const aai_image *host_dst,
                 void *stream, int synchronize);
int aai_peer_device_source(const aai_peer *peer, aai_image *out);
int aai_peer_last_timing(aai_peer *peer, float ms[4]);
int aai_peer_destroy(aai_peer *peer);

int64_t aai_launch_count(void);

int aai_last_host_timing(float *h2d_ms, float *kernel_ms, float *d2h_ms);

#ifdef __cplusplus
}
#endif
#endif
```

Before: 41580.

## Launch only covered tiles via per-launch tile table, zero empty spans cheaply

Builds a host-side table of which destination tiles per tile-row intersect the rotated source footprint, passes it as a grid-constant kernel argument, and launches a 1-D grid. One block per tile-row zero-fills the uncovered spans with vectorised stores, and the remaining blocks map to covered tiles by binary search over a prefix sum. This is meant to avoid spending full interpolation blocks on output tiles that lie outside the source. In exchange it adds host work to build the table (cached per plan and row range), a large kernel parameter, and a small per-block lookup cost.

```diff
diff --git a/area_average_interpolation_b200/__init__.py b/area_average_interpolation_b200/__init__.py
--- a/area_average_interpolation_b200/__init__.py
+++ b/area_average_interpolation_b200/__init__.py
@@ -204,6 +204,19 @@
     return int(lib().aai_covered_pixels(C.byref(plan), int(row0), int(plan.dst_h if row1 is None else row1)))
 
 
+def covered_tiles(plan: Plan, row0: int = 0, row1: Optional[int] = None, tile_w: int = 16, tile_h: int = 8):
+    row1 = plan.dst_h if row1 is None else int(row1)
+    n = max(0, -(-(row1 - int(row0)) // int(tile_h))) if tile_h > 0 else 0
+    first, count = np.zeros(n, np.int32), np.zeros(n, np.int32)
+    ptr = C.POINTER(C.c_int32)
+    f = lib().aai_covered_tiles
+    f.restype = C.c_int
+    f.argtypes = [C.POINTER(Plan), C.c_int64, C.c_int64, C.c_int32, C.c_int32, ptr, ptr]
+    _check(f(C.byref(plan), int(row0), row1, int(tile_w), int(tile_h), first.ctypes.data_as(ptr),
+             count.ctypes.data_as(ptr)))
+    return first, count
+
+
 def device_count() -> int:
     return int(lib().aai_device_count())
 
@@ -468,7 +481,7 @@
 
 __all__ = [
     "AreaAverageInterpolation", "Result", "Plan", "Image", "AaiError", "make_plan", "partition_rows",
-    "band_source_window", "covered_pixels", "device_count", "launch_count", "last_host_timing", "run_device", "run_device_batch", "run_device_adjoint",
+    "band_source_window", "covered_pixels", "covered_tiles", "device_count", "launch_count", "last_host_timing", "run_device", "run_device_batch", "run_device_adjoint",
     "expand_device", "measure_fp32_tflops", "image_alloc", "image_free", "image_upload", "image_download", "image_copy_rows",
     "ipc_export", "ipc_open", "ipc_close",
     "run_host", "run_host_band", "run_host_batch", "PeerGroup", "tensor_image", "status_string", "last_error", "lib", "LIB_PATH",
diff --git a/area_average_interpolation_b200/csrc/aai_capi.cu b/area_average_interpolation_b200/csrc/aai_capi.cu
--- a/area_average_interpolation_b200/csrc/aai_capi.cu
+++ b/area_average_interpolation_b200/csrc/aai_capi.cu
@@ -169,20 +169,29 @@
     const int32_t row0 = kp.row0, row1 = kp.row1;
     kp.staged = arith == AAI_ARITH_F32_STAGED ? 1 : arith == AAI_ARITH_F32_BINNED ? 2 : arith == AAI_ARITH_F32_RING ? 3 : 0;
     if (kp.staged) arith = AAI_ARITH_F32;
-    for (int64_t a = row0; a < row1; a += AAI_MAX_ROWS_PER_LAUNCH) {
+    const bool tiled = arith == AAI_ARITH_F32 && (mode == AAI_MODE_FAST || !plan.axis_aligned);
+    int64_t per_launch = AAI_MAX_ROWS_PER_LAUNCH;
+    if (tiled) {
+        const int64_t tiles_x = (plan.dst_w + AAI_TILE_W - 1) / AAI_TILE_W, max_cta_rows = 0x7fffffffLL / (tiles_x + 1);
+        per_launch = AAI_MAX_TABLE_ROWS_PER_LAUNCH < max_cta_rows * AAI_TILE_H ? AAI_MAX_TABLE_ROWS_PER_LAUNCH
+                                                                                 : max_cta_rows * AAI_TILE_H;
+    }
+    static const AaiTileTable no_tiles = {};
+    for (int64_t a = row0; a < row1; a += per_launch) {
         kp.row0 = (int32_t)a;
-        kp.row1 = (int32_t)(a + AAI_MAX_ROWS_PER_LAUNCH < row1 ? a + AAI_MAX_ROWS_PER_LAUNCH : row1);
+        kp.row1 = (int32_t)(a + per_launch < row1 ? a + per_launch : row1);
+        const AaiTileTable &tiles = tiled ? aai_tile_table(plan, kp.row0, kp.row1) : no_tiles;
         {
             const int64_t n = kp.row1 - kp.row0, e = n / 8 > 64 ? 64 : (n / 8 > 0 ? n / 8 : 1);
             kp.reverse_rows = aai_covered_pixels(&plan, kp.row0, kp.row0 + e) > aai_covered_pixels(&plan, kp.row1 - e, kp.row1) ? 1 : 0;
         }
         int e;
         if (mode == AAI_MODE_FAST)
-            e = aai_launch_fast(kp, arith, src_dtype, dst_dtype, stream);
+            e = aai_launch_fast(kp, tiles, arith, src_dtype, dst_dtype, stream);
         else if (plan.axis_aligned)
             e = aai_launch_separable(kp, arith, src_dtype, dst_dtype, stream);
         else
-            e = aai_launch_overlap(kp, arith, src_dtype, dst_dtype, stream);
+            e = aai_launch_overlap(kp, tiles, arith, src_dtype, dst_dtype, stream);
         if (e != (int)cudaSuccess) return e;
         g_launches.fetch_add(1);
     }
diff --git a/area_average_interpolation_b200/csrc/aai_device.cuh b/area_average_interpolation_b200/csrc/aai_device.cuh
--- a/area_average_interpolation_b200/csrc/aai_device.cuh
+++ b/area_average_interpolation_b200/csrc/aai_device.cuh
@@ -152,6 +152,47 @@
 }
 __device__ __forceinline__ int dst_row0(const AaiKernelParams &kp) {
     return kp.dst_y0 - (int)blockIdx.z * kp.dst_batch_rows;
+}
+
+__device__ __forceinline__ bool covered_tile(const AaiTileTable &tt, bool rev, int &tile_x, int &tile_y) {
+    const int b = (int)blockIdx.x - tt.nrows;
+    if (b < 0) return false;
+    const int t = rev ? tt.ncovered - 1 - b : b;
+    const int h = t >> tt.hint_shift;
+    int lo = tt.hint[h], hi = tt.hint[h + 1];
+    while (lo < hi) {
+        const int mid = (lo + hi + 1) >> 1;
+        if (tt.prefix[mid] <= t)
+            lo = mid;
+        else
+            hi = mid - 1;
+    }
+    tile_y = lo;
+    tile_x = tt.first[lo] + (t - tt.prefix[lo]);
+    return true;
+}
+
+__device__ __forceinline__ void zero_bytes(char *p, int64_t nb, int lane) {
+    if (nb <= 0) return;
+    const int64_t head = min((int64_t)((16 - ((uintptr_t)p & 15)) & 15), nb);
+    if (lane < head) p[lane] = 0;
+    p += head;
+    nb -= head;
+    const int64_t nv = nb >> 4;
+    for (int64_t i = lane; i < nv; i += TILE_W) reinterpret_cast<uint4 *>(p)[i] = make_uint4(0u, 0u, 0u, 0u);
+    if (lane < (nb & 15)) p[(nv << 4) + lane] = 0;
+}
+__device__ __forceinline__ void fill_empty_spans(const AaiKernelParams &kp, const AaiTileTable &tt, int pixel_bytes) {
+    static_assert(TILE_W >= 16, "zero_bytes() stores the up to 15 unaligned end bytes with one lane each");
+    const int k = (int)blockIdx.x;
+    const int y = kp.row0 + k * TILE_H + (int)threadIdx.y;
+    if (y >= kp.row1) return;
+    char *drow = (char *)kp.dst + (int64_t)(y - dst_row0(kp)) * kp.dst_pitch;
+    const int n = tt.prefix[k + 1] - tt.prefix[k];
+    const int64_t xa = n > 0 ? min((int64_t)tt.first[k] * TILE_W, (int64_t)kp.dst_w) : 0;
+    const int64_t xb = n > 0 ? min((int64_t)(tt.first[k] + n) * TILE_W, (int64_t)kp.dst_w) : 0;
+    zero_bytes(drow, xa * pixel_bytes, (int)threadIdx.x);
+    zero_bytes(drow + xb * pixel_bytes, (kp.dst_w - xb) * pixel_bytes, (int)threadIdx.x);
 }
 
 __device__ __forceinline__ void mod_to_src(const AaiKernelParams &kp, int mx, int my, int &sx, int &sy) {
diff --git a/area_average_interpolation_b200/csrc/aai_internal.h b/area_average_interpolation_b200/csrc/aai_internal.h
--- a/area_average_interpolation_b200/csrc/aai_internal.h
+++ b/area_average_interpolation_b200/csrc/aai_internal.h
@@ -43,6 +43,19 @@
     int32_t src_batch_rows, dst_batch_rows;
 };
 
+#define AAI_TILE_TABLE_ROWS 2560
+#define AAI_TILE_HINTS 1024
+struct AaiTileTable {
+    int32_t nrows;
+    int32_t ncovered;
+    int32_t hint_shift;
+    int32_t prefix[AAI_TILE_TABLE_ROWS + 1];
+    int32_t first[AAI_TILE_TABLE_ROWS];
+    uint16_t hint[AAI_TILE_HINTS + 1];
+};
+#define AAI_MAX_TABLE_ROWS_PER_LAUNCH ((long long)AAI_TILE_TABLE_ROWS * AAI_TILE_H)
+const AaiTileTable &aai_tile_table(const aai_plan &plan, int64_t row0, int64_t row1);
+
 inline size_t aai_elem_size(int dtype) {
     switch (dtype) {
         case AAI_F64: return 8;
@@ -71,21 +84,23 @@
 AaiKernelParams aai_make_kernel_params(const aai_plan &plan, const aai_image &src, const aai_image &dst,
                                        int64_t row0, int64_t row1);
 
-int aai_launch_overlap(const AaiKernelParams &kp, int arith, int src_dtype, int dst_dtype, void *stream);
+int aai_launch_overlap(const AaiKernelParams &kp, const AaiTileTable &tiles, int arith, int src_dtype, int dst_dtype,
+                       void *stream);
 int aai_launch_separable(const AaiKernelParams &kp, int arith, int src_dtype, int dst_dtype, void *stream);
-int aai_launch_fast(const AaiKernelParams &kp, int arith, int src_dtype, int dst_dtype, void *stream);
+int aai_launch_fast(const AaiKernelParams &kp, const AaiTileTable &tiles, int arith, int src_dtype, int dst_dtype,
+                    void *stream);
 int aai_launch_expand(const AaiKernelParams &kp, int elem_bytes, void *stream);
 int aai_probe_fp32(int blocks, int iters, float *scratch, double *flop, void *stream);
 int aai_launch_separable_tma(const AaiKernelParams &kp, int arith, int src_dtype, int dst_dtype, void *stream);
 int aai_launch_separable_direct_f32(const AaiKernelParams &kp, int src_dtype, int dst_dtype, void *stream);
-int aai_launch_overlap_f32_n4(const AaiKernelParams &kp, int src_dtype, int dst_dtype, void *stream);
-int aai_launch_overlap_f32_n5(const AaiKernelParams &kp, int src_dtype, int dst_dtype, void *stream);
-int aai_launch_overlap_f32_n6(const AaiKernelParams &kp, int src_dtype, int dst_dtype, void *stream);
-int aai_launch_overlap_f32_n8(const AaiKernelParams &kp, int src_dtype, int dst_dtype, void *stream);
-int aai_launch_fast_f32_n4(const AaiKernelParams &kp, int src_dtype, int dst_dtype, void *stream);
-int aai_launch_fast_f32_n5(const AaiKernelParams &kp, int src_dtype, int dst_dtype, void *stream);
-int aai_launch_fast_f32_n6(const AaiKernelParams &kp, int src_dtype, int dst_dtype, void *stream);
-int aai_launch_fast_f32_n8(const AaiKernelParams &kp, int src_dtype, int dst_dtype, void *stream);
+int aai_launch_overlap_f32_n4(const AaiKernelParams &kp, const AaiTileTable &tiles, int src_dtype, int dst_dtype, void *stream);
+int aai_launch_overlap_f32_n5(const AaiKernelParams &kp, const AaiTileTable &tiles, int src_dtype, int dst_dtype, void *stream);
+int aai_launch_overlap_f32_n6(const AaiKernelParams &kp, const AaiTileTable &tiles, int src_dtype, int dst_dtype, void *stream);
+int aai_launch_overlap_f32_n8(const AaiKernelParams &kp, const AaiTileTable &tiles, int src_dtype, int dst_dtype, void *stream);
+int aai_launch_fast_f32_n4(const AaiKernelParams &kp, const AaiTileTable &tiles, int src_dtype, int dst_dtype, void *stream);
+int aai_launch_fast_f32_n5(const AaiKernelParams &kp, const AaiTileTable &tiles, int src_dtype, int dst_dtype, void *stream);
+int aai_launch_fast_f32_n6(const AaiKernelParams &kp, const AaiTileTable &tiles, int src_dtype, int dst_dtype, void *stream);
+int aai_launch_fast_f32_n8(const AaiKernelParams &kp, const AaiTileTable &tiles, int src_dtype, int dst_dtype, void *stream);
 int aai_launch_fast_bin(const AaiKernelParams &kp, int src_dtype, int dst_dtype, void *stream);
 int aai_launch_overlap_f64_n4(const AaiKernelParams &kp, int src_dtype, int dst_dtype, void *stream);
 int aai_launch_overlap_f64_n5(const AaiKernelParams &kp, int src_dtype, int dst_dtype, void *stream);
diff --git a/area_average_interpolation_b200/csrc/aai_kernels.cu b/area_average_interpolation_b200/csrc/aai_kernels.cu
--- a/area_average_interpolation_b200/csrc/aai_kernels.cu
+++ b/area_average_interpolation_b200/csrc/aai_kernels.cu
@@ -214,13 +214,14 @@
 
 }
 
-int aai_launch_overlap(const AaiKernelParams &kp, int arith, int src_dtype, int dst_dtype, void *stream) {
+int aai_launch_overlap(const AaiKernelParams &kp, const AaiTileTable &tiles, int arith, int src_dtype, int dst_dtype,
+                       void *stream) {
     if (arith == AAI_ARITH_F32 && kp.f32_ok && (kp.channels == 1 || kp.channels == 3)) {
         const int n = (int)floor(2.0 * (double)kp.ext32 + 1e-6) + 1;
-        if (n <= 4) return aai_launch_overlap_f32_n4(kp, src_dtype, dst_dtype, stream);
-        if (n <= 5) return aai_launch_overlap_f32_n5(kp, src_dtype, dst_dtype, stream);
-        if (n <= 6) return aai_launch_overlap_f32_n6(kp, src_dtype, dst_dtype, stream);
-        if (n <= 8) return aai_launch_overlap_f32_n8(kp, src_dtype, dst_dtype, stream);
+        if (n <= 4) return aai_launch_overlap_f32_n4(kp, tiles, src_dtype, dst_dtype, stream);
+        if (n <= 5) return aai_launch_overlap_f32_n5(kp, tiles, src_dtype, dst_dtype, stream);
+        if (n <= 6) return aai_launch_overlap_f32_n6(kp, tiles, src_dtype, dst_dtype, stream);
+        if (n <= 8) return aai_launch_overlap_f32_n8(kp, tiles, src_dtype, dst_dtype, stream);
     }
     const uint64_t max_e = (uint64_t)(kp.mod_w > kp.mod_h ? kp.mod_w : kp.mod_h);
     bool unrolled = kp.shape.sn > 0.0 && kp.shape.cs > 0.0 && max_e * (uint64_t)kp.scale < 0x100000000ULL;
@@ -274,7 +275,8 @@
     return (int)cudaSuccess;
 }
 
-int aai_launch_fast(const AaiKernelParams &kp, int arith, int src_dtype, int dst_dtype, void *stream) {
+int aai_launch_fast(const AaiKernelParams &kp, const AaiTileTable &tiles, int arith, int src_dtype, int dst_dtype,
+                    void *stream) {
     const uint64_t max_e = (uint64_t)(kp.mod_w > kp.mod_h ? kp.mod_w : kp.mod_h);
     const bool f32 = arith == AAI_ARITH_F32 && src_dtype != AAI_F64 && dst_dtype != AAI_F64 && max_e < (1u << 30);
     if (f32 && kp.staged == 2) {
@@ -283,10 +285,10 @@
     }
     if (f32 && (kp.channels == 1 || kp.channels == 3) && max_e * (uint64_t)kp.scale < 0x100000000ULL) {
         const int nf = (int)floor(2.0 * ((double)kp.shapef.hb + 4e-6) + 1e-6) + 1;
-        if (nf <= 3) return aai_launch_fast_f32_n4(kp, src_dtype, dst_dtype, stream);
-        if (nf <= 4) return aai_launch_fast_f32_n5(kp, src_dtype, dst_dtype, stream);
-        if (nf <= 5) return aai_launch_fast_f32_n6(kp, src_dtype, dst_dtype, stream);
-        if (nf <= 7) return aai_launch_fast_f32_n8(kp, src_dtype, dst_dtype, stream);
+        if (nf <= 3) return aai_launch_fast_f32_n4(kp, tiles, src_dtype, dst_dtype, stream);
+        if (nf <= 4) return aai_launch_fast_f32_n5(kp, tiles, src_dtype, dst_dtype, stream);
+        if (nf <= 5) return aai_launch_fast_f32_n6(kp, tiles, src_dtype, dst_dtype, stream);
+        if (nf <= 7) return aai_launch_fast_f32_n8(kp, tiles, src_dtype, dst_dtype, stream);
     }
     return (int)launch_any(f32 ? K_FAST_F32 : K_FAST, kp, src_dtype, dst_dtype, (cudaStream_t)stream);
 }
diff --git a/area_average_interpolation_b200/csrc/aai_kernels_f32.cu b/area_average_interpolation_b200/csrc/aai_kernels_f32.cu
--- a/area_average_interpolation_b200/csrc/aai_kernels_f32.cu
+++ b/area_average_interpolation_b200/csrc/aai_kernels_f32.cu
@@ -2,6 +2,7 @@
 
 #include <algorithm>
 #include <cmath>
+#include <type_traits>
 
 #include "aai_device.cuh"
 
@@ -135,14 +136,14 @@
 #define AAI_F32_MIN_BLOCKS ((AAI_MAXN <= 4 ? 896 : AAI_MAXN == 5 ? 768 : 512) / (AAI_TILE_W * AAI_TILE_H))
 #endif
 enum { ADDR_GENERAL = 0, ADDR_IDENT = 1, ADDR_GROUPED = 2 };
-template <typename TI, typename TO, int NC, int ADDR, bool STAGED, bool PDL = false, bool REV = false>
-__device__ __forceinline__ void overlap_body(const AaiKernelParams &kp, const char *stage, int spitch, int sox, int soy) {
+template <typename TI, typename TO, int NC, int ADDR, bool STAGED, bool PDL = false>
+__device__ __forceinline__ void overlap_body(const AaiKernelParams &kp, const char *stage, int spitch, int sox, int soy,
+                                             int tile_x, int tile_y) {
     constexpr bool IDENT = ADDR == ADDR_IDENT, GROUPED = ADDR == ADDR_GROUPED;
     static_assert(!STAGED || IDENT, "staging is implemented for identity addressing");
     if constexpr (PDL) asm volatile("griddepcontrol.launch_dependents;");
-    const int x = blockIdx.x * TILE_W + threadIdx.x;
-    const int by = REV ? (int)gridDim.y - 1 - (int)blockIdx.y : (int)blockIdx.y;
-    const int y = kp.row0 + by * TILE_H + threadIdx.y;
+    const int x = tile_x * TILE_W + threadIdx.x;
+    const int y = kp.row0 + tile_y * TILE_H + threadIdx.y;
     const bool valid = x < kp.dst_w && y < kp.row1;
     const double cx = fma((double)x, kp.aff_xx, fma((double)y, kp.aff_xy, kp.aff_x0));
     const double cy = fma((double)x, kp.aff_yx, fma((double)y, kp.aff_yy, kp.aff_y0));
@@ -395,10 +396,21 @@
     }
 }
 
+struct NoTiles {};
+template <int ADDR>
+using TilesArg = typename std::conditional<ADDR == ADDR_GROUPED, AaiTileTable, NoTiles>::type;
 template <typename TI, typename TO, int NC, int ADDR, bool PDL = false, bool REV = false>
 __global__ void __launch_bounds__(TILE_W *TILE_H, AAI_F32_MIN_BLOCKS)
-    overlap_kernel_f32(const __grid_constant__ AaiKernelParams kp) {
-    overlap_body<TI, TO, NC, ADDR, false, PDL, REV>(kp, nullptr, 0, 0, 0);
+    overlap_kernel_f32(const __grid_constant__ AaiKernelParams kp, const __grid_constant__ TilesArg<ADDR> tt) {
+    if constexpr (ADDR != ADDR_GROUPED) {
+        const int by = REV ? (int)gridDim.y - 1 - (int)blockIdx.y : (int)blockIdx.y;
+        overlap_body<TI, TO, NC, ADDR, false, PDL>(kp, nullptr, 0, 0, 0, blockIdx.x, by);
+    } else {
+        static_assert(!PDL && !REV, "the short-launch instantiations use identity addressing");
+        int tx, ty;
+        if (!covered_tile(tt, false, tx, ty)) return fill_empty_spans(kp, tt, NC * (int)sizeof(TO));
+        overlap_body<TI, TO, NC, ADDR, false, false>(kp, nullptr, 0, 0, 0, tx, ty);
+    }
 }
 #ifndef AAI_PDL
 #define AAI_PDL 1
@@ -416,8 +428,9 @@
     attr[0].val.programmaticStreamSerializationAllowed = 1;
     cfg.attrs = attr;
     cfg.numAttrs = 1;
-    if (kp.reverse_rows) return cudaLaunchKernelEx(&cfg, overlap_kernel_f32<TI, TO, NC, ADDR_IDENT, true, true>, kp);
-    return cudaLaunchKernelEx(&cfg, overlap_kernel_f32<TI, TO, NC, ADDR_IDENT, true, false>, kp);
+    if (kp.reverse_rows)
+        return cudaLaunchKernelEx(&cfg, overlap_kernel_f32<TI, TO, NC, ADDR_IDENT, true, true>, kp, NoTiles{});
+    return cudaLaunchKernelEx(&cfg, overlap_kernel_f32<TI, TO, NC, ADDR_IDENT, true, false>, kp, NoTiles{});
 }
 
 template <typename TI, typename TO, int NC>
@@ -429,40 +442,49 @@
     __shared__ int origin[2];
     int sox, soy;
     stage_window<(int)sizeof(TI), NC>(&tmap, kp, sp, stage_raw, &bar, origin, kp.ext32, sox, soy);
-    overlap_body<TI, TO, NC, ADDR_IDENT, true>(kp, (const char *)stage_raw, sp.bw * (int)sizeof(TI), sox, soy);
+    overlap_body<TI, TO, NC, ADDR_IDENT, true>(kp, (const char *)stage_raw, sp.bw * (int)sizeof(TI), sox, soy, blockIdx.x,
+                                               blockIdx.y);
 }
 
 template <typename TI, typename TO, int NC>
-cudaError_t launch3(const AaiKernelParams &kp, cudaStream_t stream) {
+cudaError_t launch3(const AaiKernelParams &kp, const AaiTileTable &tt, cudaStream_t stream) {
     const int rows = kp.row1 - kp.row0;
     if (rows <= 0 || kp.dst_w <= 0) return cudaSuccess;
     dim3 block(TILE_W, TILE_H);
-    dim3 grid((kp.dst_w + TILE_W - 1) / TILE_W, (rows + TILE_H - 1) / TILE_H, kp.batch > 1 ? kp.batch : 1);
+    const unsigned nz = kp.batch > 1 ? kp.batch : 1;
+    const dim3 grid((unsigned)(tt.nrows + tt.ncovered), 1, nz);
+    const dim3 grid2((kp.dst_w + TILE_W - 1) / TILE_W, (rows + TILE_H - 1) / TILE_H, nz);
     if (kp.scale == 1 && kp.quadrant == 0) {
         StageHost h;
         if (kp.staged == 1 && stage_prepare<TI, NC>(kp, (double)kp.ext32, h)) {
-            overlap_kernel_f32_tma<TI, TO, NC><<<grid, block, h.smem, stream>>>(h.map, kp, h.sp);
+            overlap_kernel_f32_tma<TI, TO, NC><<<grid2, block, h.smem, stream>>>(h.map, kp, h.sp);
             return cudaGetLastError();
         }
-        if (AAI_PDL && (long long)grid.x * grid.y * grid.z <= kPdlMaxCtas) return launch_short_pdl<TI, TO, NC>(kp, grid, block, stream);
-        overlap_kernel_f32<TI, TO, NC, ADDR_IDENT><<<grid, block, 0, stream>>>(kp);
-    } else if (MAXN == 4 && kp.scale >= MAXN - 1)
-        overlap_kernel_f32<TI, TO, NC, (MAXN == 4 ? ADDR_GROUPED : ADDR_GENERAL)><<<grid, block, 0, stream>>>(kp);
-    else
-        overlap_kernel_f32<TI, TO, NC, ADDR_GENERAL><<<grid, block, 0, stream>>>(kp);
+        if (AAI_PDL && (long long)grid2.x * grid2.y * grid2.z <= kPdlMaxCtas)
+            return launch_short_pdl<TI, TO, NC>(kp, grid2, block, stream);
+        overlap_kernel_f32<TI, TO, NC, ADDR_IDENT><<<grid2, block, 0, stream>>>(kp, NoTiles{});
+        return cudaGetLastError();
+    }
+    if constexpr (MAXN == 4) {
+        if (kp.scale >= MAXN - 1) {
+            overlap_kernel_f32<TI, TO, NC, ADDR_GROUPED><<<grid, block, 0, stream>>>(kp, tt);
+            return cudaGetLastError();
+        }
+    }
+    overlap_kernel_f32<TI, TO, NC, ADDR_GENERAL><<<grid2, block, 0, stream>>>(kp, NoTiles{});
     return cudaGetLastError();
 }
 template <typename TI, typename TO>
-cudaError_t launch2(const AaiKernelParams &kp, cudaStream_t stream) {
-    return kp.channels == 1 ? launch3<TI, TO, 1>(kp, stream) : launch3<TI, TO, 3>(kp, stream);
+cudaError_t launch2(const AaiKernelParams &kp, const AaiTileTable &tt, cudaStream_t stream) {
+    return kp.channels == 1 ? launch3<TI, TO, 1>(kp, tt, stream) : launch3<TI, TO, 3>(kp, tt, stream);
 }
 template <typename TI>
-cudaError_t launch1(const AaiKernelParams &kp, int dst_dtype, cudaStream_t stream) {
+cudaError_t launch1(const AaiKernelParams &kp, const AaiTileTable &tt, int dst_dtype, cudaStream_t stream) {
     switch (dst_dtype) {
-        case AAI_F64: return launch2<TI, double>(kp, stream);
-        case AAI_F32: return launch2<TI, float>(kp, stream);
-        case AAI_U8: if constexpr (pair_ok<TI, uint8_t>()) return launch2<TI, uint8_t>(kp, stream); break;
-        case AAI_U16: if constexpr (pair_ok<TI, uint16_t>()) return launch2<TI, uint16_t>(kp, stream); break;
+        case AAI_F64: return launch2<TI, double>(kp, tt, stream);
+        case AAI_F32: return launch2<TI, float>(kp, tt, stream);
+        case AAI_U8: if constexpr (pair_ok<TI, uint8_t>()) return launch2<TI, uint8_t>(kp, tt, stream); break;
+        case AAI_U16: if constexpr (pair_ok<TI, uint16_t>()) return launch2<TI, uint16_t>(kp, tt, stream); break;
     }
     return cudaErrorInvalidValue;
 }
@@ -649,13 +671,17 @@
 
 template <typename TI, typename TO, int NC, bool IDENT>
 __global__ void __launch_bounds__(TILE_W *TILE_H, 1024 / (TILE_W * TILE_H))
-    fast_kernel_f32u(const __grid_constant__ AaiKernelParams kp) {
-    fast_body<TI, TO, NC, IDENT, false>(kp, nullptr, 0, 0, 0, blockIdx.x, blockIdx.y);
+    fast_kernel_f32u(const __grid_constant__ AaiKernelParams kp, const __grid_constant__ AaiTileTable tt) {
+    int tx, ty;
+    if (!covered_tile(tt, false, tx, ty)) return fill_empty_spans(kp, tt, NC * (int)sizeof(TO));
+    fast_body<TI, TO, NC, IDENT, false>(kp, nullptr, 0, 0, 0, tx, ty);
 }
 template <typename TO>
 __global__ void __launch_bounds__(TILE_W *TILE_H, 1024 / (TILE_W * TILE_H))
-    fast_kernel_f32u_vec(const __grid_constant__ AaiKernelParams kp) {
-    fast_body<float, TO, 1, true, false, true>(kp, nullptr, 0, 0, 0, blockIdx.x, blockIdx.y);
+    fast_kernel_f32u_vec(const __grid_constant__ AaiKernelParams kp, const __grid_constant__ AaiTileTable tt) {
+    int tx, ty;
+    if (!covered_tile(tt, false, tx, ty)) return fill_empty_spans(kp, tt, (int)sizeof(TO));
+    fast_body<float, TO, 1, true, false, true>(kp, nullptr, 0, 0, 0, tx, ty);
 }
 
 template <typename TI, typename TO, int NC>
@@ -736,11 +762,12 @@
 }
 
 template <typename TI, typename TO, int NC>
-cudaError_t launch_fast3(const AaiKernelParams &kp, cudaStream_t stream) {
+cudaError_t launch_fast3(const AaiKernelParams &kp, const AaiTileTable &tt, cudaStream_t stream) {
     const int rows = kp.row1 - kp.row0;
     if (rows <= 0 || kp.dst_w <= 0) return cudaSuccess;
     dim3 block(TILE_W, TILE_H);
     dim3 grid((kp.dst_w + TILE_W - 1) / TILE_W, (rows + TILE_H - 1) / TILE_H, kp.batch > 1 ? kp.batch : 1);
+    const dim3 grid1((unsigned)(tt.nrows + tt.ncovered), 1, grid.z);
     if (kp.scale == 1 && kp.quadrant == 0) {
         StageHost h;
         if ((kp.staged == 1 || kp.staged == 3) && stage_prepare<TI, NC>(kp, (double)kp.shapef.hb + 1e-5, h)) {
@@ -767,28 +794,28 @@
         }
         if constexpr (sizeof(TI) == 4 && NC == 1) {
             if ((kp.src_pitch % 16) == 0 && (reinterpret_cast<uintptr_t>(kp.src) % 16) == 0 && AAI_FAST_VEC_LOADS) {
-                fast_kernel_f32u_vec<TO><<<grid, block, 0, stream>>>(kp);
+                fast_kernel_f32u_vec<TO><<<grid1, block, 0, stream>>>(kp, tt);
                 return cudaGetLastError();
             }
         }
-        fast_kernel_f32u<TI, TO, NC, true><<<grid, block, 0, stream>>>(kp);
+        fast_kernel_f32u<TI, TO, NC, true><<<grid1, block, 0, stream>>>(kp, tt);
     } else {
-        fast_kernel_f32u<TI, TO, NC, false><<<grid, block, 0, stream>>>(kp);
+        fast_kernel_f32u<TI, TO, NC, false><<<grid1, block, 0, stream>>>(kp, tt);
     }
     return cudaGetLastError();
 }
 template <typename TI>
-cudaError_t launch_fast1(const AaiKernelParams &kp, int dst_dtype, cudaStream_t stream) {
+cudaError_t launch_fast1(const AaiKernelParams &kp, const AaiTileTable &tt, int dst_dtype, cudaStream_t stream) {
     const bool one = kp.channels == 1;
     switch (dst_dtype) {
-        case AAI_F32: return one ? launch_fast3<TI, float, 1>(kp, stream) : launch_fast3<TI, float, 3>(kp, stream);
+        case AAI_F32: return one ? launch_fast3<TI, float, 1>(kp, tt, stream) : launch_fast3<TI, float, 3>(kp, tt, stream);
         case AAI_U8:
             if constexpr (pair_ok<TI, uint8_t>())
-                return one ? launch_fast3<TI, uint8_t, 1>(kp, stream) : launch_fast3<TI, uint8_t, 3>(kp, stream);
+                return one ? launch_fast3<TI, uint8_t, 1>(kp, tt, stream) : launch_fast3<TI, uint8_t, 3>(kp, tt, stream);
             break;
         case AAI_U16:
             if constexpr (pair_ok<TI, uint16_t>())
-                return one ? launch_fast3<TI, uint16_t, 1>(kp, stream) : launch_fast3<TI, uint16_t, 3>(kp, stream);
+                return one ? launch_fast3<TI, uint16_t, 1>(kp, tt, stream) : launch_fast3<TI, uint16_t, 3>(kp, tt, stream);
             break;
     }
     return cudaErrorInvalidValue;
@@ -799,23 +826,25 @@
 #define AAI_CAT2(a, b) a##b
 #define AAI_CAT(a, b) AAI_CAT2(a, b)
 
-int AAI_CAT(aai_launch_overlap_f32_n, AAI_MAXN)(const AaiKernelParams &kp, int src_dtype, int dst_dtype, void *stream) {
+int AAI_CAT(aai_launch_overlap_f32_n, AAI_MAXN)(const AaiKernelParams &kp, const AaiTileTable &tiles, int src_dtype,
+                                                int dst_dtype, void *stream) {
     cudaStream_t st = (cudaStream_t)stream;
     switch (src_dtype) {
-        case AAI_F64: return (int)launch1<double>(kp, dst_dtype, st);
-        case AAI_F32: return (int)launch1<float>(kp, dst_dtype, st);
-        case AAI_U8: return (int)launch1<uint8_t>(kp, dst_dtype, st);
-        case AAI_U16: return (int)launch1<uint16_t>(kp, dst_dtype, st);
+        case AAI_F64: return (int)launch1<double>(kp, tiles, dst_dtype, st);
+        case AAI_F32: return (int)launch1<float>(kp, tiles, dst_dtype, st);
+        case AAI_U8: return (int)launch1<uint8_t>(kp, tiles, dst_dtype, st);
+        case AAI_U16: return (int)launch1<uint16_t>(kp, tiles, dst_dtype, st);
         default: return (int)cudaErrorInvalidValue;
     }
 }
 
-int AAI_CAT(aai_launch_fast_f32_n, AAI_MAXN)(const AaiKernelParams &kp, int src_dtype, int dst_dtype, void *stream) {
+int AAI_CAT(aai_launch_fast_f32_n, AAI_MAXN)(const AaiKernelParams &kp, const AaiTileTable &tiles, int src_dtype,
+                                             int dst_dtype, void *stream) {
     cudaStream_t st = (cudaStream_t)stream;
     switch (src_dtype) {
-        case AAI_F32: return (int)launch_fast1<float>(kp, dst_dtype, st);
-        case AAI_U8: return (int)launch_fast1<uint8_t>(kp, dst_dtype, st);
-        case AAI_U16: return (int)launch_fast1<uint16_t>(kp, dst_dtype, st);
+        case AAI_F32: return (int)launch_fast1<float>(kp, tiles, dst_dtype, st);
+        case AAI_U8: return (int)launch_fast1<uint8_t>(kp, tiles, dst_dtype, st);
+        case AAI_U16: return (int)launch_fast1<uint16_t>(kp, tiles, dst_dtype, st);
         default: return (int)cudaErrorInvalidValue;
     }
 }
diff --git a/area_average_interpolation_b200/csrc/aai_plan.cpp b/area_average_interpolation_b200/csrc/aai_plan.cpp
--- a/area_average_interpolation_b200/csrc/aai_plan.cpp
+++ b/area_average_interpolation_b200/csrc/aai_plan.cpp
@@ -46,6 +46,59 @@
     if (xb < xa) xb = xa;
 }
 
+void covered_tile_rows(const aai_plan &p, int64_t row0, int64_t row1, int tile_w, int tile_h, int32_t *first,
+                       int32_t *count, int count_stride) {
+    const int64_t n = (row1 - row0 + tile_h - 1) / tile_h;
+    for (int64_t k = 0; k < n; ++k) {
+        int64_t lo = INT64_MAX, hi = 0;
+        const int64_t y1 = row0 + (k + 1) * tile_h < row1 ? row0 + (k + 1) * tile_h : row1;
+        for (int64_t y = row0 + k * tile_h; y < y1; ++y) {
+            int64_t xa, xb;
+            covered_span(p, y, xa, xb);
+            if (xb > xa) {
+                if (xa < lo) lo = xa;
+                if (xb > hi) hi = xb;
+            }
+        }
+        const bool any = hi > lo;
+        first[k] = any ? (int32_t)(lo / tile_w) : 0;
+        count[k * count_stride] = any ? (int32_t)((hi + tile_w - 1) / tile_w - lo / tile_w) : 0;
+    }
+}
+
+}
+
+const AaiTileTable &aai_tile_table(const aai_plan &plan, int64_t row0, int64_t row1) {
+    struct Cache {
+        aai_plan plan;
+        int64_t row0 = -1, row1 = -1;
+        AaiTileTable t;
+    };
+    static thread_local Cache c;
+    if (c.row0 != row0 || c.row1 != row1 || std::memcmp(&c.plan, &plan, sizeof plan) != 0) {
+        c.row0 = c.row1 = -1;
+        AaiTileTable &u = c.t;
+        const int n = (int)((row1 - row0 + AAI_TILE_H - 1) / AAI_TILE_H);
+        u.nrows = n;
+        covered_tile_rows(plan, row0, row1, AAI_TILE_W, AAI_TILE_H, u.first, u.prefix + 1, 1);
+        u.prefix[0] = 0;
+        for (int k = 0; k < n; ++k) u.prefix[k + 1] += u.prefix[k];
+        u.ncovered = u.prefix[n];
+        int shift = 0;
+        while (((int64_t)AAI_TILE_HINTS << shift) < (int64_t)u.ncovered) ++shift;
+        u.hint_shift = shift;
+        int k = 0;
+        for (int b = 0; b <= AAI_TILE_HINTS; ++b) {
+            const int64_t tb = (int64_t)b << shift;
+            const int64_t tt = tb < u.ncovered ? tb : (int64_t)u.ncovered - 1;
+            while (k + 1 < n && u.prefix[k + 1] <= tt) ++k;
+            u.hint[b] = (uint16_t)k;
+        }
+        c.plan = plan;
+        c.row0 = row0;
+        c.row1 = row1;
+    }
+    return c.t;
 }
 
 extern "C" {
@@ -159,6 +212,15 @@
     return total;
 }
 
+int aai_covered_tiles(const aai_plan *plan, int64_t row0, int64_t row1, int32_t tile_w, int32_t tile_h, int32_t *first,
+                      int32_t *count) {
+    if (!plan || plan->status != AAI_OK || tile_w <= 0 || tile_h <= 0 || !first || !count || row0 < 0 || row0 > row1 ||
+        row1 > plan->dst_h)
+        return AAI_ERR_ARGUMENT;
+    covered_tile_rows(*plan, row0, row1, tile_w, tile_h, first, count, 1);
+    return AAI_OK;
+}
+
 double aai_band_empty_weight(const aai_plan *plan, int mode, int arith) {
     if (mode == AAI_MODE_FAST) return 0.27;
     if (arith == AAI_ARITH_F64) return 0.06;
diff --git a/include/aai.h b/include/aai.h
--- a/include/aai.h
+++ b/include/aai.h
@@ -84,6 +84,9 @@
 
 int64_t aai_covered_pixels(const aai_plan *plan, int64_t row0, int64_t row1);
 
+int aai_covered_tiles(const aai_plan *plan, int64_t row0, int64_t row1, int32_t tile_w, int32_t tile_h, int32_t *first,
+                      int32_t *count);
+
 
 int aai_device_count(void);
 
```

Result: no change. 41570, median of 6 (-0.0%).
